# deepreinforce-ai/CUDA-L2

Measured on NVIDIA H100. Metric: HGEMM TFLOP/s, offline mode, per (M,N,K), higher is better.
Workload: dtype f16 x f16 -> f32 accumulate -> f16

## Files before the change

cuda_l2_b200/build.py:

```python
from __future__ import annotations

import os
import shutil
import subprocess
import sys
from pathlib import Path

PKG_DIR = Path(__file__).resolve().parent
REPO = PKG_DIR.parent
CSRC = PKG_DIR / "csrc"
LIB_DIR = PKG_DIR / "lib"

ARCH_FLAGS = ["-gencode", "arch=compute_90a,code=sm_90a"]
COMMON = ["-std=c++17", "-O3", "-lineinfo", "-Xcompiler", "-fPIC", "-Xcompiler", "-fno-gnu-unique"]


def nvcc_path() -> str:
    cand = os.environ.get("NVCC") or shutil.which("nvcc") or "/usr/local/cuda/bin/nvcc"
    if not Path(cand).exists():
        raise RuntimeError("nvcc not found: the HGEMM library cannot be built")
    return cand


def _stale(out: Path, inputs: list[Path]) -> bool:
    if not out.exists():
        return True
    t = out.stat().st_mtime
    return any(p.stat().st_mtime > t for p in inputs if p.exists())


def _run(cmd: list[str], verbose: bool) -> None:
    if verbose:
        print("+", " ".join(cmd), flush=True)
    r = subprocess.run(cmd, stdout=subprocess.PIPE, stderr=subprocess.STDOUT, text=True)
    if r.returncode != 0:
        sys.stderr.write(r.stdout)
        raise RuntimeError(f"build step failed ({r.returncode}): {' '.join(cmd)}")
    if verbose and r.stdout.strip():
        print(r.stdout)
    elif "warning" in r.stdout.lower():
        sys.stderr.write(r.stdout)
    if "C7510" in r.stdout:
        raise RuntimeError(f"ptxas serialised wgmma (warning C7510) in: {' '.join(cmd)}")


def _headers() -> list[Path]:
    return (sorted(CSRC.glob("*.cuh")) + sorted(CSRC.glob("*.inc")) + sorted(CSRC.glob("*.h")) +
            sorted((REPO / "include").glob("*.h")))


def _compile_and_link(out: Path, objects: list[tuple[Path, list[str]]], link_flags: list[str], verbose: bool,
                      force: bool) -> Path:
    LIB_DIR.mkdir(exist_ok=True)
    if force or _stale(out, [src for src, _ in objects] + _headers()):
        objs = [LIB_DIR / f"{out.stem}_{i}.o" for i in range(len(objects))]
        from concurrent.futures import ThreadPoolExecutor
        with ThreadPoolExecutor(len(objects)) as pool:
            for f in [pool.submit(_run, [nvcc_path(), *ARCH_FLAGS, *COMMON, *defines, "-c", "-o", str(obj), str(src)],
                                  verbose)
                      for (src, defines), obj in zip(objects, objs)]:
                f.result()
        _run([nvcc_path(), *ARCH_FLAGS, *COMMON, "--shared", "-o", str(out), *map(str, objs), *link_flags], verbose)
        for obj in objs:
            obj.unlink()
    return out


VARIANTS = (0, 1, 2)
BLOCK_VARIANTS = (5, 6)
BWD_VARIANTS = (0, 2)
EPILOGUE_VARIANTS = (0, 2, 3, 4)
BLOCK_1D1D_VARIANTS = (7, 8)
WGRAD_ACCUM_VARIANTS = (0, 2, 3, 7)
SWIGLU_VARIANTS = (0, 2)


def _per_variant(source: str, variants: tuple[int, ...]) -> list[tuple[Path, list[str]]]:
    return [(CSRC / source, [f"-DB200_VARIANT={v}"]) for v in variants]


LIBRARIES = {
    "capi": ("libb200_hgemm.so", [(CSRC / "b200_hgemm_capi.cu", []), (CSRC / "b200_fp8_capi.cu", [])], []),
    "fp8block": ("libb200_fp8block.so", [(CSRC / "b200_fp8_block_capi.cu", [])], []),
    "fp8block_1d1d": ("libb200_fp8block_1d1d.so", _per_variant("b200_fp8_block_1d1d.cu", BLOCK_1D1D_VARIANTS), []),
    "batched": ("libb200_batched.so", _per_variant("b200_batched_capi.cu", VARIANTS), []),
    "grouped": ("libb200_grouped.so", _per_variant("b200_grouped_capi.cu", VARIANTS), []),
    "grouped_fp8": ("libb200_grouped_fp8.so", _per_variant("b200_grouped_fp8_capi.cu", BLOCK_VARIANTS), []),
    "batched_fp8": ("libb200_batched_fp8.so", _per_variant("b200_batched_fp8_capi.cu", BLOCK_VARIANTS), []),
    "nn": ("libb200_nn.so", _per_variant("b200_nn.cu", VARIANTS), []),
    "grouped_bwd": ("libb200_grouped_bwd.so", _per_variant("b200_grouped_bwd.cu", BWD_VARIANTS), []),
    "epilogue": ("libb200_epilogue.so", _per_variant("b200_epilogue.cu", EPILOGUE_VARIANTS), []),
    "wgrad_accum": ("libb200_wgrad_accum.so", _per_variant("b200_wgrad_accum.cu", WGRAD_ACCUM_VARIANTS), []),
    "swiglu": ("libb200_swiglu.so", _per_variant("b200_swiglu.cu", SWIGLU_VARIANTS), []),
    "quant": ("libb200_quant.so", [(CSRC / "b200_quant.cu", [])], []),
    "quant_dual": ("libb200_quant_dual.so", [(CSRC / "b200_quant_dual.cu", [])], []),
    "quant_block_dual": ("libb200_quant_block_dual.so", [(CSRC / "b200_quant_block_dual.cu", [])], []),
    "baselines": ("libb200_baselines.so", [(CSRC / "b200_baselines_capi.cu", [])], ["-lcublas", "-lcublasLt"]),
}


def build_library(key: str, verbose: bool = False, force: bool = False) -> Path:
    name, objects, link_flags = LIBRARIES[key]
    return _compile_and_link(LIB_DIR / name, objects, link_flags, verbose, force)


def build_dev_check(verbose: bool = False, force: bool = False) -> Path:
    lib = build_library("capi", verbose, force)
    build_library("baselines", verbose, force)
    out = LIB_DIR / "dev_check"
    src = CSRC / "dev_check.cu"
    if force or _stale(out, [src, lib] + _headers()):
        _run([nvcc_path(), *ARCH_FLAGS, "-std=c++17", "-O3", "-lineinfo", "-o", str(out), str(src),
              f"-L{LIB_DIR}", "-lb200_hgemm", "-lb200_baselines", "-lcublas", "-Xlinker", "-rpath", "-Xlinker", "$ORIGIN"], verbose)
    return out


def build_all(verbose: bool = False, force: bool = False) -> dict[str, Path]:
    from concurrent.futures import ThreadPoolExecutor
    with ThreadPoolExecutor(len(LIBRARIES)) as pool:
        futures = {key: pool.submit(build_library, key, verbose, force) for key in LIBRARIES}
        out = {key: f.result() for key, f in futures.items()}
    out["dev_check"] = build_dev_check(verbose, force)
    return out


if __name__ == "__main__":
    for k, v in build_all(verbose=True, force="--force" in sys.argv).items():
        print(f"{k}: {v}")
```

cuda_l2_b200/capi.py:

```python
from __future__ import annotations

import ctypes
from pathlib import Path
from typing import NamedTuple

LIB_DIR = Path(__file__).resolve().parent / "lib"

ACC_BITS = {"fp32": 32, "fp16": 16, 32: 32, 16: 16}


class B200HgemmError(RuntimeError):
    pass


_vp, _i, _ip = ctypes.c_void_p, ctypes.c_int, ctypes.POINTER(ctypes.c_int)
_TILE_LIST_ABI = {
    "gemm": ([_i, _vp, _vp, _vp, _vp, _i, _i, _i, _i, _vp], _i),
    "gemm_run_config": ([_i, _i, _vp, _vp, _vp, _vp, _i, _i, _i, _i, _i, _i, _vp], _i),
    "select": ([_i, _i, _i, _i, _i, _ip, _ip], _i),
    "schedule_units": ([_i, _i, _i, _i, _i, _ip, _i, _i, _ip, _i, _ip], _i),
    "launch_count": ([], ctypes.c_ulonglong),
    "strerror": ([_i], ctypes.c_char_p),
}
_FP8_TILE_LIST_ABI = {
    "gemm": ([_vp, _vp, _vp, _vp, _i, _vp, _i, _vp, _i, _i, _i, _i, _vp], _i),
    "gemm_run_config": ([_i, _i, _vp, _vp, _vp, _vp, _i, _vp, _vp, _i, _i, _i, _i, _i, _i, _vp], _i),
    "select": ([_i, _i, _i, _i, _ip, _ip], _i),
    "launch_count": ([], ctypes.c_ulonglong),
    "strerror": ([_i], ctypes.c_char_p),
}


def _prefixed(prefix: str, abi: dict) -> dict:
    return {f"b200_{prefix}_{suffix}": sig for suffix, sig in abi.items()}


_GEMM = ([_vp, _vp, _vp, _vp, _i, _i, _i, _vp], _i)
_FP8GEMM = ([_vp, _vp, _vp, _vp, _vp, _i, _i, _i, _i, _vp], _i)
_FP8GEMM_RUN_CONFIG = ([_i, _i, _vp, _vp, _vp, _vp, _vp, _i, _i, _i, _i, _i, _i, _vp], _i)
_BASELINE = ([_i, _i, _vp, _vp, _vp, _i, _i, _i], _i)
ABI = {
    "libb200_hgemm.so": {
        "b200_hgemm_f32acc": _GEMM,
        "b200_hgemm_f16acc": _GEMM,
        "b200_bgemm_f32acc": _GEMM,
        "b200_bgemm_run_config": ([_i, _vp, _vp, _vp, _i, _i, _i, _i, _i, _i, _vp], _i),
        "b200_fp8gemm": _FP8GEMM,
        "b200_fp8gemm_run_config": _FP8GEMM_RUN_CONFIG,
        "b200_fp8gemm_rowwise": _FP8GEMM,
        "b200_fp8gemm_rowwise_run_config": _FP8GEMM_RUN_CONFIG,
        "b200_fp8gemm_select": ([_i, _i, _i, _ip, _ip, _ip], _i),
        "b200_hgemm_num_configs": ([], _i),
        "b200_hgemm_config_info": ([_i, _ip, _ip, _ip], _i),
        "b200_hgemm_config_cluster": ([_i, _ip, _ip], _i),
        "b200_hgemm_config_m_rep": ([_i], _i),
        "b200_hgemm_config_stages_requested": ([_i], _i),
        "b200_hgemm_select_config": ([_i, _i, _i, _i], _i),
        "b200_hgemm_select": ([_i, _i, _i, _i, _ip, _ip, _ip], _i),
        "b200_hgemm_run_config": ([_i, _i, _vp, _vp, _vp, _i, _i, _i, _i, _i, _i, _vp], _i),
        "b200_hgemm_host": ([_i, _vp, _vp, _vp, _i, _i, _i], _i),
        "b200_hgemm_schedule_units": ([_i, _i, _i, _i, _i, _i, _i, _ip, _i, _ip, _ip, _ip, _ip], _i),
        "b200_hgemm_prewarm": ([_vp], _i),
        "b200_hgemm_release": ([], _i),
        "b200_hgemm_launch_count": ([], ctypes.c_ulonglong),
        "b200_hgemm_strerror": ([_i], ctypes.c_char_p),
    },
    "libb200_fp8block.so": {
        "b200_fp8gemm_blockwise": ([_vp, _vp, _vp, _vp, _i, _vp, _i, _i, _i, _i, _vp], _i),
        "b200_fp8gemm_blockwise_run_config": ([_i, _i, _vp, _vp, _vp, _vp, _i, _vp, _i, _i, _i, _i, _i, _i, _vp], _i),
        "b200_fp8gemm_blockwise_select": ([_i, _i, _i, _ip, _ip, _ip], _i),
        "b200_fp8block_launch_count": ([], ctypes.c_ulonglong),
        "b200_fp8block_strerror": ([_i], ctypes.c_char_p),
    },
    "libb200_batched.so": _prefixed("batched", _TILE_LIST_ABI),
    "libb200_grouped.so": _prefixed("grouped", _TILE_LIST_ABI),
    "libb200_grouped_fp8.so": _prefixed("grouped_fp8", _FP8_TILE_LIST_ABI),
    "libb200_batched_fp8.so": _prefixed("batched_fp8", _FP8_TILE_LIST_ABI),
    "libb200_baselines.so": {
        "b200_bl_init": ([_i], _i),
        "b200_bl_destroy": ([_i], None),
        "b200_bl_cublas": _BASELINE,
        "b200_bl_lt_heuristic": _BASELINE,
        "b200_bl_lt_autotune_find": ([_i, _i, _i, _i, _i, _i, _i], _i),
        "b200_bl_lt_autotune": _BASELINE,
        "b200_bl_lt_autotune_info": ([_i, _i, _ip, ctypes.POINTER(ctypes.c_float)], _i),
    },
}
GROUPED_BWD_LIB = "libb200_grouped_bwd.so"
_BWD_RUN = ([_i, _i, _vp, _vp, _vp, _vp, _i, _i, _i, _i, _i, _i, _vp], _i)
_BWD_SELECT = ([_i, _i, _i, _i, _i, _ip, _ip], _i)
EPILOGUE_LIB = "libb200_epilogue.so"
QUANT_LIB = "libb200_quant.so"
QUANT_DUAL_LIB = "libb200_quant_dual.so"
FP8BLOCK_1D1D_LIB = "libb200_fp8block_1d1d.so"
QUANT_BLOCK_DUAL_LIB = "libb200_quant_block_dual.so"
WGRAD_ACCUM_LIB = "libb200_wgrad_accum.so"
SWIGLU_LIB = "libb200_swiglu.so"
_QUANT_BLOCK_DUAL = ([_i, _vp, _i, _i, _vp, _vp, _vp, _vp, _vp], _i)
_QUANT_BLOCKWISE = ([_i, _vp, _i, _i, _i, _vp, _vp, _i, _vp, _vp], _i)
INTERNAL_ABI = {
    GROUPED_BWD_LIB: {
        "cuda_l2_b200_grouped_bwd_nn": _BWD_RUN,
        "cuda_l2_b200_grouped_bwd_wgrad": _BWD_RUN,
        "cuda_l2_b200_grouped_bwd_nn_select": _BWD_SELECT,
        "cuda_l2_b200_grouped_bwd_wgrad_select": _BWD_SELECT,
        "cuda_l2_b200_grouped_bwd_wgrad_schedule": ([_i, _i, _i, _i, _i, _ip, _i, _i, _ip, _i, _ip], _i),
        "cuda_l2_b200_grouped_bwd_launch_count": ([], ctypes.c_ulonglong),
        "cuda_l2_b200_grouped_bwd_strerror": ([_i], ctypes.c_char_p),
    },
    EPILOGUE_LIB: {
        "cuda_l2_b200_epilogue_run": ([_i, _vp, _vp, _vp, _vp, _vp, _i, _vp, _i, _i, _i, _i, _vp], _i),
        "cuda_l2_b200_epilogue_run_config": ([_i, _i, _vp, _vp, _vp, _vp, _vp, _i, _vp, _i, _i, _i, _i, _i, _i, _i,
                                              _vp], _i),
        "cuda_l2_b200_epilogue_select": ([_i, _i, _i, _i, _ip, _ip, _ip], _i),
        "cuda_l2_b200_epilogue_prewarm": ([_vp], _i),
        "cuda_l2_b200_epilogue_release": ([], _i),
        "cuda_l2_b200_epilogue_launch_count": ([], ctypes.c_ulonglong),
        "cuda_l2_b200_epilogue_strerror": ([_i], ctypes.c_char_p),
    },
    QUANT_LIB: {
        "cuda_l2_b200_quant_e4m3_tensor": ([_i, _vp, ctypes.c_longlong, _vp, _vp, _vp, _vp], _i),
        "cuda_l2_b200_quant_e4m3_rowwise": ([_i, _vp, _i, _i, _vp, _vp, _vp], _i),
        "cuda_l2_b200_quant_e4m3_blockwise": _QUANT_BLOCKWISE,
        "cuda_l2_b200_quant_silu_mul_e4m3_blockwise": _QUANT_BLOCKWISE,
        "cuda_l2_b200_quant_launch_count": ([], ctypes.c_ulonglong),
        "cuda_l2_b200_quant_strerror": ([_i], ctypes.c_char_p),
    },
    QUANT_DUAL_LIB: {
        "cuda_l2_b200_quant_dual_e4m3_rowwise": ([_i, _vp, _i, _i, _vp, _vp, _vp, _vp, _vp, _vp], _i),
        "cuda_l2_b200_quant_dual_launch_count": ([], ctypes.c_ulonglong),
        "cuda_l2_b200_quant_dual_strerror": ([_i], ctypes.c_char_p),
    },
    FP8BLOCK_1D1D_LIB: {
        "cuda_l2_b200_fp8block_1d1d_run": ([_vp, _vp, _vp, _vp, _i, _vp, _i, _i, _i, _i, _i, _vp], _i),
        "cuda_l2_b200_fp8block_1d1d_run_config": ([_i, _i, _vp, _vp, _vp, _vp, _i, _vp, _i, _i, _i, _i, _i, _i, _i,
                                                   _vp], _i),
        "cuda_l2_b200_fp8block_1d1d_select": ([_i, _i, _i, _ip, _ip, _ip], _i),
        "cuda_l2_b200_fp8block_1d1d_launch_count": ([], ctypes.c_ulonglong),
        "cuda_l2_b200_fp8block_1d1d_strerror": ([_i], ctypes.c_char_p),
    },
    QUANT_BLOCK_DUAL_LIB: {
        "cuda_l2_b200_quant_block_dual_e4m3_1x128": _QUANT_BLOCK_DUAL,
        "cuda_l2_b200_quant_block_dual_e4m3_128x128": _QUANT_BLOCK_DUAL,
        "cuda_l2_b200_quant_block_dual_launch_count": ([], ctypes.c_ulonglong),
        "cuda_l2_b200_quant_block_dual_strerror": ([_i], ctypes.c_char_p),
    },
    WGRAD_ACCUM_LIB: {
        "cuda_l2_b200_wgrad_accum_grouped": _BWD_RUN,
        "cuda_l2_b200_wgrad_accum_fp8": ([_i, _i, _vp, _vp, _vp, _vp, _i, _vp, _i, _i, _i, _i, _i, _i, _i, _vp], _i),
        "cuda_l2_b200_wgrad_accum_grouped_select": _BWD_SELECT,
        "cuda_l2_b200_wgrad_accum_fp8_select": ([_i, _i, _i, _i, _ip, _ip, _ip], _i),
        "cuda_l2_b200_wgrad_accum_prewarm": ([_vp], _i),
        "cuda_l2_b200_wgrad_accum_release": ([], _i),
        "cuda_l2_b200_wgrad_accum_launch_count": ([], ctypes.c_ulonglong),
        "cuda_l2_b200_wgrad_accum_strerror": ([_i], ctypes.c_char_p),
    },
    SWIGLU_LIB: {
        "cuda_l2_b200_swiglu_run": ([_i, _vp, _vp, _vp, _vp, _i, _i, _i, _vp], _i),
        "cuda_l2_b200_swiglu_run_config": ([_i, _i, _vp, _vp, _vp, _vp, _i, _i, _i, _i, _i, _i, _vp], _i),
        "cuda_l2_b200_swiglu_select": ([_i, _i, _i, _i, _ip, _ip, _ip], _i),
        "cuda_l2_b200_swiglu_backward": ([_i, _vp, _vp, _vp, _i, _i, _vp], _i),
        "cuda_l2_b200_swiglu_launch_count": ([], ctypes.c_ulonglong),
        "cuda_l2_b200_swiglu_strerror": ([_i], ctypes.c_char_p),
    },
}
_TABLES = {**ABI, **INTERNAL_ABI}
_LIBRARY_OF = {symbol: name for name, table in _TABLES.items() for symbol in table}
_libs: dict = {}


def load(name: str) -> ctypes.CDLL:
    if name not in _libs:
        path = LIB_DIR / name
        if not path.exists():
            raise B200HgemmError(
                f"{path} is missing: build it with `python -c 'import __graft_entry__ as g; g.build()'` "
                "(or `python cuda_l2_b200/build.py`). There is no fallback path.")
        lib = ctypes.CDLL(str(path))
        for sym, (args, res) in _TABLES[name].items():
            fn = getattr(lib, sym)
            fn.argtypes, fn.restype = args, res
        _libs[name] = lib
    return _libs[name]


def hgemm_lib() -> ctypes.CDLL:
    return load("libb200_hgemm.so")


def fp8block_lib() -> ctypes.CDLL:
    return load("libb200_fp8block.so")


def batched_lib() -> ctypes.CDLL:
    return load("libb200_batched.so")


def grouped_lib() -> ctypes.CDLL:
    return load("libb200_grouped.so")


def grouped_fp8_lib() -> ctypes.CDLL:
    return load("libb200_grouped_fp8.so")


def batched_fp8_lib() -> ctypes.CDLL:
    return load("libb200_batched_fp8.so")


def baselines_lib() -> ctypes.CDLL:
    return load("libb200_baselines.so")


def exported_symbols() -> dict[str, list[str]]:
    return {name: list(symbols) for name, symbols in ABI.items()}


def strerror(status: int) -> str:
    return hgemm_lib().b200_hgemm_strerror(status).decode()


def _check(status: int, fn) -> None:
    if status != 0:
        symbol = fn if isinstance(fn, str) else fn.__name__
        name = _LIBRARY_OF[symbol]
        text = getattr(load(name), next(s for s in _TABLES[name] if s.endswith("_strerror")))(status).decode()
        raise B200HgemmError(f"{symbol} failed: status {status} ({text})")


def _shape_check(a, b_col_major, c):
    import torch

    for name, t in (("a", a), ("b_col_major", b_col_major), ("c", c)):
        if t.dtype != torch.half:
            raise B200HgemmError(f"{name} must be torch.half, got {t.dtype}")
        if not t.is_cuda:
            raise B200HgemmError(f"{name} must be a CUDA tensor")
        if not t.is_contiguous():
            raise B200HgemmError(f"{name} must be contiguous")
    m, k = a.shape
    kb, n = b_col_major.shape
    if kb != k or tuple(c.shape) != (m, n):
        raise B200HgemmError(f"shape mismatch: a {tuple(a.shape)}, b_col_major {tuple(b_col_major.shape)}, c {tuple(c.shape)}")
    return m, n, k


def hgemm(a, b_col_major, c, acc: str | int = "fp32", stream: int | None = None) -> None:
    m, n, k = _shape_check(a, b_col_major, c)
    bits = ACC_BITS[acc]
    fn = hgemm_lib().b200_hgemm_f32acc if bits == 32 else hgemm_lib().b200_hgemm_f16acc
    _check(fn(a.data_ptr(), None, b_col_major.data_ptr(), c.data_ptr(), m, n, k, stream), fn)


class GemmType(NamedTuple):
    k_align: int
    scale: object

    def fits(self, n: int, k: int) -> bool:
        return n % 8 == 0 and k % self.k_align == 0


_GEMM_TYPES: dict = {}


def gemm_type(operand, output, acc: str | int = "fp32") -> GemmType | None:
    if not _GEMM_TYPES:
        import torch
        h, b, e, f = torch.float16, torch.bfloat16, torch.float8_e4m3fn, torch.float32
        _GEMM_TYPES.update({(h, h, 32): GemmType(8, None), (h, h, 16): GemmType(8, None), (b, b, 32): GemmType(8, None),
                            (e, h, 32): GemmType(16, f), (e, b, 32): GemmType(16, f)})
    return _GEMM_TYPES.get((operand, output, ACC_BITS.get(acc)))


BLOCK = 128


def num_k_blocks(k: int) -> int:
    return -(-k // BLOCK)


def scale_granularity(m: int, n: int, scale_a, scale_b, k: int | None = None, groups: int | None = None,
                      batches: int | None = None) -> str:
    import torch

    sa, sb = tuple(scale_a.shape), tuple(scale_b.shape)
    lead_a = () if batches is None else (batches,)
    lead = lead_a if groups is None else (groups,)
    plain = groups is None and batches is None
    if scale_a.dtype == torch.float32 and scale_b.dtype == torch.float32:
        if plain and scale_a.numel() == 1 and scale_b.numel() == 1:
            return "tensor"
        if plain and sa == (m, 1) and sb == (1, n):
            return "rowwise"
        nkb = num_k_blocks(k) if k is not None else (sa[-1] if len(sa) == 2 + len(lead_a) else -1)
        if sa == (*lead_a, m, nkb) and sb == (*lead, -(-n // BLOCK), nkb):
            return "blockwise"
        if plain and sa == (m, nkb) and sb == (n, nkb) and n > -(-n // BLOCK):
            return "blockwise_1d1d"
    if groups is not None:
        raise B200HgemmError(f"grouped scales must be fp32 blockwise scales, scale_a [{m}, ceil(K/128)] with scale_b "
                             f"[{groups}, ceil({n}/128), ceil(K/128)], got {scale_a.dtype} {sa} and {scale_b.dtype} {sb}")
    if batches is not None:
        raise B200HgemmError(f"batched scales must be fp32 blockwise scales, scale_a [{batches}, {m}, ceil(K/128)] with "
                             f"scale_b [{batches}, ceil({n}/128), ceil(K/128)], got {scale_a.dtype} {sa} and "
                             f"{scale_b.dtype} {sb}")
    raise B200HgemmError(f"scales must be fp32 and either both one-element (per tensor), scale_a [{m}, 1] with "
                         f"scale_b [1, {n}] (rowwise), or scale_a [{m}, ceil(K/128)] with scale_b [ceil({n}/128), "
                         f"ceil(K/128)] (blockwise) or [{n}, ceil(K/128)] (blockwise_1d1d), got {scale_a.dtype} {sa} and "
                         f"{scale_b.dtype} {sb}")


def blockwise_ld_a(scale_a) -> int | None:
    *lead, m, nkb = scale_a.shape
    bsz, st = (lead[0] if lead else 1), scale_a.stride()
    ld = st[-1] if nkb > 1 else _m_major_ld(m)
    if nkb == 1 and bsz > 1:
        ld = st[0]
# ... 338 lines not shown
        raise B200HgemmError(f"the grouped backward takes fp16 or bf16 operands with fp32 accumulation, got {dtype} "
                             f"with acc={acc!r}")
    return v


def _bwd_operand_type(a, b, acc: str | int) -> GemmType:
    t = _operand_type(a, b, a.dtype, acc, (), scaled=False)
    _bwd_variant(a.dtype, acc)
    return t


def check_grouped_nn_operands(a, b, offs, acc: str | int = "fp32") -> tuple[int, int, int, int]:
    try:
        (t, k), (g, k2, n) = a.shape, b.shape
    except ValueError:
        raise B200HgemmError(f"a [T, K] and b [G, K, N] expected, got {tuple(a.shape)} and {tuple(b.shape)}") from None
    typ = _bwd_operand_type(a, b, acc)
    if k2 != k:
        raise B200HgemmError(f"inner dimensions differ: a {tuple(a.shape)}, b {tuple(b.shape)} (row-major: [G, K, N])")
    if not typ.fits(n, k):
        raise B200HgemmError(f"{a.dtype} operands need N % 8 == 0 and K % 8 == 0 (16-byte TMA strides), got N={n}, K={k}")
    _check_offs(offs, g)
    return g, t, n, k


def check_grouped_wgrad_operands(a, b, offs, acc: str | int = "fp32") -> tuple[int, int, int, int]:
    try:
        (t, m), (t2, n) = a.shape, b.shape
        (g,) = offs.shape
    except ValueError:
        raise B200HgemmError(f"a [T, M], b [T, N] and offs [G] expected, got {tuple(a.shape)}, {tuple(b.shape)} and "
                             f"{tuple(offs.shape)}") from None
    typ = _bwd_operand_type(a, b, acc)
    if t2 != t:
        raise B200HgemmError(f"row counts differ: a {tuple(a.shape)}, b {tuple(b.shape)}")
    if not typ.fits(n, m):
        raise B200HgemmError(f"{a.dtype} operands need M % 8 == 0 and N % 8 == 0 (16-byte TMA strides), got M={m}, N={n}")
    if g < 1:
        raise B200HgemmError("offs must hold at least one group")
    _check_offs(offs, g)
    return g, t, m, n


def _bwd_call(symbol: str, variant: int, ptrs: tuple, problem: tuple, config_id: int | None, group_m: int,
              max_ctas: int, stream: int | None) -> None:
    _check(getattr(grouped_bwd_lib(), symbol)(variant, -1 if config_id is None else config_id, *ptrs, *problem, group_m,
                                              max_ctas, stream), symbol)


def gemm_grouped_nn(a, b, c, offs, acc: str | int = "fp32", config_id: int | None = None, group_m: int = 0,
                    max_ctas: int = 0, stream: int | None = None) -> None:
    _contiguous_cuda(a=a, b=b, c=c, offs=offs)
    g, t, n, k = check_grouped_nn_operands(a, b, offs, acc)
    if c.dtype != a.dtype or tuple(c.shape) != (t, n):
        raise B200HgemmError(f"c must be {a.dtype} {[t, n]}, got {c.dtype} {tuple(c.shape)}")
    _bwd_call("cuda_l2_b200_grouped_bwd_nn", _bwd_variant(a.dtype, acc), (a.data_ptr(), b.data_ptr(), c.data_ptr(),
              offs.data_ptr()), (g, t, n, k), config_id, group_m, max_ctas, stream)


def gemm_grouped_wgrad(a, b, c, offs, acc: str | int = "fp32", config_id: int | None = None, group_m: int = 0,
                       max_ctas: int = 0, stream: int | None = None) -> None:
    _contiguous_cuda(a=a, b=b, c=c, offs=offs)
    g, t, m, n = check_grouped_wgrad_operands(a, b, offs, acc)
    if c.dtype != a.dtype or tuple(c.shape) != (g, m, n):
        raise B200HgemmError(f"c must be {a.dtype} {[g, m, n]}, got {c.dtype} {tuple(c.shape)}")
    _bwd_call("cuda_l2_b200_grouped_bwd_wgrad", _bwd_variant(a.dtype, acc), (a.data_ptr(), b.data_ptr(), c.data_ptr(),
              offs.data_ptr()), (g, t, m, n), config_id, group_m, max_ctas, stream)


def grouped_nn_select(variant: int, g: int, t: int, n: int, k: int) -> tuple[int, int]:
    return _select(grouped_bwd_lib().cuda_l2_b200_grouped_bwd_nn_select, variant, g, t, n, k)


def grouped_wgrad_select(variant: int, g: int, t: int, m: int, n: int) -> tuple[int, int]:
    return _select(grouped_bwd_lib().cuda_l2_b200_grouped_bwd_wgrad_select, variant, g, t, m, n)


def grouped_wgrad_schedule(config_id: int, t: int, m: int, n: int, offs, num_sms: int = 132) -> dict:
    ends = (ctypes.c_int * len(offs))(*offs)
    return _tile_list_schedule(grouped_bwd_lib().cuda_l2_b200_grouped_bwd_wgrad_schedule, 4, config_id, len(offs), t,
                               m, n, ends, num_sms)


def grouped_bwd_launch_count() -> int:
    return int(grouped_bwd_lib().cuda_l2_b200_grouped_bwd_launch_count())


def fp8_grouped_gemm(a, b_kmajor, c, scale_a, scale_b, offs, config_id: int | None = None, group_m: int = 0,
                     max_ctas: int = 0, stream: int | None = None) -> None:
    _tile_list_gemm("grouped", a, b_kmajor, c, offs, "fp32", (scale_a, scale_b), config_id, group_m, max_ctas, stream)


def fp8_grouped_select(g: int, t: int, n: int, k: int) -> tuple[int, int]:
    return _select(grouped_fp8_lib().b200_grouped_fp8_select, g, t, n, k)


def fp8_grouped_launch_count() -> int:
    return int(grouped_fp8_lib().b200_grouped_fp8_launch_count())


def fp8_batched_gemm(a, b_kmajor, c, scale_a, scale_b, masked_m=None, config_id: int | None = None, group_m: int = 0,
                     max_ctas: int = 0, stream: int | None = None) -> None:
    _tile_list_gemm("batched", a, b_kmajor, c, masked_m, "fp32", (scale_a, scale_b), config_id, group_m, max_ctas,
                    stream)


def fp8_batched_select(b: int, m: int, n: int, k: int) -> tuple[int, int]:
    return _select(batched_fp8_lib().b200_batched_fp8_select, b, m, n, k)


def fp8_batched_launch_count() -> int:
    return int(batched_fp8_lib().b200_batched_fp8_launch_count())


def hgemm_config(a, b_col_major, c, config_id: int, acc: str | int = "fp32", group_m: int = 0, max_ctas: int = 0,
                 splits: int = 1, stream: int | None = None) -> None:
    m, n, k = _shape_check(a, b_col_major, c)
    _check(hgemm_lib().b200_hgemm_run_config(ACC_BITS[acc], config_id, a.data_ptr(), b_col_major.data_ptr(),
                                            c.data_ptr(), m, n, k, group_m, max_ctas, splits, stream), "b200_hgemm_run_config")


def hgemm_host(a_host, b_col_major_host, c_host, acc: str | int = "fp32") -> None:
    m, k = a_host.shape
    kb, n = b_col_major_host.shape
    assert kb == k and tuple(c_host.shape) == (m, n)
    for t in (a_host, b_col_major_host, c_host):
        assert (not t.is_cuda) and t.is_contiguous()
    _check(hgemm_lib().b200_hgemm_host(ACC_BITS[acc], a_host.data_ptr(), b_col_major_host.data_ptr(),
                                       c_host.data_ptr(), m, n, k), "b200_hgemm_host")


def configs() -> list[dict]:
    lib = hgemm_lib()
    out = []
    for cid in range(lib.b200_hgemm_num_configs()):
        bn, st, cg = ctypes.c_int(), ctypes.c_int(), ctypes.c_int()
        lib.b200_hgemm_config_info(cid, ctypes.byref(bn), ctypes.byref(st), ctypes.byref(cg))
        cm, cn = ctypes.c_int(), ctypes.c_int()
        lib.b200_hgemm_config_cluster(cid, ctypes.byref(cm), ctypes.byref(cn))
        out.append({"id": cid, "bn": bn.value, "stages": st.value, "cta_group": cg.value,
                    "stages_requested": lib.b200_hgemm_config_stages_requested(cid),
                    "cluster_m": cm.value, "cluster_n": cn.value, "m_rep": lib.b200_hgemm_config_m_rep(cid)})
    return out


def select_config(acc: str | int, m: int, n: int, k: int) -> int:
    return hgemm_lib().b200_hgemm_select_config(ACC_BITS[acc], m, n, k)


def select(acc: str | int, m: int, n: int, k: int) -> tuple[int, int, int]:
    return _select(hgemm_lib().b200_hgemm_select, ACC_BITS[acc], m, n, k)


STREAMK_TAIL, STREAMK_TAIL_PLUS_WAVE = 100, 101
KMODES = ("plain", "split-k", "cluster-split-k", "stream-k")


def schedule(config_id: int, m: int, n: int, k: int, splits: int = 1, num_sms: int = 132) -> dict:
    lib = hgemm_lib()
    nw, sk, mode = ctypes.c_int(), ctypes.c_int(), ctypes.c_int()
    cap = 64
    buf, contrib = (ctypes.c_int * (3 * cap))(), (ctypes.c_int * cap)()
    st = lib.b200_hgemm_schedule_units(config_id, m, n, k, splits, num_sms, 0, buf, cap, ctypes.byref(nw),
                                       ctypes.byref(sk), ctypes.byref(mode), contrib)
    _check(min(st, 0), "b200_hgemm_schedule_units")
    units = []
    for w in range(nw.value):
        cnt = lib.b200_hgemm_schedule_units(config_id, m, n, k, splits, num_sms, w, buf, cap, None, None, None, contrib)
        _check(min(cnt, 0), "b200_hgemm_schedule_units")
        if cnt > cap:
            cap = cnt
            buf, contrib = (ctypes.c_int * (3 * cap))(), (ctypes.c_int * cap)()
            cnt = lib.b200_hgemm_schedule_units(config_id, m, n, k, splits, num_sms, w, buf, cap, None, None, None, contrib)
        units.append([(buf[3 * j], buf[3 * j + 1], buf[3 * j + 2], contrib[j]) for j in range(cnt)])
    return {"workers": nw.value, "sk_tiles": sk.value, "mode": KMODES[mode.value], "units": units}


def prewarm(stream: int | None = None) -> None:
    _check(hgemm_lib().b200_hgemm_prewarm(stream), "b200_hgemm_prewarm")


def release() -> None:
    _check(hgemm_lib().b200_hgemm_release(), "b200_hgemm_release")


def gpu_local_cpus(device_index: int = 0) -> set[int] | None:
    import os

    try:
        import pynvml as nv
        nv.nvmlInit()
        vis = os.environ.get("CUDA_VISIBLE_DEVICES")
        phys = device_index
        if vis:
            try:
                phys = int(vis.split(",")[device_index])
            except (ValueError, IndexError):
                pass
        h = nv.nvmlDeviceGetHandleByIndex(phys)
        words = nv.nvmlDeviceGetCpuAffinity(h, ((os.cpu_count() or 64) + 63) // 64)
        cpus = {64 * w + b for w, word in enumerate(words) for b in range(64) if (int(word) >> b) & 1}
        cpus &= os.sched_getaffinity(0)
        return cpus or None
    except Exception:
        return None


class host_near_gpu:

    def __init__(self, device_index: int = 0):
        self.device_index, self.saved, self.cpus = device_index, None, None

    def __enter__(self):
        import os
        self.cpus = gpu_local_cpus(self.device_index)
        if self.cpus:
            self.saved = os.sched_getaffinity(0)
            try:
                os.sched_setaffinity(0, self.cpus)
            except OSError:
                self.saved, self.cpus = None, None
        return self

    def __exit__(self, *exc):
        import os
        if self.saved is not None:
            os.sched_setaffinity(0, self.saved)
        return False


def launch_count() -> int:
    return int(hgemm_lib().b200_hgemm_launch_count())


class Baselines:

    NN, TN = 0, 1

    def __init__(self, acc: str | int = "fp32"):
        self.bits = ACC_BITS[acc]
        self.lib = baselines_lib()
        if self.lib.b200_bl_init(self.bits) != 0:
            raise B200HgemmError("cuBLAS/cuBLASLt handle creation failed")

    def close(self):
        self.lib.b200_bl_destroy(self.bits)

    def _call(self, fn, layout, a, b, c):
        m, k = a.shape
        n = c.shape[1]
        st = fn(self.bits, layout, a.data_ptr(), b.data_ptr(), c.data_ptr(), m, n, k)
        if st != 0:
            raise B200HgemmError(f"baseline call failed with status {st}")

    def cublas(self, layout, a, b, c):
        self._call(self.lib.b200_bl_cublas, layout, a, b, c)

    def lt_heuristic(self, layout, a, b, c):
        self._call(self.lib.b200_bl_lt_heuristic, layout, a, b, c)

    def lt_autotune_find(self, layout, m, n, k, warm_rounds=0, bench_rounds=0):
        st = self.lib.b200_bl_lt_autotune_find(self.bits, layout, m, n, k, warm_rounds, bench_rounds)
        if st != 0:
            raise B200HgemmError(f"cuBLASLt auto-tuning failed with status {st}")
        cand, ms = ctypes.c_int(), ctypes.c_float()
        self.lib.b200_bl_lt_autotune_info(self.bits, layout, ctypes.byref(cand), ctypes.byref(ms))
        return cand.value, ms.value

    def lt_autotune(self, layout, a, b, c):
        self._call(self.lib.b200_bl_lt_autotune, layout, a, b, c)


ACTIVATIONS = {"none": 0, "relu": 1, "gelu_tanh": 2}


def epilogue_lib() -> ctypes.CDLL:
    return load(EPILOGUE_LIB)


def epilogue_variant(operand, out_dtype) -> int:
    import torch

    variants = {(torch.float16, torch.float16): 0, (torch.bfloat16, torch.bfloat16): 2,
                (torch.float8_e4m3fn, torch.float16): 3, (torch.float8_e4m3fn, torch.bfloat16): 4}
    if (operand, out_dtype) not in variants:
        raise B200HgemmError(f"no bias + activation kernel for {operand} -> {out_dtype} (fp16, bf16 with fp32 accumulation; "
                             f"e4m3 -> fp16 / bf16 with per-tensor or rowwise scales)")
    return variants[(operand, out_dtype)]


def activation_code(activation: str) -> int:
    if activation not in ACTIVATIONS:
        raise B200HgemmError(f"unknown activation {activation!r}: one of {', '.join(ACTIVATIONS)}")
    return ACTIVATIONS[activation]


def check_bias(bias, n: int, out_dtype) -> None:
    if bias is not None and (bias.dim() != 1 or bias.shape[0] != n or bias.dtype != out_dtype):
        raise B200HgemmError(f"bias must be 1-D with N = {n} elements of {out_dtype}, got {bias.dtype} "
                             f"{tuple(bias.shape)}")


def _aligned(t):
    if t is None:
        return None
    t = t.contiguous()
# ... 352 lines not shown
```

cuda_l2_b200/csrc/b200_hgemm_capi.cu:

```cuda
#include "../../include/b200_hgemm.h"

#include <dlfcn.h>

#include <cstdlib>
#include <map>
#include <memory>
#include <mutex>
#include <string>

#include "b200_nn.h"
#include "hgemm_configs.cuh"
#include "hgemm_dispatch.cuh"

namespace {

using b200::host::GemmType;

template <class Cfg>
int schedule_units(int M, int N, int K, int splits, int num_sms, int worker, int* units, int max_units,
                   int* num_workers, int* sk_tiles, int* mode, int* contributors) {
  using namespace b200;
  const int max_workers = num_sms / Cfg::CLUSTER_CTAS;
  const host::Plan p = host::plan<Cfg>(M, N, K, splits, max_workers, [=] { return max_workers; });
  if (num_workers) *num_workers = p.workers;
  if (sk_tiles) *sk_tiles = p.sk_tiles;
  if (mode) *mode = p.mode;
  if (worker < 0 || worker >= p.workers) return host::kBadShape;
  WorkIter it(worker, p.workers, p.num_tiles, p.nkb, p.splits, p.sk_tiles);
  WorkUnit u;
  int n = 0;
  while (it.next(u)) {
    if (n < max_units && units) {
      units[3 * n] = u.tile; units[3 * n + 1] = u.kb0; units[3 * n + 2] = u.kb1;
      if (contributors)
        contributors[n] = (p.sk_tiles && u.kb0 == 0 && u.kb1 < p.nkb)
                              ? streamk_contributors(worker, p.workers, p.sk_tiles * p.nkb, u.tile, p.nkb) : 0;
    }
    ++n;
  }
  return n;
}

const b200::ConfigDesc* config_desc(int id) { return id >= 0 && id < b200::kNumConfigs ? &b200::kConfigs[id] : nullptr; }

GemmType fp16_type(int acc_bits) { return acc_bits == 32 ? GemmType::kF16Acc32 : GemmType::kF16Acc16; }

constexpr int kHostBlocks = 8;
struct HostCtx {
  std::mutex mu;
  void* dbuf = nullptr; size_t dcap = 0;
  cudaStream_t in = nullptr, run = nullptr, out = nullptr;
  cudaEvent_t b_in = nullptr, a_in[kHostBlocks] = {}, done[kHostBlocks] = {};
};
std::mutex g_host_mu;
std::map<int, std::unique_ptr<HostCtx>> g_host_ctx;
HostCtx& host_ctx(int dev) {
  std::lock_guard<std::mutex> lock(g_host_mu);
  auto& slot = g_host_ctx[dev];
  if (!slot) slot.reset(new HostCtx());
  return *slot;
}

b200::nn::RunConfigFn nn_run_config() {
  static const b200::nn::RunConfigFn fn = []() -> b200::nn::RunConfigFn {
    Dl_info self{};
    if (!dladdr(reinterpret_cast<const void*>(&nn_run_config), &self) || !self.dli_fname) return nullptr;
    const std::string here(self.dli_fname);
    const size_t slash = here.rfind('/');
    const std::string path = (slash == std::string::npos ? std::string() : here.substr(0, slash + 1)) + b200::nn::kLibrary;
    void* lib = dlopen(path.c_str(), RTLD_NOW | RTLD_LOCAL);
    return lib ? reinterpret_cast<b200::nn::RunConfigFn>(dlsym(lib, b200::nn::kRunConfigSymbol)) : nullptr;
  }();
  return fn;
}

template <GemmType T>
int gemm_rowmajor(const void* A, const void* B_rowmajor, void* C, int M, int N, int K, void* stream) {
  if (const int st = b200::host::validate(T, A, B_rowmajor, C, {}, M, N, K)) return st;
  const b200::nn::RunConfigFn run = nn_run_config();
  if (!run) return b200::host::kNoNNLibrary;
  const b200::dispatch::Choice ch = b200::dispatch::select_rowmajor(T, M, N, K);
  const int st = run(int(T), ch.config_id, A, B_rowmajor, C, M, N, K, ch.group_m, 0, ch.splits,
                     &b200::host::splitk_scratch, stream);
  if (st == b200::host::kOk) b200::g_launches.fetch_add(1, std::memory_order_relaxed);
  return st;
}

}

extern "C" {

int b200_hgemm_num_configs(void) { return b200::kNumConfigs; }

int b200_hgemm_config_info(int config_id, int* bn, int* stages, int* cta_group) {
  const b200::ConfigDesc* c = config_desc(config_id);
  if (!c) return b200::host::kBadConfig;
  if (bn) *bn = c->bn;
  if (stages) *stages = c->stages;
  if (cta_group) *cta_group = c->cta_group;
  return 0;
}

int b200_hgemm_config_cluster(int config_id, int* cluster_m, int* cluster_n) {
  const b200::ConfigDesc* c = config_desc(config_id);
  if (!c) return b200::host::kBadConfig;
  if (cluster_m) *cluster_m = c->cluster_m;
  if (cluster_n) *cluster_n = c->cluster_n;
  return 0;
}

int b200_hgemm_schedule_units(int config_id, int M, int N, int K, int splits, int num_sms, int worker, int* units,
                              int max_units, int* num_workers, int* sk_tiles, int* mode, int* contributors) {
  if (M <= 0 || N <= 0 || K <= 0 || num_sms <= 0) return b200::host::kBadShape;
  switch (config_id) {
#define B200_CASE(ID, BN, STAGES, CG, CM, CN, MR)                                                                   \
  case ID:                                                                                                          \
    return schedule_units<b200::Config<BN, STAGES, CG, true, CM, CN, MR>>(M, N, K, splits, num_sms, worker, units, \
                                                                          max_units, num_workers, sk_tiles, mode, contributors);
    B200_HGEMM_CONFIGS(B200_CASE)
#undef B200_CASE
    default:
      return b200::host::kBadConfig;
  }
}

int b200_hgemm_config_stages_requested(int config_id) {
  const b200::ConfigDesc* c = config_desc(config_id);
  return c ? c->stages_requested : b200::host::kBadConfig;
}

int b200_hgemm_config_m_rep(int config_id) {
  const b200::ConfigDesc* c = config_desc(config_id);
  return c ? c->m_rep : b200::host::kBadConfig;
}

int b200_hgemm_select_config(int acc_bits, int M, int N, int K) {
  if (acc_bits != 32 && acc_bits != 16) return b200::host::kBadConfig;
  if (M <= 0 || N <= 0 || K <= 0) return b200::host::kBadShape;
  return b200::dispatch::select(fp16_type(acc_bits), M, N, K).config_id;
}

int b200_hgemm_select(int acc_bits, int M, int N, int K, int* config_id, int* group_m, int* splits) {
  if (acc_bits != 32 && acc_bits != 16) return b200::host::kBadConfig;
  if (M <= 0 || N <= 0 || K <= 0) return b200::host::kBadShape;
  const b200::dispatch::Choice ch = b200::dispatch::select(fp16_type(acc_bits), M, N, K);
  if (config_id) *config_id = ch.config_id;
  if (group_m) *group_m = ch.group_m;
  if (splits) *splits = ch.splits;
  return 0;
}

int b200_hgemm_run_config(int acc_bits, int config_id, const void* A, const void* B_kmajor, void* C, int M,
                          int N, int K, int group_m, int max_ctas, int splits, void* stream) {
  if (acc_bits == 32)
    return b200::run_config<GemmType::kF16Acc32>(config_id, A, B_kmajor, C, {}, M, N, K, group_m, max_ctas, splits, stream);
  if (acc_bits == 16)
    return b200::run_config<GemmType::kF16Acc16>(config_id, A, B_kmajor, C, {}, M, N, K, group_m, max_ctas, splits, stream);
  return b200::host::kBadConfig;
}

int b200_hgemm_f32acc(const void* A, const void* B_rowmajor, const void* B_kmajor, void* C, int M, int N,
                      int K, void* stream) {
  if (!B_kmajor && B_rowmajor) return gemm_rowmajor<GemmType::kF16Acc32>(A, B_rowmajor, C, M, N, K, stream);
  return b200::dispatch::gemm<GemmType::kF16Acc32>(A, B_kmajor, C, {}, M, N, K, stream);
}

int b200_hgemm_f16acc(const void* A, const void* B_rowmajor, const void* B_kmajor, void* C, int M, int N,
                      int K, void* stream) {
  if (!B_kmajor && B_rowmajor) return gemm_rowmajor<GemmType::kF16Acc16>(A, B_rowmajor, C, M, N, K, stream);
  return b200::dispatch::gemm<GemmType::kF16Acc16>(A, B_kmajor, C, {}, M, N, K, stream);
}

int b200_bgemm_f32acc(const void* A, const void* B_rowmajor, const void* B_kmajor, void* C, int M, int N,
                      int K, void* stream) {
  if (!B_kmajor && B_rowmajor) return gemm_rowmajor<GemmType::kBF16>(A, B_rowmajor, C, M, N, K, stream);
  return b200::dispatch::gemm<GemmType::kBF16>(A, B_kmajor, C, {}, M, N, K, stream);
}

int b200_bgemm_run_config(int config_id, const void* A, const void* B_kmajor, void* C, int M, int N, int K,
                          int group_m, int max_ctas, int splits, void* stream) {
  return b200::run_config<GemmType::kBF16>(config_id, A, B_kmajor, C, {}, M, N, K, group_m, max_ctas, splits, stream);
}

int b200_hgemm_host(int acc_bits, const void* hA, const void* hB_kmajor, void* hC, int M, int N, int K) {
  if (!hA || !hB_kmajor || !hC) return b200::host::kNullPointer;
  if (M <= 0 || N <= 0 || K <= 0) return b200::host::kBadShape;
  if (acc_bits != 32 && acc_bits != 16) return b200::host::kBadConfig;
  int dev = 0;
  cudaError_t e = cudaGetDevice(&dev);
  if (e != cudaSuccess) return int(e);
  HostCtx& ctx = host_ctx(dev);
  std::lock_guard<std::mutex> turn(ctx.mu);
  const size_t a_bytes = size_t(M) * K * 2, b_bytes = size_t(N) * K * 2, c_bytes = size_t(M) * N * 2;
  auto up = [](size_t x) { return (x + 255) & ~size_t(255); };
  const size_t need = up(a_bytes) + up(b_bytes) + up(c_bytes);
  if (need > ctx.dcap) {
    if (ctx.dbuf) cudaFree(ctx.dbuf);
    ctx.dbuf = nullptr; ctx.dcap = 0;
    if ((e = cudaMalloc(&ctx.dbuf, need)) != cudaSuccess) return int(e);
    ctx.dcap = need;
  }
  char* dA = static_cast<char*>(ctx.dbuf);
  char* dB = dA + up(a_bytes);
  char* dC = dB + up(b_bytes);
  auto gemm = [&](const void* a, void* c, int m, cudaStream_t s) {
    return acc_bits == 32 ? b200_hgemm_f32acc(a, nullptr, dB, c, m, N, K, s) : b200_hgemm_f16acc(a, nullptr, dB, c, m, N, K, s);
  };

  const int blocks = std::min(kHostBlocks, M / 512);
  const bool pipelined = blocks >= 2 && (a_bytes + c_bytes) >= (size_t(8) << 20) &&
                         !(std::getenv("B200_HGEMM_HOST_UNPIPELINED"));
  if (!pipelined) {
    if ((e = cudaMemcpyAsync(dA, hA, a_bytes, cudaMemcpyHostToDevice, 0)) != cudaSuccess) return int(e);
    if ((e = cudaMemcpyAsync(dB, hB_kmajor, b_bytes, cudaMemcpyHostToDevice, 0)) != cudaSuccess) return int(e);
    int st = gemm(dA, dC, M, nullptr);
    if (st) return st;
    if ((e = cudaMemcpyAsync(hC, dC, c_bytes, cudaMemcpyDeviceToHost, 0)) != cudaSuccess) return int(e);
    e = cudaStreamSynchronize(0);
    return e == cudaSuccess ? 0 : int(e);
  }

  if (!ctx.in) {
    if ((e = cudaStreamCreateWithFlags(&ctx.in, cudaStreamNonBlocking)) != cudaSuccess) return int(e);
    if ((e = cudaStreamCreateWithFlags(&ctx.run, cudaStreamNonBlocking)) != cudaSuccess) return int(e);
    if ((e = cudaStreamCreateWithFlags(&ctx.out, cudaStreamNonBlocking)) != cudaSuccess) return int(e);
    if ((e = cudaEventCreateWithFlags(&ctx.b_in, cudaEventDisableTiming)) != cudaSuccess) return int(e);
    for (int i = 0; i < kHostBlocks; ++i) {
      if ((e = cudaEventCreateWithFlags(&ctx.a_in[i], cudaEventDisableTiming)) != cudaSuccess) return int(e);
      if ((e = cudaEventCreateWithFlags(&ctx.done[i], cudaEventDisableTiming)) != cudaSuccess) return int(e);
    }
  }
  if ((e = cudaStreamSynchronize(0)) != cudaSuccess) return int(e);
  const int rows_per = ((M + blocks - 1) / blocks + 127) / 128 * 128;
  if ((e = cudaMemcpyAsync(dB, hB_kmajor, b_bytes, cudaMemcpyHostToDevice, ctx.in)) != cudaSuccess) return int(e);
  if ((e = cudaEventRecord(ctx.b_in, ctx.in)) != cudaSuccess) return int(e);
  if ((e = cudaStreamWaitEvent(ctx.run, ctx.b_in, 0)) != cudaSuccess) return int(e);
  for (int i = 0; i < blocks; ++i) {
    const int r0 = i * rows_per, rows = std::min(rows_per, M - r0);
    if (rows <= 0) break;
    const size_t a_off = size_t(r0) * K * 2, c_off = size_t(r0) * N * 2;
    if ((e = cudaMemcpyAsync(dA + a_off, static_cast<const char*>(hA) + a_off, size_t(rows) * K * 2, cudaMemcpyHostToDevice, ctx.in)) != cudaSuccess) return int(e);
    if ((e = cudaEventRecord(ctx.a_in[i], ctx.in)) != cudaSuccess) return int(e);
    if ((e = cudaStreamWaitEvent(ctx.run, ctx.a_in[i], 0)) != cudaSuccess) return int(e);
    int st = gemm(dA + a_off, dC + c_off, rows, ctx.run);
    if (st) { cudaDeviceSynchronize(); return st; }
    if ((e = cudaEventRecord(ctx.done[i], ctx.run)) != cudaSuccess) return int(e);
    if ((e = cudaStreamWaitEvent(ctx.out, ctx.done[i], 0)) != cudaSuccess) return int(e);
    if ((e = cudaMemcpyAsync(static_cast<char*>(hC) + c_off, dC + c_off, size_t(rows) * N * 2, cudaMemcpyDeviceToHost, ctx.out)) != cudaSuccess) return int(e);
  }
  if ((e = cudaStreamSynchronize(ctx.out)) != cudaSuccess) return int(e);
  if ((e = cudaStreamSynchronize(ctx.run)) != cudaSuccess) return int(e);
  e = cudaStreamSynchronize(ctx.in);
  return e == cudaSuccess ? 0 : int(e);
}

int b200_hgemm_prewarm(void* stream) {
  int dev = 0;
  cudaError_t e = cudaGetDevice(&dev);
  if (e != cudaSuccess) return int(e);
  b200::host::SplitKScratch* sk = nullptr;
  return b200::host::splitk_scratch(dev, static_cast<cudaStream_t>(stream), &sk);
}

int b200_hgemm_release(void) {
  b200::host::release_scratch();
  int cur = 0;
  cudaGetDevice(&cur);
  std::lock_guard<std::mutex> lock(g_host_mu);
  for (auto& kv : g_host_ctx) {
    HostCtx& c = *kv.second;
    std::lock_guard<std::mutex> turn(c.mu);
    cudaSetDevice(kv.first);
    cudaDeviceSynchronize();
    if (c.dbuf) cudaFree(c.dbuf);
    c.dbuf = nullptr; c.dcap = 0;
    if (c.in) {
      cudaStreamDestroy(c.in); cudaStreamDestroy(c.run); cudaStreamDestroy(c.out);
      cudaEventDestroy(c.b_in);
      for (int i = 0; i < kHostBlocks; ++i) { cudaEventDestroy(c.a_in[i]); cudaEventDestroy(c.done[i]); }
      c.in = c.run = c.out = nullptr;
    }
  }
  cudaSetDevice(cur);
  cudaError_t e = cudaGetLastError();
  return e == cudaSuccess ? 0 : int(e);
}

unsigned long long b200_hgemm_launch_count(void) { return b200::g_launches.load(std::memory_order_relaxed); }

const char* b200_hgemm_strerror(int status) { return b200::host::status_string(status); }

}
```

cuda_l2_b200/csrc/hgemm_configs.cuh:

```cuda
#pragma once
#include <atomic>
#include <type_traits>

#include "hgemm_host.cuh"

#define B200_HGEMM_CONFIGS(X) \
  X(0, 256, 4, 1, 1, 1, 1)       \
  X(1, 128, 6, 1, 1, 1, 1)       \
  X(2, 64, 8, 1, 1, 1, 1)        \
  X(3, 256, 6, 2, 1, 1, 1)       \
  X(4, 128, 8, 2, 1, 1, 1)       \
  X(5, 192, 4, 1, 1, 1, 1)       \
  X(6, 192, 6, 2, 1, 1, 1)       \
  X(7, 64, 8, 1, 1, 2, 1)        \
  X(8, 64, 8, 1, 1, 4, 1)        \
  X(9, 64, 8, 1, 2, 2, 1)        \
  X(10, 128, 6, 1, 1, 2, 1)      \
  X(11, 128, 6, 1, 2, 2, 1)      \
  X(12, 32, 9, 1, 1, 1, 1)       \
  X(13, 32, 9, 1, 1, 4, 1)       \
  X(14, 32, 9, 1, 1, 8, 1)       \
  X(15, 64, 8, 1, 2, 1, 1)       \
  X(16, 64, 8, 1, 4, 1, 1)       \
  X(17, 128, 6, 1, 2, 1, 1)      \
  X(18, 256, 4, 1, 1, 2, 1)      \
  X(19, 256, 4, 1, 2, 1, 1)      \
  X(20, 256, 6, 2, 1, 2, 1)      \
  X(21, 256, 6, 2, 2, 1, 1)      \
  X(22, 128, 8, 2, 1, 2, 1)      \
  X(23, 128, 8, 2, 2, 1, 1)      \
  X(24, 192, 6, 2, 1, 2, 1)      \
  X(25, 192, 6, 2, 2, 1, 1)     \
  X(26, 128, 4, 2, 1, 1, 2)      \
  X(27, 128, 4, 2, 2, 1, 2)      \
  X(28, 128, 4, 2, 1, 2, 2)      \
  X(29, 256, 6, 2, 2, 2, 1)      \
  X(30, 128, 8, 2, 2, 2, 1)

namespace b200 {
constexpr int kNumConfigs = 31;

struct ConfigDesc {
  int bn, stages, stages_requested, cta_group, cluster_m, cluster_n, m_rep;
  bool split_k, stream_k;
};
template <class Cfg>
constexpr ConfigDesc describe(int stages_requested) {
  return ConfigDesc{Cfg::BN, Cfg::STAGES, stages_requested, Cfg::CTA_GROUP, Cfg::CLUSTER_M, Cfg::CLUSTER_N, Cfg::M_REP,
                    Cfg::SPLIT_K, Cfg::STREAM_K};
}
constexpr ConfigDesc kConfigs[kNumConfigs] = {
#define B200_DESC(ID, BN, STAGES, CG, CM, CN, MR) describe<Config<BN, STAGES, CG, true, CM, CN, MR>>(STAGES),
    B200_HGEMM_CONFIGS(B200_DESC)
#undef B200_DESC
};

namespace block {

constexpr bool eligible(int id) { return kConfigs[id].m_rep * kConfigs[id].bn <= 128; }

constexpr int sibling(int id) {
  const ConfigDesc& c = kConfigs[id];
  const int bn = c.bn < 128 ? c.bn : 128;
  for (int j = 0; j < kNumConfigs; ++j) {
    const ConfigDesc& d = kConfigs[j];
    if (d.cta_group == c.cta_group && d.cluster_m == c.cluster_m && d.cluster_n == c.cluster_n && d.m_rep == 1 &&
        d.bn == bn)
      return j;
  }
  return -1;
}
constexpr bool every_config_has_an_eligible_sibling() {
  for (int id = 0; id < kNumConfigs; ++id) {
    const int s = sibling(id);
    if (s < 0 || !eligible(s) || (eligible(id) && s != id)) return false;
  }
  return true;
}
static_assert(every_config_has_an_eligible_sibling(), "the configuration table lost a block-scaled sibling");

constexpr unsigned kModes = (1u << kPlain) | (1u << kClusterSplitK);

}

namespace nn {

constexpr bool has_kernel(int id) { return kConfigs[id].bn % 64 == 0; }

constexpr int sibling(int id) {
  const ConfigDesc& c = kConfigs[id];
  if (has_kernel(id)) return id;
  int best = -1;
  for (int j = 0; j < kNumConfigs; ++j) {
    const ConfigDesc& d = kConfigs[j];
    if (d.bn == 64 && d.cta_group == c.cta_group && d.cluster_m == c.cluster_m && d.m_rep == c.m_rep &&
        d.cluster_n <= c.cluster_n && (best < 0 || d.cluster_n > kConfigs[best].cluster_n))
      best = j;
  }
  return best;
}
constexpr bool every_config_has_a_sibling() {
  for (int id = 0; id < kNumConfigs; ++id) {
    const int s = sibling(id);
    if (s < 0 || !has_kernel(s) || (has_kernel(id) && s != id)) return false;
  }
  return true;
}
static_assert(every_config_has_a_sibling(), "the configuration table lost a row-major B sibling");

}

namespace gated {

constexpr bool has_kernel(int id) { return kConfigs[id].bn == 128 || kConfigs[id].bn == 256; }

constexpr int sibling(int id) {
  const ConfigDesc& c = kConfigs[id];
  if (has_kernel(id)) return id;
  int best = -1;
  for (int j = 0; j < kNumConfigs; ++j) {
    const ConfigDesc& d = kConfigs[j];
    if (d.bn == 128 && d.cta_group == c.cta_group && d.m_rep == c.m_rep && d.cluster_m <= c.cluster_m &&
        d.cluster_n <= c.cluster_n &&
        (best < 0 || d.cluster_m * d.cluster_n > kConfigs[best].cluster_m * kConfigs[best].cluster_n))
      best = j;
  }
  return best;
}
constexpr bool every_config_has_a_sibling() {
  for (int id = 0; id < kNumConfigs; ++id) {
    const int s = sibling(id);
    if (s < 0 || !has_kernel(s) || (has_kernel(id) && s != id)) return false;
  }
  return true;
}
static_assert(every_config_has_a_sibling(), "the configuration table lost a SwiGLU sibling");

constexpr unsigned kModes = 1u << kPlain;

}

template <class Probe>
constexpr bool has_kernel(int id) {
  return block_scaled<Probe>() ? block::eligible(id)
         : row_major_b<Probe>() ? nn::has_kernel(id)
         : is_gated<Probe>()    ? gated::has_kernel(id)
                                : true;
}
template <class Probe>
constexpr unsigned k_modes() { return block_scaled<Probe>() ? block::kModes : is_gated<Probe>() ? gated::kModes : 0xFu; }

template <class Cfg>
using Unwrapped = Cfg;

__attribute__((visibility("hidden"))) inline std::atomic<unsigned long long> g_launches{0};

template <host::GemmType T, template <class> class Wrapper = Unwrapped>
int run_config(int id, const void* A, const void* Bt, void* C, Scales scales, int M, int N, int K, int group_m,
               int max_ctas, int splits, void* stream, int ld_a = 0, host::ScratchFn scratch = host::splitk_scratch,
               const void* bias = nullptr, int act = kActNone, int ld_b = 0) {
  constexpr host::GemmTypeTraits t = host::traits(T);
  using Probe = Wrapper<Config<128, 6, 1, t.acc_f32, 1, 1, 1, t.bf16(), t.e4m3()>>;
  const cudaStream_t s = static_cast<cudaStream_t>(stream);
  int st = host::kBadConfig;
  switch (id) {
#define B200_CASE(ID, BN, STAGES, CG, CM, CN, MR)                                                                  \
  case ID:                                                                                                     \
    if constexpr (has_kernel<Probe>(ID))                                                                       \
      st = host::launch<Wrapper<Config<BN, STAGES, CG, t.acc_f32, CM, CN, MR, t.bf16(), t.e4m3()>>,            \
                        k_modes<Probe>()>(A, Bt, C, M, N, K, s, group_m, max_ctas, splits, scales, ld_a, scratch, \
                                          bias, act, ld_b);                                                    \
    break;
    B200_HGEMM_CONFIGS(B200_CASE)
#undef B200_CASE
    default:
      break;
  }
  if (st == host::kOk) g_launches.fetch_add(1, std::memory_order_relaxed);
  return st;
}

namespace tile_list {

inline bool known_out(int out_bf16) { return out_bf16 == 0 || out_bf16 == 1; }
inline host::GemmType block_type(int out_bf16) { return host::GemmType(int(host::GemmType::kE4M3F16Block) + out_bf16); }
inline Scales block_scales(const void* a, const void* b) {
  return Scales{static_cast<const float*>(a), static_cast<const float*>(b)};
}

__attribute__((visibility("hidden"))) inline std::atomic<unsigned long long> g_list_launches{0};

template <host::GemmType T, class Cfg>
using Variant = std::conditional_t<host::traits(T).block, BlockScaled<Cfg>, Cfg>;

template <template <class> class Wrapper, host::GemmType T>
int run_config(int id, const void* A, const void* Bt, void* C, const int* list, int count, int rows, int N, int K,
               int group_m, int max_ctas, cudaStream_t s, Scales scales, int ld_a) {
  constexpr host::GemmTypeTraits t = host::traits(T);
  static_assert(!t.scaled || t.block, "16-bit or block-scaled variants");
  using Probe = Wrapper<Variant<T, Config<128, 6, 1, t.acc_f32, 1, 1, 1, t.bf16(), t.e4m3()>>>;
  int st = host::kBadConfig;
  switch (id) {
#define B200_CASE(ID, BN, STAGES, CG, CM, CN, MR)                                                                  \
  case ID:                                                                                                     \
    if constexpr (has_kernel<Probe>(ID))                                                                       \
      st = host::launch_list<Wrapper<Variant<T, Config<BN, STAGES, CG, t.acc_f32, CM, CN, MR, t.bf16(), t.e4m3()>>>>( \
          A, Bt, C, list, count, rows, N, K, s, group_m, max_ctas, scales, ld_a);                               \
    break;
    B200_HGEMM_CONFIGS(B200_CASE)
#undef B200_CASE
    default:
      break;
  }
  if (st == host::kOk && rows > 0 && K > 0) g_list_launches.fetch_add(1, std::memory_order_relaxed);
  return st;
}

template <template <class> class Wrapper, host::GemmType... Types>
struct ListLibrary {};

template <template <class> class Wrapper, host::GemmType... Types>
constexpr bool holds(ListLibrary<Wrapper, Types...>, int variant) {
  return ((variant == int(Types)) || ...);
}

template <template <class> class Wrapper>
using ListProbe = Wrapper<Config<128, 6, 1, true>>;

#define B200_LIST_TYPES(X, W) X(W, host::GemmType::kF16Acc32) X(W, host::GemmType::kF16Acc16) X(W, host::GemmType::kBF16)
#define B200_BLOCK_LIST_TYPES(X, W) X(W, host::GemmType::kE4M3F16Block) X(W, host::GemmType::kE4M3BF16Block)

#define B200_LIST_RUN(W, T)                                                                                    \
  int run_config<W, T>(int, const void*, const void*, void*, const int*, int, int, int, int, int, int, cudaStream_t, \
                       Scales, int)
#define B200_LIST_EXTERN(W, T) extern template B200_LIST_RUN(W, T);
#define B200_LIST_ARG(W, T) , T
#define B200_LIST_OBJECT(NAME, W, TYPES)                                                                       \
  TYPES(B200_LIST_EXTERN, W)                                                                                   \
  template B200_LIST_RUN(W, host::GemmType(B200_VARIANT));                                                     \
  using NAME = ListLibrary<W TYPES(B200_LIST_ARG, W)>

template <template <class> class Wrapper, host::GemmType... Types>
int run(ListLibrary<Wrapper, Types...>, host::GemmType type, int config_id, const void* A, const void* Bt, void* C,
        Scales scales, int ld_a, const int* list, int count, int rows, int N, int K, int group_m, int max_ctas,
        void* stream) {
  const cudaStream_t s = static_cast<cudaStream_t>(stream);
  int st = host::kBadConfig;
  (void)((type == Types && (st = run_config<Wrapper, Types>(config_id, A, Bt, C, list, count, rows, N, K, group_m,
                                                            max_ctas, s, scales, ld_a), true)) || ...);
  return st;
}

template <class Cfg>
int schedule_units(int count, int rows, int N, int K, const int* list, int num_sms, int worker, int* units,
                   int max_units, int* num_workers) {
  const long long tiles = Cfg::Cursor::template max_tiles<Cfg>(count, rows, N);
  if (tiles > 0x7fffffffLL) return host::kBadShape;
  const int max_workers = num_sms / Cfg::CLUSTER_CTAS;
  const host::Plan p = host::list_plan<Cfg>(tiles, K, max_workers, [=] { return max_workers; });
  if (num_workers) *num_workers = p.workers;
  if (worker < 0 || worker >= p.workers) return host::kBadShape;
  const int n_blocks = (N + Cfg::BN * Cfg::CLUSTER_N - 1) / (Cfg::BN * Cfg::CLUSTER_N);
  typename Cfg::Cursor cursor = make_cursor<Cfg>(list, count, rows, K, Cfg::TILE_M * Cfg::CLUSTER_M, n_blocks,
                                                 host::default_group_m<Cfg>());
  constexpr int kInts = k_grouped<Cfg>() ? 4 : 3;
  WorkIter it(worker, p.workers, cursor.total(), p.nkb, 1, 0);
  WorkUnit u;
  int n = 0;
  while (it.next(u)) {
    BatchTile bt;
    if constexpr (k_grouped<Cfg>()) bt = cursor.unit(u);
    else bt = cursor.locate(u.tile);
    if (n < max_units && units) {
      int* v = units + kInts * n;
      v[0] = bt.batch; v[1] = bt.tc.m_blk; v[2] = bt.tc.n_blk;
      if constexpr (k_grouped<Cfg>()) v[3] = u.kb1 - u.kb0;
    }
    ++n;
  }
  return n;
}

template <template <class> class Wrapper>
long long fewest_tiles(int count, int rows, int N, bool block_only = false) {
  long long fewest = 0x7fffffffffffffffLL;
#define B200_TILES(ID, BN, STAGES, CG, CM, CN, MR)                                                               \
  if constexpr (has_kernel<ListProbe<Wrapper>>(ID)) {                                                           \
    using W = Wrapper<Config<BN, STAGES, CG, true, CM, CN, MR>>;                                                \
    if (!block_only || block::eligible(ID))                                                                     \
      fewest = std::min(fewest, W::Cursor::template max_tiles<W>(count, rows, N));                              \
  }
  B200_HGEMM_CONFIGS(B200_TILES)
#undef B200_TILES
  return fewest;
}

template <template <class> class Wrapper>
int schedule_config(int config_id, int count, int rows, int N, int K, const int* list, int num_sms, int worker,
                    int* units, int max_units, int* num_workers) {
  switch (config_id) {
#define B200_CASE(ID, BN, STAGES, CG, CM, CN, MR)                                                                 \
  case ID:                                                                                                      \
    if constexpr (has_kernel<ListProbe<Wrapper>>(ID))                                                           \
// ... 15 lines not shown
```

cuda_l2_b200/csrc/hgemm_host.cuh:

```cuda
#pragma once
#include <cuda.h>
#include <cuda_runtime.h>
#include <cstdint>
#include <cstdio>
#include <cstring>
#include <cstdlib>
#include <algorithm>
#include <deque>
#include <mutex>

#include "hgemm_sm90.cuh"

namespace b200 {
namespace host {

enum Status : int {
  kOk = 0,
  kBadShape = -1,
  kBadAlignment = -2,
  kNoDriver = -3,
  kEncodeFailed = -4,
  kNullPointer = -5,
  kBadConfig = -6,
  kNotHopper = -7,
  kNoScratch = -8,
  kBadFp8K = -9,
  kBadScaleLd = -10,
  kNoNNLibrary = -11,
  kBadActivation = -12,
  kBadScaleLdB = -13,
};

inline const char* status_string(int s) {
  switch (s) {
    case kOk: return "ok";
    case kBadShape: return "M, N and K must be positive";
    case kBadAlignment: return "operands must be 16-byte aligned with K % 8 == 0 and N % 8 == 0";
    case kNoDriver: return "cuTensorMapEncodeTiled unavailable (driver too old?)";
    case kEncodeFailed: return "cuTensorMapEncodeTiled failed";
    case kNullPointer: return "null operand pointer";
    case kBadConfig: return "unknown kernel configuration id";
    case kNotHopper: return "device is not compute capability 9.0 (sm_90a build)";
    case kNoScratch: return "split-K scratch unavailable (allocate it outside stream capture with b200_hgemm_prewarm)";
    case kBadFp8K: return "e4m3 operands need K % 16 == 0 (16-byte row strides at one byte per element)";
    case kBadScaleLd: return "block scales need ld_a >= M and ld_a % 4 == 0 (16-byte aligned k-block rows of A's scales)";
    case kNoNNLibrary: return "row-major B needs libb200_nn.so next to libb200_hgemm.so (missing, or it does not load)";
    case kBadActivation: return "unknown activation code (0 none, 1 relu, 2 gelu_tanh)";
    case kBadScaleLdB: return "1 x 128 scales of Bt need ld_b >= N and ld_b % 4 == 0 (16-byte aligned k-block rows)";
    default: return s > 0 ? cudaGetErrorString(static_cast<cudaError_t>(s)) : "unknown error";
  }
}

using EncodeTiledFn = CUresult (*)(CUtensorMap*, CUtensorMapDataType, cuuint32_t, void*, const cuuint64_t*,
                                   const cuuint64_t*, const cuuint32_t*, const cuuint32_t*,
                                   CUtensorMapInterleave, CUtensorMapSwizzle, CUtensorMapL2promotion,
                                   CUtensorMapFloatOOBfill);

inline EncodeTiledFn encode_fn() {
  static EncodeTiledFn fn = [] {
    void* p = nullptr;
    cudaDriverEntryPointQueryResult q;
    if (cudaGetDriverEntryPoint("cuTensorMapEncodeTiled", &p, cudaEnableDefault, &q) != cudaSuccess ||
        q != cudaDriverEntryPointSuccess)
      p = nullptr;
    return reinterpret_cast<EncodeTiledFn>(p);
  }();
  return fn;
}

enum class Elem : int { kF16 = 0, kBF16 = 1, kE4M3 = 2 };
constexpr int elem_bytes(Elem e) { return e == Elem::kE4M3 ? 1 : 2; }

enum class GemmType : int { kF16Acc32, kF16Acc16, kBF16, kE4M3F16, kE4M3BF16, kE4M3F16Block, kE4M3BF16Block,
                            kE4M3F16Block1D1D, kE4M3BF16Block1D1D };
struct GemmTypeTraits {
  Elem operand, output;
  bool acc_f32;
  int table_k_div;
  bool scaled;
  bool block = false;
  bool block_1d1d = false;
  constexpr bool bf16() const { return output == Elem::kBF16; }
  constexpr bool e4m3() const { return operand == Elem::kE4M3; }
};
constexpr GemmTypeTraits kGemmTypes[] = {
    {Elem::kF16, Elem::kF16, true, 1, false},
    {Elem::kF16, Elem::kF16, false, 1, false},
    {Elem::kBF16, Elem::kBF16, true, 1, false},
    {Elem::kE4M3, Elem::kF16, true, 2, true},
    {Elem::kE4M3, Elem::kBF16, true, 2, true},
    {Elem::kE4M3, Elem::kF16, true, 2, true, true},
    {Elem::kE4M3, Elem::kBF16, true, 2, true, true},
    {Elem::kE4M3, Elem::kF16, true, 2, true, true, true},
    {Elem::kE4M3, Elem::kBF16, true, 2, true, true, true},
};
constexpr const GemmTypeTraits& traits(GemmType t) { return kGemmTypes[int(t)]; }

template <class Cfg>
constexpr GemmType gemm_type(int t = 0) {
  const GemmTypeTraits& x = kGemmTypes[t];
  return x.acc_f32 == Cfg::ACC_F32 && x.bf16() == Cfg::BF16 && x.e4m3() == Cfg::E4M3 && x.block == block_scaled<Cfg>() &&
                 x.block_1d1d == block_1d1d<Cfg>()
             ? GemmType(t) : gemm_type<Cfg>(t + 1);
}

inline int encode_2d(CUtensorMap* map, const void* ptr, int rows, int cols, int box_rows, int box_cols = kBlockK,
                     Elem elem = Elem::kF16, int batches = 0) {
  EncodeTiledFn fn = encode_fn();
  if (!fn) return kNoDriver;
  const cuuint32_t rank = batches > 0 ? 3 : 2;
  cuuint64_t dims[3] = {cuuint64_t(cols), cuuint64_t(rows), cuuint64_t(batches)};
  cuuint64_t strides[2] = {cuuint64_t(cols) * elem_bytes(elem), cuuint64_t(rows) * cuuint64_t(cols) * elem_bytes(elem)};
  cuuint32_t box[3] = {cuuint32_t(box_cols), cuuint32_t(box_rows), 1};
  cuuint32_t estr[3] = {1, 1, 1};
  const CUtensorMapSwizzle swz = box_cols * elem_bytes(elem) == 128 ? CU_TENSOR_MAP_SWIZZLE_128B : CU_TENSOR_MAP_SWIZZLE_64B;
  static const CUtensorMapL2promotion promo = [] {
    const char* e = std::getenv("B200_HGEMM_L2_PROMOTION");
    const int v = (e && e[0] >= '0' && e[0] <= '3') ? e[0] - '0' : 3;
    return v == 0 ? CU_TENSOR_MAP_L2_PROMOTION_NONE : v == 1 ? CU_TENSOR_MAP_L2_PROMOTION_L2_64B
         : v == 2 ? CU_TENSOR_MAP_L2_PROMOTION_L2_128B : CU_TENSOR_MAP_L2_PROMOTION_L2_256B;
  }();
  const CUtensorMapDataType dt = elem == Elem::kE4M3 ? CU_TENSOR_MAP_DATA_TYPE_UINT8
                               : elem == Elem::kBF16 ? CU_TENSOR_MAP_DATA_TYPE_BFLOAT16 : CU_TENSOR_MAP_DATA_TYPE_FLOAT16;
  CUresult r = fn(map, dt, rank, const_cast<void*>(ptr), dims, strides, box, estr,
                  CU_TENSOR_MAP_INTERLEAVE_NONE, swz, promo, CU_TENSOR_MAP_FLOAT_OOB_FILL_NONE);
  return r == CUDA_SUCCESS ? kOk : kEncodeFailed;
}

struct MapKey {
  const void* ptr; int rows, cols, box_rows, box_cols; Elem elem; int batches;
  bool operator==(const MapKey& o) const {
    return ptr == o.ptr && rows == o.rows && cols == o.cols && box_rows == o.box_rows && box_cols == o.box_cols &&
           elem == o.elem && batches == o.batches;
  }
};
struct MapCache {
  static constexpr int kSlots = 64;
  MapKey keys[kSlots];
  CUtensorMap maps[kSlots];
  bool valid[kSlots];
  MapCache() { std::memset(valid, 0, sizeof(valid)); }
  int get(const void* ptr, int rows, int cols, int box_rows, CUtensorMap* out, int box_cols = kBlockK, Elem elem = Elem::kF16,
          int batches = 0) {
    MapKey k{ptr, rows, cols, box_rows, box_cols, elem, batches};
    uint64_t h = (reinterpret_cast<uint64_t>(ptr) >> 8) * 0x9E3779B97F4A7C15ull;
    h ^= uint64_t(uint32_t(rows)) * 0xC2B2AE3D27D4EB4Full + uint64_t(uint32_t(cols)) * 0x165667B19E3779F9ull +
         uint64_t(box_rows) * 131u + uint64_t(box_cols) + uint64_t(uint32_t(batches)) * 0x27D4EB2F165667C5ull;
    int slot = int((h >> 32) % kSlots);
    if (!(valid[slot] && keys[slot] == k)) {
      int st = encode_2d(&maps[slot], ptr, rows, cols, box_rows, box_cols, elem, batches);
      if (st != kOk) { valid[slot] = false; return st; }
      keys[slot] = k;
      valid[slot] = true;
    }
    std::memcpy(out, &maps[slot], sizeof(CUtensorMap));
    return kOk;
  }
};
inline MapCache& map_cache() {
  static thread_local MapCache c;
  return c;
}

struct DeviceInfo { int dev; int num_sms; int cc_major; };
inline const DeviceInfo& device_info() {
  static thread_local int cached_dev = -1;
  static thread_local DeviceInfo info{-1, 0, 0};
  int dev = 0;
  cudaGetDevice(&dev);
  if (dev != cached_dev) {
    cudaSetDevice(dev);
    cudaDeviceGetAttribute(&info.num_sms, cudaDevAttrMultiProcessorCount, dev);
    cudaDeviceGetAttribute(&info.cc_major, cudaDevAttrComputeCapabilityMajor, dev);
    info.dev = dev;
    cached_dev = dev;
  }
  return info;
}

inline int validate(GemmType type, const void* A, const void* Bt, const void* C, Scales scales, int M, int N, int K,
                    int ld_a = 0, int batches = 1, long long tiles = 1, const int* list = nullptr) {
  const GemmTypeTraits& t = traits(type);
  if (!A || !Bt || !C || (t.scaled && (!scales.a || !scales.b))) return kNullPointer;
  if (M <= 0 || N <= 0 || K <= 0 || batches < 1 || tiles > 0x7fffffffLL) return kBadShape;
  if (reinterpret_cast<uintptr_t>(list) & 3) return kBadAlignment;
  if (K % (16 / elem_bytes(t.operand))) return t.e4m3() ? kBadFp8K : kBadAlignment;
  if (N % 8) return kBadAlignment;
  if ((reinterpret_cast<uintptr_t>(A) | reinterpret_cast<uintptr_t>(Bt) | reinterpret_cast<uintptr_t>(C)) & 15)
    return kBadAlignment;
  if (t.block) {
    if ((reinterpret_cast<uintptr_t>(scales.a) & 15) || (reinterpret_cast<uintptr_t>(scales.b) & (t.block_1d1d ? 15 : 3)))
      return kBadAlignment;
    if (ld_a < M || ld_a % 4) return kBadScaleLd;
    return kOk;
  }
  if (t.scaled && ((reinterpret_cast<uintptr_t>(scales.a) | reinterpret_cast<uintptr_t>(scales.b)) & (scales.rowwise ? 15 : 3)))
    return kBadAlignment;
  return kOk;
}

inline int validate_bias_act(const void* bias, int act) {
// ... 167 lines not shown
inline bool cooperative_enabled() {
  static const bool on = [] { const char* e = std::getenv("B200_HGEMM_NO_COOPERATIVE"); return !(e && e[0] == '1'); }();
  return on;
}

inline bool pdl_enabled() {
  static const bool on = [] { const char* e = std::getenv("B200_HGEMM_NO_PDL"); return !(e && e[0] == '1'); }();
  return on;
}

struct LaunchArgs {
  CUtensorMap ma, mb, mc;
  int M, N, K, group_m;
  Plan plan;
  float* ws; unsigned* ctr; __half* c;
  uint64_t hint_a, hint_b;
  Scales scales;
  int ld_a;
  int ld_b;
  int batches;
  const int* masked_m;
  cudaStream_t stream;
  const void* bias;
  int act;
  GatedArgs gated;
};

template <class Cfg>
typename Cfg::EpiArgs epi_args(const LaunchArgs& a) {
  if constexpr (is_gated<Cfg>()) return a.gated;
  else if constexpr (accum_f32<Cfg>())
    return typename Cfg::EpiArgs{epi_args<typename Cfg::AccumBase>(a), reinterpret_cast<float*>(a.c)};
  else if constexpr (bias_act<Cfg>()) return BiasActArgs{a.scales, a.bias, a.act};
  else if constexpr (block_1d1d<Cfg>()) return Block1D1DArgs{a.scales, a.ld_b};
  else return a.scales;
}

template <class Cfg, int KMODE>
int launch_mode(const DeviceInfo& di, const LaunchArgs& a) {
  static thread_local int attr_dev = -1;
  static thread_local const void* attr_fn = nullptr;
  constexpr auto kernel = kernel_of<Cfg, KMODE>();
  const void* this_fn = reinterpret_cast<const void*>(kernel);
  if (attr_dev != di.dev || attr_fn != this_fn) {
    cudaError_t e = cudaFuncSetAttribute(kernel, cudaFuncAttributeMaxDynamicSharedMemorySize, Cfg::SMEM_BYTES);
    if (e != cudaSuccess) return int(e);
    attr_dev = di.dev;
    attr_fn = this_fn;
  }
  constexpr bool kSplit = (KMODE == kWorkspaceSplitK || KMODE == kClusterSplitK);
  const int cluster = (KMODE == kClusterSplitK) ? a.plan.cluster_reduce : Cfg::CLUSTER_CTAS;
  cudaLaunchConfig_t cfg{};
  cfg.gridDim = dim3(unsigned(a.plan.workers * (kSplit ? 1 : Cfg::CLUSTER_CTAS)), 1, 1);
  cfg.blockDim = dim3(Cfg::NUM_THREADS, 1, 1);
  cfg.dynamicSmemBytes = Cfg::SMEM_BYTES;
  cfg.stream = a.stream;
  cudaLaunchAttribute attr[3];
  unsigned na = 0;
  if (cluster > 1) {
    attr[na].id = cudaLaunchAttributeClusterDimension;
    attr[na].val.clusterDim.x = unsigned(cluster);
    attr[na].val.clusterDim.y = 1;
    attr[na].val.clusterDim.z = 1;
    ++na;
  }
  const bool coop = (KMODE == kWorkspaceSplitK || KMODE == kStreamK) && cooperative_enabled();
  if (coop) {
    attr[na].id = cudaLaunchAttributeCooperative;
    attr[na].val.cooperative = 1;
    ++na;
  }
  static bool coop_pdl_ok = [] { const char* e = std::getenv("B200_HGEMM_COOP_PDL"); return e && e[0] == '1'; }();
  const bool pdl = pdl_enabled() && (!coop || coop_pdl_ok);
  if (pdl) {
    attr[na].id = cudaLaunchAttributeProgrammaticStreamSerialization;
    attr[na].val.programmaticStreamSerializationAllowed = 1;
    ++na;
  }
  cfg.attrs = attr;
  cfg.numAttrs = na;
  const int aux = block_scaled<Cfg>() ? a.ld_a : a.plan.sk_tiles;
  constexpr bool kTileList = batched<Cfg>() || grouped<Cfg>() || k_grouped<Cfg>();
  const int splits_arg = kTileList ? a.batches : a.plan.splits;
  unsigned* ctr = kTileList ? reinterpret_cast<unsigned*>(const_cast<int*>(a.masked_m)) : a.ctr;
  cudaError_t e = cudaLaunchKernelEx(&cfg, kernel, a.ma, a.mb, a.mc, a.M, a.N, a.K, a.group_m, splits_arg, aux, a.ws,
                                     ctr, a.c, a.hint_a, a.hint_b, epi_args<Cfg>(a));
  if (e != cudaSuccess && coop && pdl && e != cudaErrorCooperativeLaunchTooLarge) {
    cudaGetLastError();
    coop_pdl_ok = false;
    cfg.numAttrs = na - 1;
    e = cudaLaunchKernelEx(&cfg, kernel, a.ma, a.mb, a.mc, a.M, a.N, a.K, a.group_m, splits_arg, aux, a.ws, ctr, a.c,
                           a.hint_a, a.hint_b, epi_args<Cfg>(a));
  }
  return e == cudaSuccess ? kOk : int(e);
}

template <class Cfg>
constexpr int default_group_m() { return Cfg::CTA_GROUP == 2 ? 8 : 16; }

template <class Cfg, unsigned MODES = 0xFu>
int launch(const void* A, const void* Bt, void* C, int M, int N, int K, cudaStream_t stream,
           int group_m = 0, int max_ctas = 0, int splits = 1, Scales scales = Scales{nullptr, nullptr}, int ld_a = 0,
           ScratchFn scratch = splitk_scratch, const void* bias = nullptr, int act = kActNone, int ld_b = 0,
           void* y = nullptr) {
  constexpr GemmType kType = gemm_type<Cfg>();
  [[maybe_unused]] const bool store_h = C != nullptr;
  if constexpr (is_gated<Cfg>()) {
    if (!y) return kNullPointer;
    if (!C) C = y;
    if ((reinterpret_cast<uintptr_t>(y) & 15) || N % 128) return kBadAlignment;
  }
  int st = validate(kType, A, Bt, C, scales, M, N, K, ld_a);
  if (st != kOk) return st;
  if constexpr (bias_act<Cfg>()) {
    if ((st = validate_bias_act(bias, act)) != kOk) return st;
  }
  if constexpr (block_1d1d<Cfg>()) {
    if (ld_b < N || ld_b % 4) return kBadScaleLdB;
  }
  const DeviceInfo& di = device_info();
  if (di.cc_major != 9) return kNotHopper;

  LaunchArgs a{};
  MapCache& cache = map_cache();
  const Elem operand = traits(kType).operand, output = traits(kType).output;
  if ((st = cache.get(A, M, K, Cfg::A_BOX_ROWS, &a.ma, Cfg::BLOCK_K, operand)) != kOk) return st;
  if constexpr (row_major_b<Cfg>()) {
    if ((st = cache.get(Bt, K, N, Cfg::B_K_ROWS, &a.mb, 64, operand)) != kOk) return st;
  } else {
    if ((st = cache.get(Bt, N, K, Cfg::B_BOX_ROWS, &a.mb, Cfg::BLOCK_K, operand)) != kOk) return st;
  }
  if constexpr (is_gated<Cfg>()) {
    if ((st = cache.get(store_h ? C : y, M, store_h ? N : N / 2, Cfg::EPI_ROWS, &a.mc, Cfg::EPI_N, output)) != kOk)
      return st;
    if ((st = cache.get(y, M, N / 2, Cfg::EPI_ROWS, &a.gated.y_map, Cfg::EPI_N, output)) != kOk) return st;
    a.gated.store_h = store_h ? 1 : 0;
  } else {
    if ((st = cache.get(C, M, N, Cfg::EPI_ROWS, &a.mc, Cfg::EPI_N, output)) != kOk) return st;
  }

  const int max_workers = (max_ctas > 0 ? max_ctas : di.num_sms) / Cfg::CLUSTER_CTAS;
  a.plan = plan<Cfg, MODES>(M, N, K, splits, max_workers, [&] { return max_resident_clusters<Cfg>(di); });
  if (a.plan.mode == kWorkspaceSplitK || a.plan.mode == kStreamK) {
    SplitKScratch* sk = nullptr;
    if (scratch(di.dev, stream, &sk) == kOk) {
      a.ws = sk->ws; a.ctr = sk->ctr;
    } else {
      cudaGetLastError();
      a.plan = undivided(a.plan);
    }
  }
  a.M = M; a.N = N; a.K = K;
  a.group_m = group_m > 0 ? group_m : default_group_m<Cfg>();
  a.c = static_cast<__half*>(C);
  a.scales = scales;
  a.ld_a = ld_a;
  a.ld_b = ld_b;
  a.stream = stream;
  a.bias = bias;
  a.act = act;
  a.hint_a = ptx::kL2EvictNormal; a.hint_b = ptx::kL2EvictNormal;
  if (cache_hints_enabled()) {
    const size_t a_bytes = size_t(M) * K * Cfg::OP_BYTES, b_bytes = size_t(N) * K * Cfg::OP_BYTES;
    const int n_tiles = (N + Cfg::BN - 1) / Cfg::BN, m_tiles = (M + Cfg::TILE_M - 1) / Cfg::TILE_M;
    constexpr size_t kL2Keep = size_t(20) << 20, kStream = size_t(40) << 20;
    if (a_bytes >= kStream && b_bytes <= kL2Keep && n_tiles <= 4) { a.hint_a = ptx::kL2EvictFirst; a.hint_b = ptx::kL2EvictLast; }
    else if (b_bytes >= kStream && a_bytes <= kL2Keep && m_tiles <= 4) { a.hint_b = ptx::kL2EvictFirst; a.hint_a = ptx::kL2EvictLast; }
  }
  auto or_undivided = [&](int err) {
    if (err != int(cudaErrorCooperativeLaunchTooLarge) && err != int(cudaErrorLaunchOutOfResources)) return err;
    cudaGetLastError();
    a.plan = undivided(a.plan);
    return launch_mode<Cfg, kPlain>(di, a);
  };
  switch (a.plan.mode) {
    case kStreamK:
      if constexpr (has_mode<Cfg, MODES>(kStreamK)) return or_undivided(launch_mode<Cfg, kStreamK>(di, a));
      break;
    case kClusterSplitK:
      if constexpr (has_mode<Cfg, MODES>(kClusterSplitK)) return launch_mode<Cfg, kClusterSplitK>(di, a);
      break;
    case kWorkspaceSplitK:
      if constexpr (has_mode<Cfg, MODES>(kWorkspaceSplitK)) return or_undivided(launch_mode<Cfg, kWorkspaceSplitK>(di, a));
      break;
    case kPlain:
      break;
  }
  return launch_mode<Cfg, kPlain>(di, a);
}

template <class Cfg, class ResidentClusters>
Plan list_plan(long long max_tiles, int K, int max_workers, ResidentClusters&& resident_clusters) {
  Plan p{};
  p.mode = kPlain;
  p.splits = 1;
  p.num_tiles = int(max_tiles);
  p.nkb = (K + Cfg::BLOCK_K - 1) / Cfg::BLOCK_K;
  if (Cfg::CLUSTER_CTAS > 2) max_workers = std::min(max_workers, resident_clusters());
  p.workers = std::min(std::max(max_workers, 1), p.num_tiles);
  return p;
}

inline int validate_grouped(GemmType type, const void* A, const void* Bt, const void* C, const int* offs, int groups,
                            int T, int N, int K, long long worst_tiles, Scales scales = Scales{nullptr, nullptr},
                            int ld_a = 0) {
  if (!A || !Bt || !C || !offs) return kNullPointer;
  if (T < 0 || groups < 1) return kBadShape;
  return validate(type, A, Bt, C, scales, T > 0 ? T : 1, N, K, ld_a, 1, worst_tiles, offs);
}

inline int validate_k_grouped(GemmType type, const void* A, const void* B, const void* C, const int* offs, int groups,
                              int T, int M, int N, long long tiles) {
  if (!C || !offs || (T != 0 && (!A || !B))) return kNullPointer;
  if (T < 0 || groups < 1) return kBadShape;
  if (T == 0) A = B = C;
  return validate(type, A, B, C, Scales{nullptr, nullptr}, M, N, M, 0, 1, tiles, offs);
}

template <class Cfg>
int validate_list(GemmType type, const void* A, const void* Bt, const void* C, const int* list, int count, int rows,
                  int N, int K, long long tiles, Scales scales, int ld_a) {
  return k_grouped<Cfg>() ? validate_k_grouped(type, A, Bt, C, list, count, K, rows, N, tiles)
         : grouped<Cfg>() ? validate_grouped(type, A, Bt, C, list, count, rows, N, K, tiles, scales, ld_a)
                          : validate(type, A, Bt, C, scales, rows, N, K, ld_a, count, tiles, list);
}

template <class Cfg>
int launch_list(const void* A, const void* Bt, void* C, const int* list, int count, int rows, int N, int K,
                cudaStream_t stream, int group_m = 0, int max_ctas = 0, Scales scales = Scales{nullptr, nullptr},
                int ld_a = 0) {
  static_assert(batched<Cfg>() || grouped<Cfg>() || k_grouped<Cfg>(), "a Batched<>, Grouped<> or GroupedK<> configuration");
  constexpr GemmType kType = gemm_type<Cfg>();
  const long long tiles = Cfg::Cursor::template max_tiles<Cfg>(count, rows, N);
  int st = validate_list<Cfg>(kType, A, Bt, C, list, count, rows, N, K, tiles, scales, ld_a);
  if (st != kOk || rows == 0) return st;
  const Elem elem = traits(kType).operand, output = traits(kType).output;
  if constexpr (k_grouped<Cfg>()) {
    if (K == 0) {
      if constexpr (accum_f32<Cfg>()) return kOk;
      const cudaError_t e = cudaMemsetAsync(C, 0, size_t(count) * size_t(rows) * size_t(N) * elem_bytes(output),
                                            stream);
      return e == cudaSuccess ? kOk : int(e);
    }
  }
  const DeviceInfo& di = device_info();
  if (di.cc_major != 9) return kNotHopper;

  LaunchArgs a{};
  MapCache& cache = map_cache();
  if constexpr (k_grouped<Cfg>()) {
    if ((st = cache.get(A, K, rows, Cfg::A_K_ROWS, &a.ma, 64, elem)) != kOk) return st;
    if ((st = cache.get(Bt, K, N, Cfg::B_K_ROWS, &a.mb, 64, elem)) != kOk) return st;
    if ((st = cache.get(C, rows, N, Cfg::EPI_ROWS, &a.mc, Cfg::EPI_N, output, count)) != kOk) return st;
  } else {
  const int depth = batched<Cfg>() ? count : 0;
  if ((st = cache.get(A, rows, K, Cfg::A_BOX_ROWS, &a.ma, Cfg::BLOCK_K, elem, depth)) != kOk) return st;
  if constexpr (row_major_b<Cfg>()) {
    if ((st = cache.get(Bt, K, N, Cfg::B_K_ROWS, &a.mb, 64, elem, count)) != kOk) return st;
  } else {
    if ((st = cache.get(Bt, N, K, Cfg::B_BOX_ROWS, &a.mb, Cfg::BLOCK_K, elem, count)) != kOk) return st;
  }
  if ((st = cache.get(C, rows, N, Cfg::EPI_ROWS, &a.mc, Cfg::EPI_N, output, depth)) != kOk) return st;
  }
  const int max_workers = (max_ctas > 0 ? max_ctas : di.num_sms) / Cfg::CLUSTER_CTAS;
  a.plan = list_plan<Cfg>(tiles, K, max_workers, [&] { return max_resident_clusters<Cfg>(di); });
  a.M = rows; a.N = N; a.K = K;
  a.group_m = group_m > 0 ? group_m : default_group_m<Cfg>();
  a.c = static_cast<__half*>(C);
  a.hint_a = ptx::kL2EvictNormal; a.hint_b = ptx::kL2EvictNormal;
  a.scales = scales;
  a.ld_a = ld_a;
  a.batches = count;
  a.masked_m = list;
  a.stream = stream;
  return launch_mode<Cfg, kPlain>(di, a);
}

}
}
```

cuda_l2_b200/csrc/hgemm_schedule.cuh:

```cuda
#pragma once
#include <cuda_runtime.h>

namespace b200 {

struct TileCoord { int m_blk, n_blk; };

__host__ __device__ __forceinline__ TileCoord tile_coord(int t, int num_m_blocks, int num_n_blocks, int group_m) {
  const int tiles_per_group = group_m * num_n_blocks;
  const int group = t / tiles_per_group;
  const int first_m = group * group_m;
  const int rest = num_m_blocks - first_m;
  const int gsz = group_m < rest ? group_m : rest;
  const int in_group = t - group * tiles_per_group;
  TileCoord c;
  c.m_blk = first_m + in_group % gsz;
  c.n_blk = in_group / gsz;
  if (group & 1) c.n_blk = num_n_blocks - 1 - c.n_blk;
  return c;
}

struct WorkUnit {
  int tile;
  int kb0, kb1;
};

__host__ __device__ __forceinline__ int streamk_slice_begin(int w, int num_workers, int sk_iters) {
  const int base = sk_iters / num_workers, rem = sk_iters - base * num_workers;
  return w * base + (w < rem ? w : rem);
}

struct WorkIter {
  int it, end;
  int dp_tile;
  int nkb, num_tiles, num_workers;

  __host__ __device__ WorkIter(int worker, int num_workers_, int num_tiles_, int nkb_, int splits, int sk_tiles)
      : nkb(nkb_), num_tiles(num_tiles_), num_workers(num_workers_) {
    if (splits > 1) {
      const int t = worker / splits, s = worker - t * splits;
      const int per = (nkb + splits - 1) / splits;
      const int k0 = s * per, k1 = (k0 + per < nkb) ? k0 + per : nkb;
      it = t * nkb + k0;
      end = (t < num_tiles && k0 < k1) ? t * nkb + k1 : it;
      dp_tile = num_tiles;
    } else {
      const int sk_iters = sk_tiles * nkb;
      it = streamk_slice_begin(worker, num_workers, sk_iters);
      end = streamk_slice_begin(worker + 1, num_workers, sk_iters);
      dp_tile = sk_tiles + worker;
    }
  }

  __host__ __device__ __forceinline__ bool has_more() const { return it < end || dp_tile < num_tiles; }

  __host__ __device__ __forceinline__ bool next(WorkUnit& u) {
    if (it < end) {
      u.tile = it / nkb;
      u.kb0 = it - u.tile * nkb;
      const int left = end - it, room = nkb - u.kb0;
      u.kb1 = u.kb0 + (left < room ? left : room);
      it += u.kb1 - u.kb0;
      return true;
    }
    if (dp_tile < num_tiles) {
      u.tile = dp_tile;
      u.kb0 = 0;
      u.kb1 = nkb;
      dp_tile += num_workers;
      return true;
    }
    return false;
  }
};

struct BatchTile {
  int batch;
  int rows;
  TileCoord tc;
};

struct BatchCursor {
  const int* counts;
  int num_batches, M, block_rows, n_blocks, group_m;
  int batch, first, m_blocks;

  __host__ __device__ BatchCursor(const int* counts_, int num_batches_, int M_, int block_rows_, int n_blocks_,
                                  int group_m_)
      : counts(counts_), num_batches(num_batches_), M(M_), block_rows(block_rows_), n_blocks(n_blocks_),
        group_m(group_m_), batch(0), first(0), m_blocks(blocks_of(0)) {}

  template <class Cfg>
  static constexpr long long max_tiles(int num_batches, int M, int N) {
    const long long per_matrix = ((M - 1LL + Cfg::TILE_M * Cfg::CLUSTER_M) / (Cfg::TILE_M * Cfg::CLUSTER_M)) *
                                 ((N - 1LL + Cfg::BN * Cfg::CLUSTER_N) / (Cfg::BN * Cfg::CLUSTER_N));
    return num_batches * (per_matrix < 0x80000000LL ? per_matrix : 0x80000000LL);
  }

  __host__ __device__ __forceinline__ int rows_of(int b) const {
    if (!counts) return M;
    const int r = counts[b];
    return r < 0 ? 0 : r < M ? r : M;
  }
  __host__ __device__ __forceinline__ int blocks_of(int b) const {
    return b < num_batches ? (rows_of(b) + block_rows - 1) / block_rows : 0;
  }
  __host__ __device__ __forceinline__ int total() const {
    if (!counts) return num_batches * m_blocks * n_blocks;
    int blocks = 0;
    for (int b = 0; b < num_batches; ++b) blocks += blocks_of(b);
    return blocks * n_blocks;
  }
  __host__ __device__ __forceinline__ BatchTile locate(int t) {
    if (!counts) {
      const int per = m_blocks * n_blocks;
      batch = t / per;
      first = batch * per;
    } else {
      while (t >= first + m_blocks * n_blocks) {
        first += m_blocks * n_blocks;
        m_blocks = blocks_of(++batch);
      }
    }
    BatchTile r;
    r.batch = batch;
    r.rows = rows_of(batch);
    r.tc = tile_coord(t - first, m_blocks, n_blocks, group_m);
    return r;
  }
};

struct GroupCursor {
  const int* offs;
  int num_groups, T, block_rows, n_blocks, group_m;
  int group, first, m_blocks, start, end;

  __host__ __device__ GroupCursor(const int* offs_, int num_groups_, int T_, int block_rows_, int n_blocks_,
                                  int group_m_)
      : offs(offs_), num_groups(num_groups_), T(T_), block_rows(block_rows_), n_blocks(n_blocks_), group_m(group_m_),
        group(0), first(0), start(0) {
    end = end_of(0, 0);
    m_blocks = (end - start + block_rows - 1) / block_rows;
  }

  template <class Cfg>
  static constexpr long long max_tiles(int num_groups, int T, int N) {
    return (((long long)T + Cfg::TILE_M * Cfg::CLUSTER_M - 1) / (Cfg::TILE_M * Cfg::CLUSTER_M) + num_groups) *
           (((long long)N + Cfg::BN * Cfg::CLUSTER_N - 1) / (Cfg::BN * Cfg::CLUSTER_N));
  }

  __host__ __device__ __forceinline__ int end_of(int g, int s) const {
    if (g >= num_groups) return s;
    const int e = offs[g];
    return e < s ? s : e < T ? e : T;
  }
  __host__ __device__ __forceinline__ int total() const {
    int blocks = 0, s = 0;
    for (int g = 0; g < num_groups; ++g) {
      const int e = end_of(g, s);
      blocks += (e - s + block_rows - 1) / block_rows;
      s = e;
    }
    return blocks * n_blocks;
  }
  __host__ __device__ __forceinline__ BatchTile locate(int t) {
    while (t >= first + m_blocks * n_blocks) {
      first += m_blocks * n_blocks;
      start = end;
      end = end_of(++group, start);
      m_blocks = (end - start + block_rows - 1) / block_rows;
    }
    BatchTile r;
// ... 68 lines not shown
```

cuda_l2_b200/csrc/hgemm_sm90.cuh:

```cuda
#pragma once
#include <cuda.h>
#include <cuda_runtime.h>
#include <cstdint>
#include <type_traits>

#include "hgemm_schedule.cuh"
#include "ptx_sm90.cuh"
#include "swiglu_arith.cuh"
#include "wgmma_sm90.cuh"


namespace b200 {

constexpr int kBlockKBytes = 128;
constexpr int kBlockK = 64;
constexpr int kWgmmaK = 16;
constexpr int kBlockM = 128;
constexpr int kNumThreads = 384;
constexpr int kEpiWarp0 = 4;
constexpr int kConsumerThreads = 256;
constexpr int kProducerRegs = 40;
constexpr int kConsumerRegs = 232;
constexpr int kSmemLimit = 232448;
enum KMode : int { kPlain = 0, kWorkspaceSplitK = 1, kClusterSplitK = 2, kStreamK = 3 };
struct Scales;
struct Block1D1DArgs;

template <int BN_, int STAGES_, int CTA_GROUP_, bool ACC_F32_, int CLUSTER_M_ = 1, int CLUSTER_N_ = 1, int M_REP_ = 1, bool BF16_ = false,
          bool E4M3_ = false>
struct Config {
  static constexpr int BN = BN_;
  static constexpr int CTA_GROUP = CTA_GROUP_;
  static constexpr bool ACC_F32 = ACC_F32_;
  static constexpr bool BF16 = BF16_;
  static_assert(!BF16_ || ACC_F32_, "bf16 operands accumulate in fp32");
  static constexpr bool E4M3 = E4M3_;
  static_assert(!E4M3_ || ACC_F32_, "e4m3 operands accumulate in fp32");
  static constexpr int OP_BYTES = E4M3_ ? 1 : 2;
  static constexpr int BLOCK_K = kBlockKBytes / OP_BYTES;
  static constexpr int CLUSTER_M = CLUSTER_M_;
  static constexpr int CLUSTER_N = CLUSTER_N_;
  static constexpr int MCAST_CTAS = CLUSTER_M * CLUSTER_N;
  static constexpr int MCAST_M = CTA_GROUP * CLUSTER_M;
  static constexpr int CLUSTER_CTAS = MCAST_M * CLUSTER_N;
  static constexpr int M_REP = M_REP_;
  static constexpr int CTA_M = kBlockM * M_REP;
  static constexpr int TILE_M = CTA_M * CTA_GROUP;
  static constexpr int A_BOX_ROWS = CTA_M / CLUSTER_N;
  static constexpr int B_BOX_ROWS = BN / MCAST_M;
  static constexpr int A_STAGE_BYTES = CTA_M * kBlockK * 2;
  static constexpr int B_STAGE_BYTES = BN * kBlockK * 2;
  static constexpr int STAGE_BYTES = A_STAGE_BYTES + B_STAGE_BYTES;
  static constexpr int EPI_N = BN < 64 ? BN : 64;
  static constexpr int EPI_CHUNKS = BN / EPI_N;
  static constexpr int EPI_ROWS = 16;
  static constexpr int NUM_THREADS = kNumThreads;
  static constexpr bool STREAM_K = CLUSTER_M_ * CLUSTER_N_ == 1 && BN_ >= 64 && M_REP_ == 1;
  static constexpr bool SPLIT_K = STREAM_K && CTA_GROUP_ == 1;
  static constexpr bool BLOCK_SCALED = false, BATCHED = false, GROUPED = false, ROW_MAJOR_B = false, K_GROUPED = false,
                        BIAS_ACT = false, BLOCK_1D1D = false, ACCUM_F32 = false;
  using Cursor = NoBatches;
  using EpiArgs = Scales;
  static constexpr int EPI_BYTES = 8 * EPI_ROWS * 64 * 2;
  static constexpr int BAR_BYTES = 256;
  static constexpr int MAX_STAGES = (kSmemLimit - 1024 - EPI_BYTES - BAR_BYTES) / STAGE_BYTES;
  static constexpr int STAGES = STAGES_ < MAX_STAGES ? STAGES_ : MAX_STAGES;
  static constexpr int SMEM_BYTES = 1024  + STAGES * STAGE_BYTES + EPI_BYTES + BAR_BYTES;
  static_assert(BN == 32 || BN % 64 == 0, "tile N is 32 or a multiple of 64");
  static_assert(BN >= 32 && BN <= 256, "wgmma N constraints");
  static_assert(M_REP * BN <= 256, "register accumulators: at most 256 columns x 128 rows per consumer warpgroup");
  static_assert(CLUSTER_CTAS <= 8, "portable cluster size");
  static_assert(A_BOX_ROWS % 8 == 0 && B_BOX_ROWS % 8 == 0, "slices must cover whole 8-row swizzle atoms");
  static_assert(M_REP == 1 || M_REP == 2, "one or two 128-row blocks per CTA");
  static_assert(A_BOX_ROWS <= 256 && B_BOX_ROWS <= 256, "TMA box dimension limit");
  static_assert(STAGES >= 2, "the ring needs two stages");
  static_assert(SMEM_BYTES <= kSmemLimit, "exceeds 227 KB of shared memory");
  static_assert(A_STAGE_BYTES % 1024 == 0 && B_STAGE_BYTES % 1024 == 0, "swizzle-128B tiles need 1 KB alignment");
  static_assert(8 * (2 * STAGES + 1) <= BAR_BYTES, "barrier block too small");
};

constexpr int kMaxSplitTiles = 256;

template <class Base>
struct BlockScaled : Base {
  static constexpr bool BLOCK_SCALED = true;
  static_assert(Base::E4M3 && Base::M_REP * Base::BN <= 128, "block scales: e4m3, and room for two accumulator sets");
  static constexpr int SA_WINDOW_BYTES = Base::CTA_M * 4;
  static constexpr int SCALE_STAGE_BYTES = SA_WINDOW_BYTES + 16;
  static constexpr int MAX_STAGES =
      (kSmemLimit - 1024 - Base::EPI_BYTES - Base::BAR_BYTES) / (Base::STAGE_BYTES + SCALE_STAGE_BYTES);
  static constexpr int STAGES = Base::STAGES < MAX_STAGES ? Base::STAGES : MAX_STAGES;
  static constexpr int SMEM_BYTES = Base::SMEM_BYTES + STAGES * SCALE_STAGE_BYTES - (Base::STAGES - STAGES) * Base::STAGE_BYTES;
  static_assert(STAGES >= 2 && SMEM_BYTES <= kSmemLimit, "block-scaled ring does not fit");
};
template <class Cfg>
__host__ __device__ constexpr bool block_scaled() { return Cfg::BLOCK_SCALED; }

template <class Base>
struct BlockScaled1D1D : BlockScaled<Base> {
  static constexpr bool BLOCK_1D1D = true;
  using EpiArgs = Block1D1DArgs;
  static constexpr int SA_WINDOW_BYTES = Base::CTA_M * 4;
  static constexpr int SCALE_STAGE_BYTES = SA_WINDOW_BYTES + Base::BN * 4;
  static constexpr int MAX_STAGES =
      (kSmemLimit - 1024 - Base::EPI_BYTES - Base::BAR_BYTES) / (Base::STAGE_BYTES + SCALE_STAGE_BYTES);
  static constexpr int STAGES = Base::STAGES < MAX_STAGES ? Base::STAGES : MAX_STAGES;
  static constexpr int SMEM_BYTES = Base::SMEM_BYTES + STAGES * SCALE_STAGE_BYTES - (Base::STAGES - STAGES) * Base::STAGE_BYTES;
  static_assert(STAGES >= 2 && SMEM_BYTES <= kSmemLimit, "1D1D block-scaled ring does not fit");
  static_assert(SA_WINDOW_BYTES % 16 == 0 && SCALE_STAGE_BYTES % 16 == 0, "bulk copies need 16-byte aligned slices");
};
template <class Cfg>
__host__ __device__ constexpr bool block_1d1d() { return Cfg::BLOCK_1D1D; }

template <class Base>
struct Batched : Base {
  static constexpr bool BATCHED = true;
  using Cursor = BatchCursor;
  static_assert(!Base::E4M3, "batched: 16-bit operands, or block-scaled e4m3 (Batched<BlockScaled<...>>)");
};
template <class Base>
struct Batched<BlockScaled<Base>> : BlockScaled<Base> {
  static constexpr bool BATCHED = true;
  using Cursor = BatchCursor;
};
template <class Cfg>
__host__ __device__ constexpr bool batched() { return Cfg::BATCHED; }

template <class Base>
struct Grouped : Base {
  static constexpr bool GROUPED = true;
  using Cursor = GroupCursor;
  static_assert(!Base::E4M3, "grouped: 16-bit operands, or block-scaled e4m3 (Grouped<BlockScaled<...>>)");
};
template <class Base>
struct Grouped<BlockScaled<Base>> : BlockScaled<Base> {
  static constexpr bool GROUPED = true;
  using Cursor = GroupCursor;
  static constexpr int SA_WINDOW_BYTES = Base::CTA_M * 4 + 16;
  static constexpr int SCALE_STAGE_BYTES = SA_WINDOW_BYTES + 16;
  static constexpr int MAX_STAGES =
      (kSmemLimit - 1024 - Base::EPI_BYTES - Base::BAR_BYTES) / (Base::STAGE_BYTES + SCALE_STAGE_BYTES);
  static constexpr int STAGES = Base::STAGES < MAX_STAGES ? Base::STAGES : MAX_STAGES;
  static constexpr int SMEM_BYTES = Base::SMEM_BYTES + STAGES * SCALE_STAGE_BYTES - (Base::STAGES - STAGES) * Base::STAGE_BYTES;
  static_assert(STAGES >= 2 && SMEM_BYTES <= kSmemLimit, "grouped block-scaled ring does not fit");
  static_assert(Base::CTA_M % 4 == 0, "the scale window's shift is the group's");
};
template <class Cfg>
__host__ __device__ constexpr bool grouped() { return Cfg::GROUPED; }

template <class Base>
struct RowMajorB : Base {
  static constexpr bool ROW_MAJOR_B = true;
  static_assert(!Base::E4M3 && !Base::BLOCK_SCALED && !Base::BATCHED && !Base::GROUPED,
                "row-major B: the 2-D 16-bit kernels only");
  static_assert(Base::BN % 64 == 0, "row-major B: whole 64-column atom columns");
  static constexpr int B_ATOMS = Base::BN / 64;
  static constexpr int B_ATOM_BYTES = 64 * kBlockK * 2;
  static constexpr int B_K_ROWS = kBlockK / Base::MCAST_M;
  static_assert(B_K_ROWS % 8 == 0, "K slices of whole 8-row swizzle groups");
  static_assert(B_ATOMS * B_ATOM_BYTES == Base::B_STAGE_BYTES, "the stage holds the same bytes as the K-major one");
};
template <class Cfg>
__host__ __device__ constexpr bool row_major_b() { return Cfg::ROW_MAJOR_B; }

template <class Base>
struct Grouped<RowMajorB<Base>> : RowMajorB<Base> {
  static constexpr bool GROUPED = true;
  using Cursor = GroupCursor;
};

template <class Base>
struct GroupedK : Base {
  static constexpr bool K_GROUPED = true;
  using Cursor = GroupKCursor;
  static_assert(Base::ROW_MAJOR_B && !Base::GROUPED && Base::ACC_F32, "K-grouped: RowMajorB<> 16-bit configurations, fp32 accumulation");
  static constexpr int A_ATOMS = Base::CTA_M / 64;
  static constexpr int A_K_ROWS = kBlockK / Base::CLUSTER_N;
  static_assert(A_K_ROWS % 8 == 0, "K slices of whole 8-row swizzle groups");
  static_assert(A_ATOMS * Base::B_ATOM_BYTES == Base::A_STAGE_BYTES, "the stage holds the same bytes as the K-major one");
};
template <class Cfg>
__host__ __device__ constexpr bool k_grouped() { return Cfg::K_GROUPED; }

template <class Cfg>
__host__ __device__ __forceinline__ typename Cfg::Cursor make_cursor(const int* list, int count, int M, int K,
                                                                     int block_rows, int n_blocks, int group_m) {
  if constexpr (k_grouped<Cfg>()) return typename Cfg::Cursor(list, count, M, K, block_rows, n_blocks, group_m);
  else return typename Cfg::Cursor(list, count, M, block_rows, n_blocks, group_m);
}

struct Scales { const float* a; const float* b; bool rowwise = false; };

enum Activation : int { kActNone = 0, kActRelu = 1, kActGeluTanh = 2 };
constexpr int kNumActivations = 3;
struct BiasActArgs { Scales scales; const void* bias; int act; };
template <class Base>
struct BiasAct : Base {
  static constexpr bool BIAS_ACT = true;
  using EpiArgs = BiasActArgs;
  static_assert(Base::ACC_F32 && !Base::BLOCK_SCALED && !Base::BATCHED && !Base::GROUPED && !Base::ROW_MAJOR_B &&
                    !Base::K_GROUPED,
                "bias + activation: the 2-D TN kernels with fp32 accumulation only");
};
template <class Cfg>
__host__ __device__ constexpr bool bias_act() { return Cfg::BIAS_ACT; }
__host__ __device__ __forceinline__ const Scales& scales_of(const Scales& s) { return s; }
__host__ __device__ __forceinline__ const Scales& scales_of(const BiasActArgs& e) { return e.scales; }

struct Block1D1DArgs { Scales scales; int ld_b; };
__host__ __device__ __forceinline__ const Scales& scales_of(const Block1D1DArgs& e) { return e.scales; }
template <class E>
__host__ __device__ __forceinline__ int ld_b_of(const E& e) {
  if constexpr (std::is_same_v<E, Block1D1DArgs>) return e.ld_b;
  else return 0;
}

template <class E>
struct AccumArgs { E base; float* c32; };
template <class Base>
struct AccumF32 : Base {
  static constexpr bool ACCUM_F32 = true;
  using AccumBase = Base;
  using EpiArgs = AccumArgs<typename Base::EpiArgs>;
  static_assert(Base::ACC_F32 && !Base::BIAS_ACT && !Base::BATCHED && !Base::GROUPED &&
                    (Base::K_GROUPED || (Base::E4M3 && !Base::ROW_MAJOR_B)) && (!Base::BLOCK_SCALED || Base::BLOCK_1D1D),
                "fp32 accumulation: the K-grouped 16-bit kernels, the 2-D e4m3 ones and the 1 x 128 block-scaled ones");
};
template <class Cfg>
__host__ __device__ constexpr bool accum_f32() { return Cfg::ACCUM_F32; }
template <class E>
__host__ __device__ __forceinline__ const Scales& scales_of(const AccumArgs<E>& e) { return scales_of(e.base); }
template <class E>
__host__ __device__ __forceinline__ int ld_b_of(const AccumArgs<E>& e) { return ld_b_of(e.base); }
template <class E>
__host__ __device__ __forceinline__ float* c32_of(const E&) { return nullptr; }
template <class E>
__host__ __device__ __forceinline__ float* c32_of(const AccumArgs<E>& e) { return e.c32; }

struct GatedArgs { CUtensorMap y_map; int store_h; };
template <class Base>
struct Gated : Base {
  using EpiArgs = GatedArgs;
  static_assert(Base::ACC_F32 && !Base::E4M3 && !Base::BLOCK_SCALED && !Base::BATCHED && !Base::GROUPED &&
                    !Base::ROW_MAJOR_B && !Base::K_GROUPED && !Base::BIAS_ACT && !Base::ACCUM_F32,
                "SwiGLU: the 2-D 16-bit TN kernels with fp32 accumulation only");
  static_assert(Base::BN == 128 || Base::BN == 256, "SwiGLU: whole gate / up pairs of 64-column chunks per tile");
};
template <class Cfg>
__host__ __device__ constexpr bool is_gated() { return std::is_same_v<typename Cfg::EpiArgs, GatedArgs>; }

__device__ __forceinline__ float activate(float z, int act) {
  if (act == kActRelu) return z > 0.f ? z : 0.f;
  if (act == kActGeluTanh) {
    const float inner = __fadd_rn(z, __fmul_rn(0.044715f, __fmul_rn(__fmul_rn(z, z), z)));
    const float u = __fmul_rn(0.7978845608028654f, inner);
    return __fmul_rn(__fmul_rn(0.5f, z), __fadd_rn(1.f, tanhf(u)));
  }
  return z;
}
template <class Cfg>
__device__ __forceinline__ float2 unpack_out_x2(uint32_t v) {
  if constexpr (Cfg::BF16) return make_float2(__uint_as_float(v << 16), __uint_as_float(v & 0xffff0000u));
  else {
    const __half2 h = *reinterpret_cast<const __half2*>(&v);
    return make_float2(__low2float(h), __high2float(h));
  }
}
constexpr uint32_t kNegZeroPair = 0x80008000u;

template <class Cfg>
__device__ __forceinline__ float output_scale(const Scales& s) {
  if constexpr (Cfg::E4M3 && !block_scaled<Cfg>()) return s.rowwise ? 1.f : __fmul_rn(*s.a, *s.b);
  else return 1.f;
}

template <class Cfg>
__device__ __forceinline__ void scale_quad(float4& acc, float scale, const Scales& s, int gm, int gn) {
  if constexpr (Cfg::E4M3 && !block_scaled<Cfg>()) {
    if (s.rowwise) {
      const float sa = s.a[gm];
      const float4 sb = *reinterpret_cast<const float4*>(s.b + gn);
      acc.x = __fmul_rn(__fmul_rn(acc.x, sb.x), sa); acc.y = __fmul_rn(__fmul_rn(acc.y, sb.y), sa);
      acc.z = __fmul_rn(__fmul_rn(acc.z, sb.z), sa); acc.w = __fmul_rn(__fmul_rn(acc.w, sb.w), sa);
    } else {
      acc.x = __fmul_rn(acc.x, scale); acc.y = __fmul_rn(acc.y, scale);
      acc.z = __fmul_rn(acc.z, scale); acc.w = __fmul_rn(acc.w, scale);
    }
  }
}

template <class Cfg>
__device__ __forceinline__ void bias_act_quad(float4& acc, const typename Cfg::EpiArgs& epi, int gn) {
  if constexpr (bias_act<Cfg>()) {
    uint2 bv = make_uint2(kNegZeroPair, kNegZeroPair);
    if (epi.bias) bv = *reinterpret_cast<const uint2*>(static_cast<const uint16_t*>(epi.bias) + gn);
    const float2 lo = unpack_out_x2<Cfg>(bv.x), hi = unpack_out_x2<Cfg>(bv.y);
    acc.x = activate(__fadd_rn(acc.x, lo.x), epi.act); acc.y = activate(__fadd_rn(acc.y, lo.y), epi.act);
    acc.z = activate(__fadd_rn(acc.z, hi.x), epi.act); acc.w = activate(__fadd_rn(acc.w, hi.y), epi.act);
  }
}

struct RowwiseEpi { float sa_lo, sa_hi; const float* sb; };

__device__ __forceinline__ int frag_row(int lane, int p) { return (lane >> 2) + 8 * (p & 1); }
__device__ __forceinline__ int frag_col(int lane, int p) { return (p >> 1) * 8 + (lane & 3) * 2; }

template <class Cfg, class Reg, int NR>
__device__ __forceinline__ float2 acc_pair(const Reg (&d)[NR], int p) {
  if constexpr (Cfg::ACC_F32) {
    return make_float2(d[2 * p], d[2 * p + 1]);
  } else {
    const uint32_t v = d[p];
    const __half2 h = *reinterpret_cast<const __half2*>(&v);
    return make_float2(__low2float(h), __high2float(h));
  }
}
template <class Cfg, class Reg, int NR>
__device__ __forceinline__ uint32_t acc_packed(const Reg (&d)[NR], int p) {
  if constexpr (Cfg::ACC_F32) return ptx::pack_out_x2_rn<Cfg::BF16>(d[2 * p], d[2 * p + 1]);
  else return d[p];
}

template <class Cfg>
__device__ __forceinline__ void bias_act_prefetch(const BiasActArgs& epi, int m0, int n0, int M, int N, int lane) {
  constexpr int kLine = 128;
  const int cols = min(Cfg::BN, N - n0), rows = min(64 * Cfg::M_REP, M - m0);
  if (cols <= 0) return;
  auto fetch = [&](const void* base, int bytes, int first_line) {
    const int i = lane - first_line;
    if (i >= 0 && i * kLine < bytes) asm volatile("prefetch.global.L1 [%0];" ::"l"(static_cast<const char*>(base) + i * kLine));
  };
  if (epi.bias) fetch(static_cast<const uint16_t*>(epi.bias) + n0, cols * 2, 0);
  if constexpr (Cfg::E4M3) {
    if (epi.scales.rowwise) {
      fetch(epi.scales.b + n0, cols * 4, 4);
      if (rows > 0) fetch(epi.scales.a + m0, rows * 4, 12);
    }
  }
}

template <class Cfg, class Reg, int MR, int NR>
__device__ __forceinline__ void bias_in_place(Reg (&d)[MR][NR], int lane, int m_row0, int n0, int M, int N,
                                              const BiasActArgs& epi) {
  const uint32_t* bias = static_cast<const uint32_t*>(epi.bias);
  [[maybe_unused]] const float scale = output_scale<Cfg>(epi.scales);
  [[maybe_unused]] float sa_held[2] = {0.f, 0.f};
  if constexpr (Cfg::E4M3 && MR == 1) {
    if (epi.scales.rowwise) {
#pragma unroll
      for (int h = 0; h < 2; ++h) {
        const int m = m_row0 + frag_row(lane, h);
        sa_held[h] = m < M ? epi.scales.a[m] : 0.f;
      }
    }
  }
#pragma unroll
  for (int c = 0; c < NR / 4; ++c) {
    const int n = n0 + frag_col(lane, 2 * c);
    const float2 b = unpack_out_x2<Cfg>(bias && n < N ? __ldg(bias + n / 2) : kNegZeroPair);
    [[maybe_unused]] float2 sb = make_float2(0.f, 0.f);
    if constexpr (Cfg::E4M3) {
      if (epi.scales.rowwise && n < N) sb = __ldg(reinterpret_cast<const float2*>(epi.scales.b + n));
    }
#pragma unroll
    for (int r = 0; r < MR; ++r) {
#pragma unroll
      for (int h = 0; h < 2; ++h) {
        const int p = 2 * c + h;
        float x = d[r][2 * p], y = d[r][2 * p + 1];
        if constexpr (Cfg::E4M3) {
          if (epi.scales.rowwise) {
            float sa = sa_held[h];
            if constexpr (MR > 1) {
              const int m = m_row0 + 64 * r + frag_row(lane, p);
              sa = m < M ? __ldg(epi.scales.a + m) : 0.f;
            }
            x = __fmul_rn(__fmul_rn(x, sb.x), sa);
            y = __fmul_rn(__fmul_rn(y, sb.y), sa);
          } else {
            x = __fmul_rn(x, scale);
            y = __fmul_rn(y, scale);
          }
        }
        d[r][2 * p] = __fadd_rn(x, b.x);
        d[r][2 * p + 1] = __fadd_rn(y, b.y);
      }
    }
  }
}

template <class Cfg, int ACT, class Reg, int NR>
__device__ __forceinline__ void store_activated(const Reg (&d)[NR], int chunk, uint32_t epi_buf, int lane) {
  constexpr int EN = Cfg::EPI_N;
  constexpr int PER_CHUNK = EN / 4;
#pragma unroll
  for (int q = 0; q < PER_CHUNK; ++q) {
    uint32_t off = uint32_t(frag_row(lane, q) * (EN * 2) + frag_col(lane, q) * 2);
    off ^= (EN == 64 ? ((off >> 7) & 7u) : ((off >> 7) & 3u)) << 4;
    const float2 v = acc_pair<Cfg>(d, chunk * PER_CHUNK + q);
    ptx::st_shared_b32(epi_buf + off, ptx::pack_out_x2_rn<Cfg::BF16>(activate(v.x, ACT), activate(v.y, ACT)));
  }
}

template <class Cfg, class Reg, int NR>
__device__ __forceinline__ void epilogue_store_chunk(const Reg (&d)[NR], int chunk, uint32_t epi_buf, int lane,
                                                     const CUtensorMap* tmap_c, int col0, int row0, int M, int N,
                                                     const RowwiseEpi* rw = nullptr, int batch = 0,
                                                     __half* __restrict__ c_raw = nullptr,
                                                     const typename Cfg::EpiArgs* epi = nullptr) {
  using namespace ptx;
  constexpr int EN = Cfg::EPI_N;
  constexpr int PER_CHUNK = EN / 4;
  if (lane == 0) tma_store_wait_read<0>();
  __syncwarp();
  [[maybe_unused]] float2 sb_lane = make_float2(0.f, 0.f);
  [[maybe_unused]] float sbx = 0.f, sby = 0.f;
  if constexpr (Cfg::E4M3) {
    const int n = col0 + 2 * lane;
    if (rw && 2 * lane < EN && n < N) sb_lane = *reinterpret_cast<const float2*>(rw->sb + n);
  }
  if constexpr (bias_act<Cfg>()) {
    if (epi->act == kActGeluTanh) store_activated<Cfg, kActGeluTanh>(d, chunk, epi_buf, lane);
    else if (epi->act == kActRelu) store_activated<Cfg, kActRelu>(d, chunk, epi_buf, lane);
    else store_activated<Cfg, kActNone>(d, chunk, epi_buf, lane);
  } else {
#pragma unroll
  for (int q = 0; q < PER_CHUNK; ++q) {
    uint32_t off = uint32_t(frag_row(lane, q) * (EN * 2) + frag_col(lane, q) * 2);
    off ^= (EN == 64 ? ((off >> 7) & 7u) : ((off >> 7) & 3u)) << 4;
    if constexpr (Cfg::E4M3) {
      if (rw) {
        if ((q & 1) == 0) {
          const int src = frag_col(lane, q) / 2;
          sbx = __shfl_sync(0xffffffffu, sb_lane.x, src);
          sby = __shfl_sync(0xffffffffu, sb_lane.y, src);
        }
        const float sa = (q & 1) ? rw->sa_hi : rw->sa_lo;
        const float2 v = acc_pair<Cfg>(d, chunk * PER_CHUNK + q);
        st_shared_b32(epi_buf + off, pack_out_x2_rn<Cfg::BF16>(__fmul_rn(__fmul_rn(v.x, sbx), sa),
                                                               __fmul_rn(__fmul_rn(v.y, sby), sa)));
        continue;
      }
    }
    st_shared_b32(epi_buf + off, acc_packed<Cfg>(d, chunk * PER_CHUNK + q));
  }
  }
  fence_proxy_async_smem();
  __syncwarp();
  if constexpr (grouped<Cfg>()) {
    if (row0 + Cfg::EPI_ROWS > M) {
      constexpr int CPR = EN * 2 / 16;
#pragma unroll 1
      for (int i = lane; i < Cfg::EPI_ROWS * CPR; i += 32) {
        const int r = i / CPR, c = i % CPR;
        if (row0 + r < M && col0 + 8 * c < N) {
          uint32_t off = uint32_t(r * (EN * 2) + c * 16);
          off ^= (EN == 64 ? ((off >> 7) & 7u) : ((off >> 7) & 3u)) << 4;
          *reinterpret_cast<uint4*>(c_raw + size_t(row0 + r) * N + col0 + 8 * c) = ld_shared_v4_b32(epi_buf + off);
        }
      }
      return;
    }
  }
  if (lane == 0) {
    if (row0 < M && col0 < N) {
      if constexpr (batched<Cfg>() || k_grouped<Cfg>()) tma_store_3d(tmap_c, epi_buf, col0, row0, batch);
      else tma_store_2d(tmap_c, epi_buf, col0, row0);
    }
    tma_store_commit();
  }
}

template <class Cfg, int R = 0, int J = 0, class Reg, int MR, int NR>
__device__ __forceinline__ void bias_act_epilogue(Reg (&acc)[MR][NR], uint32_t epi_buf, int lane, const CUtensorMap* tmap_c,
                                                  int m_row0, int n0, int M, int N, const BiasActArgs& epi) {
  if constexpr (R < MR) {
    const int row0 = m_row0 + R * 64;
    if constexpr (R == 0 && J == 0) {
      bias_in_place<Cfg>(acc, lane, m_row0, n0, M, N, epi);
#pragma unroll
      for (int r = 0; r < MR; ++r) ptx::reg_fence(acc[r]);
    }
    if constexpr (J < Cfg::EPI_CHUNKS) {
      epilogue_store_chunk<Cfg>(acc[R], J, epi_buf, lane, tmap_c, n0 + J * Cfg::EPI_N, row0, M, N, nullptr, 0, nullptr,
                                &epi);
      bias_act_epilogue<Cfg, R, J + 1>(acc, epi_buf, lane, tmap_c, m_row0, n0, M, N, epi);
    } else {
      bias_act_epilogue<Cfg, R + 1, 0>(acc, epi_buf, lane, tmap_c, m_row0, n0, M, N, epi);
    }
  }
}

template <class Cfg, class Reg, int NR>
__device__ __forceinline__ void gated_store_chunk(const Reg (&d)[NR], int chunk, uint32_t epi_buf, int lane,
                                                  const CUtensorMap* tmap_y, int col0, int row0, int M, int I) {
  using namespace ptx;
  using T = std::conditional_t<Cfg::BF16, __nv_bfloat16, __half>;
  constexpr int EN = Cfg::EPI_N;
  constexpr int PER_CHUNK = EN / 4;
  static_assert(EN == 64, "64-column chunks");
  if (lane == 0) tma_store_wait_read<0>();
  __syncwarp();
#pragma unroll
  for (int q = 0; q < PER_CHUNK; ++q) {
    uint32_t off = uint32_t(frag_row(lane, q) * (EN * 2) + frag_col(lane, q) * 2);
    off ^= ((off >> 7) & 7u) << 4;
    const float2 g = acc_pair<Cfg>(d, chunk * PER_CHUNK + q), u = acc_pair<Cfg>(d, (chunk + 1) * PER_CHUNK + q);
    const float y0 = silu_mul<T>(round_to(g.x, T()), round_to(u.x, T()));
    const float y1 = silu_mul<T>(round_to(g.y, T()), round_to(u.y, T()));
    st_shared_b32(epi_buf + off, pack_out_x2_rn<Cfg::BF16>(y0, y1));
  }
  fence_proxy_async_smem();
  __syncwarp();
  if (lane == 0) {
    if (row0 < M && col0 < I) tma_store_2d(tmap_y, epi_buf, col0, row0);
    tma_store_commit();
  }
}

template <class Cfg, int R = 0, int J = 0, class Reg, int MR, int NR>
__device__ __forceinline__ void gated_epilogue(const Reg (&acc)[MR][NR], uint32_t epi_buf, int lane,
                                               const CUtensorMap* tmap_h, const GatedArgs& epi, int m_row0, int n0,
                                               int M, int N) {
  if constexpr (R < MR) {
    const int row0 = m_row0 + R * 64;
    if constexpr (J < Cfg::EPI_CHUNKS) {
      if (epi.store_h) {
        epilogue_store_chunk<Cfg>(acc[R], J, epi_buf, lane, tmap_h, n0 + J * Cfg::EPI_N, row0, M, N);
        epilogue_store_chunk<Cfg>(acc[R], J + 1, epi_buf, lane, tmap_h, n0 + (J + 1) * Cfg::EPI_N, row0, M, N);
      }
      gated_store_chunk<Cfg>(acc[R], J, epi_buf, lane, &epi.y_map, (n0 + J * Cfg::EPI_N) / 2, row0, M, N / 2);
      gated_epilogue<Cfg, R, J + 2>(acc, epi_buf, lane, tmap_h, epi, m_row0, n0, M, N);
    } else {
      gated_epilogue<Cfg, R + 1, 0>(acc, epi_buf, lane, tmap_h, epi, m_row0, n0, M, N);
    }
  }
}

template <class Cfg>
__device__ __forceinline__ void zero_tile_store(__half* __restrict__ c, int batch, int row0, int col0, int M, int N,
                                                int lane) {
  constexpr int CPR = Cfg::BN / 8;
#pragma unroll 1
  for (int r = 0; r < Cfg::M_REP; ++r) {
#pragma unroll 1
    for (int i = lane; i < Cfg::EPI_ROWS * CPR; i += 32) {
      const int gm = row0 + r * 64 + i / CPR, gn = col0 + 8 * (i % CPR);
      if (gm < M && gn < N) *reinterpret_cast<uint4*>(c + (size_t(batch) * M + gm) * N + gn) = make_uint4(0u, 0u, 0u, 0u);
    }
  }
}

__device__ __forceinline__ void accum_quad(float* __restrict__ dst, const float4& v) {
  float4* p = reinterpret_cast<float4*>(dst);
  float4 o = *p;
  o.x = __fadd_rn(o.x, v.x); o.y = __fadd_rn(o.y, v.y);
  o.z = __fadd_rn(o.z, v.z); o.w = __fadd_rn(o.w, v.w);
  *p = o;
}

template <class Cfg, class Reg, int NR>
__device__ __forceinline__ void accum_block(const Reg (&d)[NR], int lane, int row0, int n0, int M, int N,
                                           float* __restrict__ c32, const Scales& s, float scale) {
  constexpr int PAIRS = NR / 4;
  constexpr int G_MAX = (Cfg::E4M3 && !block_scaled<Cfg>()) ? 2 : 8;
  constexpr int G = PAIRS < G_MAX ? PAIRS : G_MAX;
  static_assert(PAIRS % G == 0, "whole groups");
#pragma unroll
  for (int h = 0; h < 2; ++h) {
    const int m = row0 + frag_row(lane, h);
    if (m >= M) continue;
    [[maybe_unused]] float sa = 0.f;
    if constexpr (Cfg::E4M3 && !block_scaled<Cfg>()) {
      if (s.rowwise) sa = __ldg(s.a + m);
    }
    float* row = c32 + size_t(m) * N;
#pragma unroll
    for (int c0 = 0; c0 < PAIRS; c0 += G) {
      float2 old[G];
#pragma unroll
      for (int j = 0; j < G; ++j) {
        const int n = n0 + frag_col(lane, 2 * (c0 + j) + h);
        old[j] = n < N ? *reinterpret_cast<const float2*>(row + n) : make_float2(0.f, 0.f);
      }
#pragma unroll
      for (int j = 0; j < G; ++j) {
        const int p = 2 * (c0 + j) + h;
        const int n = n0 + frag_col(lane, p);
        if (n >= N) continue;
        float x = d[2 * p], y = d[2 * p + 1];
        if constexpr (Cfg::E4M3 && !block_scaled<Cfg>()) {
          if (s.rowwise) {
            const float2 sb = __ldg(reinterpret_cast<const float2*>(s.b + n));
            x = __fmul_rn(__fmul_rn(x, sb.x), sa);
            y = __fmul_rn(__fmul_rn(y, sb.y), sa);
          } else {
            x = __fmul_rn(x, scale);
            y = __fmul_rn(y, scale);
          }
        }
        *reinterpret_cast<float2*>(row + n) = make_float2(__fadd_rn(old[j].x, x), __fadd_rn(old[j].y, y));
      }
    }
  }
}

template <class Cfg, class Reg, int MR, int NR>
__device__ __forceinline__ void accum_epilogue(const Reg (&d)[MR][NR], int lane, int m_row0, int n0, int M, int N,
                                               float* __restrict__ c32, const Scales& s) {
  static_assert(MR == 1 || MR == 2, "one or two 64-row blocks per warpgroup");
  const float scale = output_scale<Cfg>(s);
  accum_block<Cfg>(d[0], lane, m_row0, n0, M, N, c32, s, scale);
  if constexpr (MR == 2) accum_block<Cfg>(d[1], lane, m_row0 + 64, n0, M, N, c32, s, scale);
}

template <class Cfg, class Reg, int NR>
__device__ __forceinline__ void splitk_epilogue(const Reg (&d)[NR], int e, int row_base, int lane, int tile, int split,
                                                int splits, int m_base, int n0, int M, int N, float* __restrict__ ws,
                                                unsigned* __restrict__ ctr, __half* __restrict__ C,
// ... 284 lines not shown
```

cuda_l2_b200/csrc/hgemm_tn_kernel_body.inc:

```
  constexpr bool kBiasAct = bias_act<Cfg>();
  constexpr bool kAccum = accum_f32<Cfg>();
  constexpr bool kGated = is_gated<Cfg>();
  constexpr int BN = Cfg::BN;
  constexpr int STAGES = Cfg::STAGES;
  constexpr int EM = Cfg::MCAST_M;
  constexpr int CN = Cfg::CLUSTER_N;
  constexpr int MR = Cfg::M_REP;
  constexpr bool kSplit = (KMODE == kWorkspaceSplitK || KMODE == kClusterSplitK);
  static_assert(!kSplit || Cfg::SPLIT_K, "this configuration has no split-K epilogues");
  static_assert(KMODE != kStreamK || Cfg::STREAM_K, "this configuration has no stream-K epilogues");
  static_assert(!kSplit || (kBlockM + 32) * BN * 4 <= STAGES * Cfg::STAGE_BYTES, "split-K partials must fit the pipeline smem");
  const int splits = kSplit ? splits_arg : 1;
  const int sk_tiles = (KMODE == kStreamK) ? aux_arg : 0;
  using namespace ptx;

  extern __shared__ uint8_t smem_raw[];
  const uint32_t smem_base = (smem_u32(smem_raw) + 1023u) & ~1023u;
  const uint32_t smem_a = smem_base;
  const uint32_t smem_b = smem_a + STAGES * Cfg::A_STAGE_BYTES;
  const uint32_t smem_epi = smem_b + STAGES * Cfg::B_STAGE_BYTES;
  const uint32_t smem_bar = smem_epi + Cfg::EPI_BYTES;
  const uint32_t bar_full = smem_bar;
  const uint32_t bar_empty = bar_full + 8 * STAGES;
  const uint32_t bar_splitk = bar_empty + 8 * STAGES;
  constexpr bool kBlock = block_scaled<Cfg>();
  static_assert(!kBlock || KMODE == kPlain || KMODE == kClusterSplitK, "block scales: plain and cluster split-K only");
  [[maybe_unused]] const int ld_a = kBlock ? aux_arg : 0;
  constexpr bool k1D1D = block_1d1d<Cfg>();
  [[maybe_unused]] const int ld_b = ld_b_of(epi);
  [[maybe_unused]] const uint32_t smem_scales = smem_bar + Cfg::BAR_BYTES;
  constexpr bool kBatched = batched<Cfg>();
  constexpr bool kGrouped = grouped<Cfg>();
  constexpr bool kKGrouped = k_grouped<Cfg>();
  constexpr bool kTileList = kBatched || kGrouped || kKGrouped;
  constexpr bool kRowMajorB = row_major_b<Cfg>();
  static_assert(!kTileList || KMODE == kPlain, "batched / grouped: plain schedule only");
  [[maybe_unused]] const int num_batches = kTileList ? splits_arg : 1;
  [[maybe_unused]] const int* masked_m = kTileList ? reinterpret_cast<const int*>(splitk_ctr) : nullptr;
  using Cursor = typename Cfg::Cursor;

  const int warp = __shfl_sync(0xffffffffu, int(threadIdx.x) >> 5, 0);
  const int lane = threadIdx.x & 31;
  const uint32_t cluster_rank = (Cfg::CLUSTER_CTAS > 1) ? cluster_ctarank() : 0u;
  const int mi = int(cluster_rank) % EM;
  const int cn = int(cluster_rank) / EM;

  const int num_m_blocks = (M + Cfg::CTA_M * EM - 1) / (Cfg::CTA_M * EM);
  const int num_n_blocks = (N + BN * CN - 1) / (BN * CN);
  const int num_tiles = num_m_blocks * num_n_blocks;
  [[maybe_unused]] auto gated_m_blocks = [&]() {
    int m = M;
    asm volatile("" : "+r"(m));
    return (m + Cfg::CTA_M * EM - 1) / (Cfg::CTA_M * EM);
  };
  const int num_k_blocks = (K + Cfg::BLOCK_K - 1) / Cfg::BLOCK_K;
  const int num_workers = gridDim.x / Cfg::CLUSTER_CTAS;
  const int worker = blockIdx.x / Cfg::CLUSTER_CTAS;

  constexpr int kReleaseTargets = EM + CN - 1;
  if (threadIdx.x == 0) {
    for (int s = 0; s < STAGES; ++s) {
      mbar_init(bar_full + 8 * s, 1);
      mbar_init(bar_empty + 8 * s, 8 * kReleaseTargets);
    }
    mbar_init(bar_splitk, 1);
    fence_mbar_init();
    tma_prefetch_desc(&tmap_a);
    tma_prefetch_desc(&tmap_b);
    tma_prefetch_desc(&tmap_c);
  }
  if constexpr (Cfg::CLUSTER_CTAS > 1) cluster_sync_all(); else __syncthreads();

  grid_dependency_launch_dependents();
  grid_dependency_wait();

  if (warp < kEpiWarp0) {
    setmaxnreg_dec<kProducerRegs>();
    if (warp == 0) {
      uint16_t mask_a = 0, mask_b = 0;
#pragma unroll
      for (int j = 0; j < CN; ++j) mask_a |= uint16_t(1u << (mi + EM * j));
#pragma unroll
      for (int i = 0; i < EM; ++i) mask_b |= uint16_t(1u << (i + EM * cn));
      const uint32_t a_slice = uint32_t(cn) * (Cfg::A_BOX_ROWS * kBlockK * 2);
      const uint32_t b_slice = uint32_t(mi) * (Cfg::B_BOX_ROWS * kBlockK * 2);
      int stage = 0; uint32_t phase = 0;
      [[maybe_unused]] Cursor batches = make_cursor<Cfg>(masked_m, num_batches, M, K, Cfg::CTA_M * EM, num_n_blocks, group_m);
      WorkIter work(worker, num_workers,
                    kTileList ? batches.total() : kGated ? gated_m_blocks() * num_n_blocks : num_tiles, num_k_blocks,
                    splits, sk_tiles);
      WorkUnit u;
      while (work.next(u)) {
        [[maybe_unused]] BatchTile bt{0, M, TileCoord{0, 0}};
        if constexpr (kKGrouped) bt = batches.unit(u);
        else if constexpr (kTileList) bt = batches.locate(u.tile);
        const TileCoord tc =
            kTileList ? bt.tc : tile_coord(u.tile, kGated ? gated_m_blocks() : num_m_blocks, num_n_blocks, group_m);
        const int m0 = (tc.m_blk * EM + mi) * Cfg::CTA_M + cn * Cfg::A_BOX_ROWS;
        const int n0 = (tc.n_blk * CN + cn) * BN + mi * Cfg::B_BOX_ROWS;
        [[maybe_unused]] int sa_m0 = (tc.m_blk * EM + mi) * Cfg::CTA_M;
        [[maybe_unused]] int sa_rows = kBlock ? max(0, min(Cfg::CTA_M, ld_a - sa_m0)) : 0;
        [[maybe_unused]] const int sb_n0 = (tc.n_blk * CN + cn) * BN;
        [[maybe_unused]] const float* sb_row = (kBlock && !k1D1D && sb_n0 < N) ? scales.b + size_t(sb_n0 / 128) * num_k_blocks : nullptr;
        [[maybe_unused]] const int sb_rows = k1D1D ? max(0, min(BN, ld_b - sb_n0)) : 0;
        if constexpr (kBlock && kGrouped) {
          const int r0 = batches.start + sa_m0;
          sa_m0 = r0 & ~3;
          sa_rows = max(0, min(ld_a - sa_m0, ((r0 & 3) + Cfg::CTA_M + 3) & ~3));
        }
        if constexpr (kBlock && kTileList) {
          if (sb_row) sb_row += size_t(bt.batch) * ((N + 127) / 128) * num_k_blocks;
        }
        [[maybe_unused]] float sb_chunk = 0.f;
        for (int kb = u.kb0; kb < u.kb1; ++kb) {
          mbar_wait(bar_empty + 8 * stage, phase ^ 1);
          [[maybe_unused]] float sb_kb = 0.f;
          if constexpr (kBlock && !k1D1D) {
            if (((kb - u.kb0) & 31) == 0) sb_chunk = (sb_row && kb + lane < u.kb1) ? sb_row[kb + lane] : 0.f;
            sb_kb = __shfl_sync(0xffffffffu, sb_chunk, (kb - u.kb0) & 31);
          }
          if (elect_one()) {
            const uint32_t full = bar_full + 8 * stage;
            if constexpr (k1D1D) {
              const uint32_t sc = smem_scales + stage * Cfg::SCALE_STAGE_BYTES;
              mbar_arrive_expect_tx(full, Cfg::STAGE_BYTES + uint32_t(sa_rows + sb_rows) * 4u);
              if (sa_rows > 0) bulk_load_1d(sc, scales.a + size_t(kb) * ld_a + sa_m0, uint32_t(sa_rows) * 4u, full);
              if (sb_rows > 0)
                bulk_load_1d(sc + Cfg::SA_WINDOW_BYTES, scales.b + size_t(kb) * ld_b + sb_n0, uint32_t(sb_rows) * 4u, full);
            } else if constexpr (kBlock) {
              const uint32_t sc = smem_scales + stage * Cfg::SCALE_STAGE_BYTES;
              st_shared_f32(sc + Cfg::SA_WINDOW_BYTES, sb_kb);
              mbar_arrive_expect_tx(full, Cfg::STAGE_BYTES + uint32_t(sa_rows) * 4u);
              if (sa_rows > 0) {
                if constexpr (kBatched)
                  bulk_load_1d(sc, scales.a + (size_t(bt.batch) * num_k_blocks + kb) * ld_a + sa_m0,
                               uint32_t(sa_rows) * 4u, full);
                else
                  bulk_load_1d(sc, scales.a + size_t(kb) * ld_a + sa_m0, uint32_t(sa_rows) * 4u, full);
              }
            } else {
              mbar_arrive_expect_tx(full, Cfg::STAGE_BYTES);
            }
            const uint32_t dst_a = smem_a + stage * Cfg::A_STAGE_BYTES + a_slice;
            const uint32_t dst_b = smem_b + stage * Cfg::B_STAGE_BYTES + b_slice;
            if constexpr (kBatched) {
              const int b = bt.batch;
              if constexpr (CN > 1) tma_load_3d_mcast_hint(dst_a, &tmap_a, full, kb * Cfg::BLOCK_K, m0, b, mask_a, hint_a);
              else tma_load_3d_hint(dst_a, &tmap_a, full, kb * Cfg::BLOCK_K, m0, b, hint_a);
              if constexpr (EM > 1) tma_load_3d_mcast_hint(dst_b, &tmap_b, full, kb * Cfg::BLOCK_K, n0, b, mask_b, hint_b);
              else tma_load_3d_hint(dst_b, &tmap_b, full, kb * Cfg::BLOCK_K, n0, b, hint_b);
            } else if constexpr (kGrouped) {
              const int ma = batches.start + m0, g = bt.batch;
              if constexpr (CN > 1) tma_load_2d_mcast_hint(dst_a, &tmap_a, full, kb * Cfg::BLOCK_K, ma, mask_a, hint_a);
              else tma_load_2d_hint(dst_a, &tmap_a, full, kb * Cfg::BLOCK_K, ma, hint_a);
              if constexpr (kRowMajorB) {
                const uint32_t dst = smem_b + stage * Cfg::B_STAGE_BYTES + uint32_t(mi) * (Cfg::B_K_ROWS * kBlockKBytes);
                const int nb = (tc.n_blk * CN + cn) * BN, kr = kb * Cfg::BLOCK_K + mi * Cfg::B_K_ROWS;
#pragma unroll
                for (int j = 0; j < Cfg::B_ATOMS; ++j) {
                  if constexpr (EM > 1)
                    tma_load_3d_mcast_hint(dst + j * Cfg::B_ATOM_BYTES, &tmap_b, full, nb + 64 * j, kr, g, mask_b, hint_b);
                  else
                    tma_load_3d_hint(dst + j * Cfg::B_ATOM_BYTES, &tmap_b, full, nb + 64 * j, kr, g, hint_b);
                }
              } else {
              if constexpr (EM > 1) tma_load_3d_mcast_hint(dst_b, &tmap_b, full, kb * Cfg::BLOCK_K, n0, g, mask_b, hint_b);
              else tma_load_3d_hint(dst_b, &tmap_b, full, kb * Cfg::BLOCK_K, n0, g, hint_b);
              }
            } else if constexpr (kKGrouped) {
              const int t0 = batches.start + kb * Cfg::BLOCK_K;
              const uint32_t da = smem_a + stage * Cfg::A_STAGE_BYTES + uint32_t(cn) * (Cfg::A_K_ROWS * kBlockKBytes);
              const int ma = (tc.m_blk * EM + mi) * Cfg::CTA_M, ka = t0 + cn * Cfg::A_K_ROWS;
#pragma unroll
              for (int j = 0; j < Cfg::A_ATOMS; ++j) {
                if constexpr (CN > 1)
                  tma_load_2d_mcast_hint(da + j * Cfg::B_ATOM_BYTES, &tmap_a, full, ma + 64 * j, ka, mask_a, hint_a);
                else
                  tma_load_2d_hint(da + j * Cfg::B_ATOM_BYTES, &tmap_a, full, ma + 64 * j, ka, hint_a);
              }
              const uint32_t db = smem_b + stage * Cfg::B_STAGE_BYTES + uint32_t(mi) * (Cfg::B_K_ROWS * kBlockKBytes);
              const int nb = (tc.n_blk * CN + cn) * BN, kr = t0 + mi * Cfg::B_K_ROWS;
#pragma unroll
              for (int j = 0; j < Cfg::B_ATOMS; ++j) {
                if constexpr (EM > 1)
                  tma_load_2d_mcast_hint(db + j * Cfg::B_ATOM_BYTES, &tmap_b, full, nb + 64 * j, kr, mask_b, hint_b);
                else
                  tma_load_2d_hint(db + j * Cfg::B_ATOM_BYTES, &tmap_b, full, nb + 64 * j, kr, hint_b);
              }
            } else {
            if constexpr (CN > 1) tma_load_2d_mcast_hint(dst_a, &tmap_a, full, kb * Cfg::BLOCK_K, m0, mask_a, hint_a);
            else tma_load_2d_hint(dst_a, &tmap_a, full, kb * Cfg::BLOCK_K, m0, hint_a);
            if constexpr (kRowMajorB) {
              const uint32_t dst = smem_b + stage * Cfg::B_STAGE_BYTES + uint32_t(mi) * (Cfg::B_K_ROWS * kBlockKBytes);
              const int nb = (tc.n_blk * CN + cn) * BN, kr = kb * Cfg::BLOCK_K + mi * Cfg::B_K_ROWS;
#pragma unroll
              for (int j = 0; j < Cfg::B_ATOMS; ++j) {
                if constexpr (EM > 1)
                  tma_load_2d_mcast_hint(dst + j * Cfg::B_ATOM_BYTES, &tmap_b, full, nb + 64 * j, kr, mask_b, hint_b);
                else
                  tma_load_2d_hint(dst + j * Cfg::B_ATOM_BYTES, &tmap_b, full, nb + 64 * j, kr, hint_b);
              }
            } else {
            if constexpr (EM > 1) tma_load_2d_mcast_hint(dst_b, &tmap_b, full, kb * Cfg::BLOCK_K, n0, mask_b, hint_b);
            else tma_load_2d_hint(dst_b, &tmap_b, full, kb * Cfg::BLOCK_K, n0, hint_b);
            }
            }
          }
          __syncwarp();
          if (++stage == STAGES) { stage = 0; phase ^= 1; }
        }
      }
    }
    __syncwarp();
    if constexpr (KMODE == kClusterSplitK) {
      cluster_sync_all();
      cluster_sync_all();
    } else if constexpr (Cfg::CLUSTER_CTAS > 1) {
      cluster_sync_all();
    }
  } else {
    setmaxnreg_inc<kConsumerRegs>();
    using W = typename std::conditional<kKGrouped, Wgmma<BN, true, Cfg::BF16, false, true, true>,
                                        Wgmma<BN, Cfg::ACC_F32, Cfg::BF16 && !Cfg::E4M3, Cfg::E4M3, kRowMajorB>>::type;
    constexpr int kDescBStep = kRowMajorB ? 16 * kBlockKBytes / 16 : 2;
    constexpr int kDescAStep = kKGrouped ? 16 * kBlockKBytes / 16 : 2;
    using Reg = typename W::Reg;
    constexpr int NR = W::kRegs;
    const int wg = warp / 4 - 1;
    const int wq = warp % 4;
    const int ew = warp - kEpiWarp0;
    const int t = int(threadIdx.x) - 128;
    const uint32_t epi_buf = smem_epi + uint32_t(ew) * (Cfg::EPI_ROWS * 64 * 2);
    [[maybe_unused]] int ck_m_base = 0, ck_n0 = 0, ck_split = 0;
    Reg acc[MR][NR];
#pragma unroll
    for (int r = 0; r < MR; ++r)
#pragma unroll
      for (int i = 0; i < NR; ++i) acc[r][i] = Reg(0);
    uint32_t empty_target = bar_empty;
    if constexpr (kReleaseTargets > 1) {
      uint32_t rank = cluster_rank;
      if (lane < EM) rank = uint32_t(lane + EM * cn);
      else if (lane < kReleaseTargets) { const int j = lane - EM; rank = uint32_t(mi + EM * (j < cn ? j : j + 1)); }
      empty_target = mapa(bar_empty, rank);
    }
    auto release = [&](int s) {
      __syncwarp();
      if constexpr (kReleaseTargets > 1) {
        if (lane < kReleaseTargets) mbar_arrive_cluster(empty_target + 8 * s);
      } else {
        if (lane == 0) mbar_arrive(bar_empty + 8 * s);
      }
    };
    int stage = 0; uint32_t phase = 0;
    [[maybe_unused]] Cursor batches = make_cursor<Cfg>(masked_m, num_batches, M, K, Cfg::CTA_M * EM, num_n_blocks, group_m);
    WorkIter work(worker, num_workers,
                  kTileList ? batches.total() : kGated ? gated_m_blocks() * num_n_blocks : num_tiles, num_k_blocks,
                  splits, sk_tiles);
    WorkUnit u;
    while (work.next(u)) {
      if constexpr (kKGrouped) {
        const BatchTile zt = batches.unit(u);
        if (u.kb1 == 0) {
          if constexpr (!kAccum)
            zero_tile_store<Cfg>(c_raw, zt.batch, (zt.tc.m_blk * EM + mi) * Cfg::CTA_M + wg * MR * 64 + wq * 16,
                                 (zt.tc.n_blk * CN + cn) * BN, M, N, lane);
          continue;
        }
      }
      if constexpr (kBiasAct && !kSplit) {
        const TileCoord ptc = tile_coord(u.tile, num_m_blocks, num_n_blocks, group_m);
        if (wq == 0 && (KMODE != kStreamK || u.kb0 == 0))
          bias_act_prefetch<Cfg>(epi, (ptc.m_blk * EM + mi) * Cfg::CTA_M + wg * MR * 64, (ptc.n_blk * CN + cn) * BN, M,
                                 N, lane);
      }
      if constexpr (kBlock) {
        static_assert(MR == 1 && Cfg::ACC_F32, "one 64-row block of fp32 accumulators per warpgroup");
        Reg part[NR];
        [[maybe_unused]] uint32_t sa_shift = 0;
        if constexpr (kGrouped) {
          batches.locate(u.tile);
          sa_shift = uint32_t(batches.start & 3) * 4u;
        }
        const uint32_t sa_off = uint32_t(wg * 64 + wq * 16 + (lane >> 2)) * 4u + sa_shift;
        for (int kb = u.kb0; kb < u.kb1; ++kb) {
          mbar_wait(bar_full + 8 * stage, phase);
          const uint64_t da = make_smem_desc(smem_a + stage * Cfg::A_STAGE_BYTES + uint32_t(wg) * (64 * kBlockK * 2));
          const uint64_t db = make_smem_desc(smem_b + stage * Cfg::B_STAGE_BYTES);
          reg_fence(part);
          wgmma_fence();
#pragma unroll
          for (int k = 0; k < kBlockK / kWgmmaK; ++k) W::mma(da + uint64_t(2 * k), db + uint64_t(2 * k), part, k > 0 ? 1u : 0u);
          wgmma_commit();
          wgmma_wait<0>();
          reg_fence(part);
          const uint32_t sc = smem_scales + stage * Cfg::SCALE_STAGE_BYTES;
          if constexpr (k1D1D) {
            const float sa_lo = ld_shared_f32(sc + sa_off), sa_hi = ld_shared_f32(sc + sa_off + 32u);
            const uint32_t sb_addr = sc + Cfg::SA_WINDOW_BYTES + uint32_t(2 * (lane & 3)) * 4u;
            if (kb == u.kb0) {
#pragma unroll
              for (int j = 0; j < BN / 8; ++j) {
                const float2 sb = ld_shared_v2f(sb_addr + uint32_t(32 * j));
#pragma unroll
                for (int e = 0; e < 4; ++e)
                  acc[0][4 * j + e] = __fmul_rn(part[4 * j + e], __fmul_rn((e & 2) ? sa_hi : sa_lo, (e & 1) ? sb.y : sb.x));
              }
            } else {
#pragma unroll
              for (int j = 0; j < BN / 8; ++j) {
                const float2 sb = ld_shared_v2f(sb_addr + uint32_t(32 * j));
#pragma unroll
                for (int e = 0; e < 4; ++e)
                  acc[0][4 * j + e] = __fmaf_rn(part[4 * j + e], __fmul_rn((e & 2) ? sa_hi : sa_lo, (e & 1) ? sb.y : sb.x),
                                                acc[0][4 * j + e]);
              }
            }
            release(stage);
            if (++stage == STAGES) { stage = 0; phase ^= 1; }
            continue;
          }
          const float sb = ld_shared_f32(sc + Cfg::SA_WINDOW_BYTES);
          const float s_lo = __fmul_rn(ld_shared_f32(sc + sa_off), sb);
          const float s_hi = __fmul_rn(ld_shared_f32(sc + sa_off + 32u), sb);
          release(stage);
          if (kb == u.kb0) {
#pragma unroll
            for (int i = 0; i < NR; ++i) acc[0][i] = __fmul_rn(part[i], (i & 2) ? s_hi : s_lo);
          } else {
#pragma unroll
            for (int i = 0; i < NR; ++i) acc[0][i] = __fmaf_rn(part[i], (i & 2) ? s_hi : s_lo, acc[0][i]);
          }
          if (++stage == STAGES) { stage = 0; phase ^= 1; }
        }
        reg_fence(acc[0]);
      } else {
      int prev = -1;
      for (int kb = u.kb0; kb < u.kb1; ++kb) {
        mbar_wait(bar_full + 8 * stage, phase);
        if constexpr (kKGrouped) {
          const int r = (batches.end - batches.start) - kb * Cfg::BLOCK_K;
          if (r < Cfg::BLOCK_K) {
            const uint32_t a0 = smem_a + stage * Cfg::A_STAGE_BYTES, b0 = smem_b + stage * Cfg::B_STAGE_BYTES;
#pragma unroll 1
            for (uint32_t o = uint32_t(r * kBlockKBytes + 16 * t); o < uint32_t(Cfg::B_ATOM_BYTES); o += 16u * kConsumerThreads) {
#pragma unroll
              for (int j = 0; j < Cfg::A_ATOMS; ++j) st_shared_zero_v4(a0 + uint32_t(j * Cfg::B_ATOM_BYTES) + o);
#pragma unroll
              for (int j = 0; j < Cfg::B_ATOMS; ++j) st_shared_zero_v4(b0 + uint32_t(j * Cfg::B_ATOM_BYTES) + o);
            }
            fence_proxy_async_smem();
            asm volatile("bar.sync 2, %0;" ::"n"(kConsumerThreads) : "memory");
          }
        }
        uint64_t da;
        if constexpr (kKGrouped)
          da = make_smem_desc_mn(smem_a + stage * Cfg::A_STAGE_BYTES + uint32_t(wg * MR) * (64 * kBlockK * 2), 64 * kBlockKBytes);
        else
          da = make_smem_desc(smem_a + stage * Cfg::A_STAGE_BYTES + uint32_t(wg * MR) * (64 * kBlockK * 2));
        uint64_t db;
        if constexpr (kRowMajorB) db = make_smem_desc_mn(smem_b + stage * Cfg::B_STAGE_BYTES, 64 * kBlockKBytes);
        else db = make_smem_desc(smem_b + stage * Cfg::B_STAGE_BYTES);
#pragma unroll
        for (int r = 0; r < MR; ++r) reg_fence(acc[r]);
        wgmma_fence();
#pragma unroll
        for (int k = 0; k < kBlockK / kWgmmaK; ++k) {
#pragma unroll
          for (int r = 0; r < MR; ++r)
            W::mma(da + uint64_t(r * ((64 * kBlockK * 2) >> 4) + kDescAStep * k), db + uint64_t(kDescBStep * k), acc[r],
                   (kb > u.kb0 || k > 0) ? 1u : 0u);
        }
        wgmma_commit();
        if constexpr (KMODE == kStreamK) wgmma_wait<0>();
        else wgmma_wait<1>();
#pragma unroll
        for (int r = 0; r < MR; ++r) reg_fence(acc[r]);
        if (prev >= 0) release(prev);
        prev = stage;
        if (++stage == STAGES) { stage = 0; phase ^= 1; }
      }
      wgmma_wait<0>();
#pragma unroll
      for (int r = 0; r < MR; ++r) reg_fence(acc[r]);
      release(prev);
      }

      const int tile = u.tile;
      [[maybe_unused]] BatchTile bt{0, M, TileCoord{0, 0}};
      if constexpr (kTileList) bt = batches.locate(tile);
      const TileCoord tc =
          kTileList ? bt.tc : tile_coord(tile, kGated ? gated_m_blocks() : num_m_blocks, num_n_blocks, group_m);
      const int m_cta = (tc.m_blk * EM + mi) * Cfg::CTA_M;
      const int n0 = (tc.n_blk * CN + cn) * BN;
      [[maybe_unused]] uint4* ws4 = reinterpret_cast<uint4*>(splitk_ws);
      [[maybe_unused]] unsigned* sk_flags = splitk_ctr + 2 * kMaxSplitTiles;
      if constexpr (KMODE == kStreamK) {
        const int slot = worker * Cfg::CLUSTER_CTAS + int(cluster_rank);
        if (u.kb0 > 0) {
          streamk_contribute<Cfg>(acc[0], t, ew, lane, ws4, sk_flags, slot);
          continue;
        }
        if (u.kb1 < num_k_blocks) {
          const int n = streamk_contributors(worker, num_workers, sk_tiles * num_k_blocks, tile, num_k_blocks);
          streamk_own<Cfg>(acc[0], t, ew, lane, ws4, sk_flags, slot + Cfg::CLUSTER_CTAS, Cfg::CLUSTER_CTAS, n);
        }
      }
      if constexpr (KMODE == kClusterSplitK) {
        asm volatile("bar.sync 1, %0;" ::"n"(kConsumerThreads) : "memory");
        cluster_splitk_park<Cfg>(acc[0], wg * 64 + wq * 16, lane, smem_a);
        ck_m_base = m_cta; ck_n0 = n0; ck_split = worker - tile * splits;
      } else if constexpr (KMODE == kWorkspaceSplitK) {
        splitk_epilogue<Cfg>(acc[0], t, wg * 64 + wq * 16, lane, tile, worker - tile * splits, splits, m_cta, n0, M, N,
                             splitk_ws, splitk_ctr, c_raw, smem_a, bar_splitk, epi);
      } else if constexpr (kAccum) {
        float* c32 = c32_of(epi);
        if constexpr (kKGrouped) c32 += size_t(bt.batch) * M * N;
        accum_epilogue<Cfg>(acc, lane, m_cta + wg * MR * 64 + wq * 16, n0, M, N, c32, scales);
      } else if constexpr (kGated) {
        gated_epilogue<Cfg>(acc, epi_buf, lane, &tmap_c, epi, m_cta + wg * MR * 64 + wq * 16, n0, M, N);
      } else if constexpr (kBiasAct) {
        bias_act_epilogue<Cfg>(acc, epi_buf, lane, &tmap_c, m_cta + wg * MR * 64 + wq * 16, n0, M, N, epi);
      } else {
        if constexpr (Cfg::E4M3 && !kBlock) {
          if (scales.rowwise) {
#pragma unroll
            for (int r = 0; r < MR; ++r) {
              const int row0 = m_cta + (wg * MR + r) * 64 + wq * 16;
              const int ra = row0 + (lane >> 2), rb = ra + 8;
              const RowwiseEpi rw{ra < M ? scales.a[ra] : 0.f, rb < M ? scales.a[rb] : 0.f, scales.b};
#pragma unroll
              for (int j = 0; j < Cfg::EPI_CHUNKS; ++j)
                epilogue_store_chunk<Cfg>(acc[r], j, epi_buf, lane, &tmap_c, n0 + j * Cfg::EPI_N, row0, M, N, &rw);
            }
            continue;
          }
          const float scale = output_scale<Cfg>(scales);
#pragma unroll
          for (int r = 0; r < MR; ++r)
#pragma unroll
            for (int i = 0; i < NR; ++i) acc[r][i] = __fmul_rn(acc[r][i], scale);
#pragma unroll
          for (int r = 0; r < MR; ++r) reg_fence(acc[r]);
        }
#pragma unroll
        for (int r = 0; r < MR; ++r) {
          const int row0 = m_cta + (wg * MR + r) * 64 + wq * 16;
#pragma unroll
          for (int j = 0; j < Cfg::EPI_CHUNKS; ++j) {
            if constexpr (kGrouped)
              epilogue_store_chunk<Cfg>(acc[r], j, epi_buf, lane, &tmap_c, n0 + j * Cfg::EPI_N, batches.start + row0,
                                        batches.end, N, nullptr, 0, c_raw);
            else
              epilogue_store_chunk<Cfg>(acc[r], j, epi_buf, lane, &tmap_c, n0 + j * Cfg::EPI_N, row0,
                                        kBatched ? bt.rows : M, N, nullptr, bt.batch);
          }
        }
      }
    }
    if (lane == 0) tma_store_wait_read<0>();
    __syncwarp();
    if constexpr (KMODE == kClusterSplitK) {
      cluster_sync_all();
      cluster_splitk_reduce<Cfg>(t, ck_split, splits, ck_m_base, ck_n0, M, N, smem_a, c_raw, epi);
      __syncwarp();
      cluster_sync_all();
    } else if constexpr (Cfg::CLUSTER_CTAS > 1) {
      cluster_sync_all();
    }
  }
```

cuda_l2_b200/csrc/ptx_sm90.cuh:

```cuda
#pragma once
#include <cstdint>
#include <cuda_bf16.h>
#include <cuda_fp16.h>

#ifndef B200_HGEMM_WATCHDOG
#define B200_HGEMM_WATCHDOG 1
#endif

namespace b200 {
namespace ptx {

__device__ __forceinline__ uint32_t smem_u32(const void* p) {
  return static_cast<uint32_t>(__cvta_generic_to_shared(p));
}

__device__ __forceinline__ bool elect_one() {
  uint32_t pred = 0;
  asm volatile(
      "{\n\t.reg .pred P;\n\t"
      "elect.sync _|P, 0xffffffff;\n\t"
      "selp.u32 %0, 1, 0, P;\n\t}\n"
      : "=r"(pred));
  return pred != 0;
}

__device__ __forceinline__ uint32_t cluster_ctarank() {
  uint32_t r;
  asm volatile("mov.u32 %0, %%cluster_ctarank;" : "=r"(r));
  return r;
}
__device__ __forceinline__ void cluster_sync_all() {
  asm volatile("barrier.cluster.arrive.release.aligned;\n\t"
               "barrier.cluster.wait.acquire.aligned;" ::: "memory");
}
__device__ __forceinline__ uint32_t mapa(uint32_t local_addr, uint32_t rank) {
  uint32_t r;
  asm volatile("mapa.shared::cluster.u32 %0, %1, %2;" : "=r"(r) : "r"(local_addr), "r"(rank));
  return r;
}

__device__ __forceinline__ void mbar_init(uint32_t bar, uint32_t count) {
  asm volatile("mbarrier.init.shared::cta.b64 [%0], %1;" ::"r"(bar), "r"(count) : "memory");
}
__device__ __forceinline__ void fence_mbar_init() {
  asm volatile("fence.mbarrier_init.release.cluster;" ::: "memory");
}
__device__ __forceinline__ void mbar_arrive(uint32_t bar) {
  asm volatile("mbarrier.arrive.shared::cta.b64 _, [%0];" ::"r"(bar) : "memory");
}
__device__ __forceinline__ void mbar_arrive_cluster(uint32_t cluster_bar) {
  asm volatile("mbarrier.arrive.shared::cluster.b64 _, [%0];" ::"r"(cluster_bar)
               : "memory");
}
__device__ __forceinline__ void mbar_arrive_expect_tx(uint32_t bar, uint32_t bytes) {
  asm volatile("mbarrier.arrive.expect_tx.shared::cta.b64 _, [%0], %1;" ::"r"(bar), "r"(bytes)
               : "memory");
}
__device__ __forceinline__ bool mbar_try_wait(uint32_t bar, uint32_t parity) {
  uint32_t ok;
  asm volatile(
      "{\n\t.reg .pred P;\n\t"
      "mbarrier.try_wait.parity.shared::cta.b64 P, [%1], %2;\n\t"
      "selp.u32 %0, 1, 0, P;\n\t}\n"
      : "=r"(ok)
      : "r"(bar), "r"(parity)
      : "memory");
  return ok != 0;
}
__device__ __forceinline__ void mbar_wait(uint32_t bar, uint32_t parity) {
#if B200_HGEMM_WATCHDOG
  uint32_t spins = 0;
  while (!mbar_try_wait(bar, parity)) {
    if (++spins > (1u << 26)) __trap();
  }
#else
  while (!mbar_try_wait(bar, parity)) {}
#endif
}

__device__ __forceinline__ void fence_proxy_async_smem() {
  asm volatile("fence.proxy.async.shared::cta;" ::: "memory");
}
__device__ __forceinline__ void fence_proxy_async_all() {
  asm volatile("fence.proxy.async;" ::: "memory");
}

__device__ __forceinline__ void tma_prefetch_desc(const void* tmap) {
  asm volatile("prefetch.tensormap [%0];" ::"l"(reinterpret_cast<uint64_t>(tmap)) : "memory");
}
constexpr uint64_t kL2EvictNormal = 0x1000000000000000ull;
constexpr uint64_t kL2EvictFirst = 0x12F0000000000000ull;
constexpr uint64_t kL2EvictLast = 0x14F0000000000000ull;

__device__ __forceinline__ void tma_load_2d_hint(uint32_t smem_dst, const void* tmap, uint32_t bar,
                                                 int32_t c0, int32_t c1, uint64_t hint) {
  asm volatile(
      "cp.async.bulk.tensor.2d.shared::cluster.global.mbarrier::complete_tx::bytes.L2::cache_hint"
      " [%0], [%1, {%3, %4}], [%2], %5;"
      ::"r"(smem_dst), "l"(reinterpret_cast<uint64_t>(tmap)), "r"(bar), "r"(c0), "r"(c1), "l"(hint)
      : "memory");
}
__device__ __forceinline__ void tma_load_2d_mcast_hint(uint32_t smem_dst, const void* tmap, uint32_t bar,
                                                       int32_t c0, int32_t c1, uint16_t mask, uint64_t hint) {
  asm volatile(
      "cp.async.bulk.tensor.2d.shared::cluster.global.mbarrier::complete_tx::bytes.multicast::cluster.L2::cache_hint"
      " [%0], [%1, {%3, %4}], [%2], %5, %6;"
      ::"r"(smem_dst), "l"(reinterpret_cast<uint64_t>(tmap)), "r"(bar), "r"(c0), "r"(c1), "h"(mask), "l"(hint)
      : "memory");
}

__device__ __forceinline__ void tma_load_3d_hint(uint32_t smem_dst, const void* tmap, uint32_t bar,
                                                 int32_t c0, int32_t c1, int32_t c2, uint64_t hint) {
  asm volatile(
      "cp.async.bulk.tensor.3d.shared::cluster.global.mbarrier::complete_tx::bytes.L2::cache_hint"
      " [%0], [%1, {%3, %4, %5}], [%2], %6;"
      ::"r"(smem_dst), "l"(reinterpret_cast<uint64_t>(tmap)), "r"(bar), "r"(c0), "r"(c1), "r"(c2), "l"(hint)
      : "memory");
}
__device__ __forceinline__ void tma_load_3d_mcast_hint(uint32_t smem_dst, const void* tmap, uint32_t bar,
                                                       int32_t c0, int32_t c1, int32_t c2, uint16_t mask, uint64_t hint) {
  asm volatile(
      "cp.async.bulk.tensor.3d.shared::cluster.global.mbarrier::complete_tx::bytes.multicast::cluster.L2::cache_hint"
      " [%0], [%1, {%3, %4, %5}], [%2], %6, %7;"
      ::"r"(smem_dst), "l"(reinterpret_cast<uint64_t>(tmap)), "r"(bar), "r"(c0), "r"(c1), "r"(c2), "h"(mask), "l"(hint)
      : "memory");
}

__device__ __forceinline__ void bulk_load_1d(uint32_t smem_dst, const void* gsrc, uint32_t bytes, uint32_t bar) {
  asm volatile("cp.async.bulk.shared::cluster.global.mbarrier::complete_tx::bytes [%0], [%1], %2, [%3];"
               ::"r"(smem_dst), "l"(reinterpret_cast<uint64_t>(gsrc)), "r"(bytes), "r"(bar)
               : "memory");
}
__device__ __forceinline__ void tma_store_2d(const void* tmap, uint32_t smem_src, int32_t c0, int32_t c1) {
  asm volatile("cp.async.bulk.tensor.2d.global.shared::cta.bulk_group [%0, {%2, %3}], [%1];"
               ::"l"(reinterpret_cast<uint64_t>(tmap)), "r"(smem_src), "r"(c0), "r"(c1)
               : "memory");
}
__device__ __forceinline__ void tma_store_3d(const void* tmap, uint32_t smem_src, int32_t c0, int32_t c1, int32_t c2) {
  asm volatile("cp.async.bulk.tensor.3d.global.shared::cta.bulk_group [%0, {%2, %3, %4}], [%1];"
               ::"l"(reinterpret_cast<uint64_t>(tmap)), "r"(smem_src), "r"(c0), "r"(c1), "r"(c2)
               : "memory");
}
__device__ __forceinline__ void tma_store_commit() {
  asm volatile("cp.async.bulk.commit_group;" ::: "memory");
}
template <int kPending>
__device__ __forceinline__ void tma_store_wait_read() {
  asm volatile("cp.async.bulk.wait_group.read %0;" ::"n"(kPending) : "memory");
}

__device__ __forceinline__ uint64_t make_smem_desc(uint32_t smem_addr) {
  uint64_t d = 0;
  d |= uint64_t((smem_addr & 0x3FFFF) >> 4);
  d |= uint64_t(1) << 16;
  d |= uint64_t(1024 >> 4) << 32;
  d |= uint64_t(1) << 62;
  return d;
}
__device__ __forceinline__ uint64_t make_smem_desc_mn(uint32_t smem_addr, uint32_t lbo) {
  uint64_t d = 0;
  d |= uint64_t((smem_addr & 0x3FFFF) >> 4);
  d |= uint64_t((lbo & 0x3FFFF) >> 4) << 16;
  d |= uint64_t(1024 >> 4) << 32;
  d |= uint64_t(1) << 62;
  return d;
}
__device__ __forceinline__ void wgmma_fence() {
  asm volatile("wgmma.fence.sync.aligned;" ::: "memory");
}
__device__ __forceinline__ void wgmma_commit() {
  asm volatile("wgmma.commit_group.sync.aligned;" ::: "memory");
}
template <int kPending>
__device__ __forceinline__ void wgmma_wait() {
  asm volatile("wgmma.wait_group.sync.aligned %0;" ::"n"(kPending) : "memory");
}
template <int N>
__device__ __forceinline__ void reg_fence(float (&r)[N]) {
#pragma unroll
  for (int i = 0; i < N; ++i) asm volatile("" : "+f"(r[i])::"memory");
}
template <int N>
__device__ __forceinline__ void reg_fence(uint32_t (&r)[N]) {
#pragma unroll
  for (int i = 0; i < N; ++i) asm volatile("" : "+r"(r[i])::"memory");
}

template <int kRegs>
__device__ __forceinline__ void setmaxnreg_dec() {
  asm volatile("setmaxnreg.dec.sync.aligned.u32 %0;" ::"n"(kRegs));
}
template <int kRegs>
__device__ __forceinline__ void setmaxnreg_inc() {
  asm volatile("setmaxnreg.inc.sync.aligned.u32 %0;" ::"n"(kRegs));
}

__device__ __forceinline__ void grid_dependency_wait() {
  asm volatile("griddepcontrol.wait;" ::: "memory");
}
__device__ __forceinline__ void grid_dependency_launch_dependents() {
  asm volatile("griddepcontrol.launch_dependents;" ::: "memory");
}

__device__ __forceinline__ void st_shared_b32(uint32_t addr, uint32_t v) {
  asm volatile("st.shared.b32 [%0], %1;" ::"r"(addr), "r"(v) : "memory");
}
__device__ __forceinline__ void st_shared_f32(uint32_t addr, float v) {
  asm volatile("st.shared.f32 [%0], %1;" ::"r"(addr), "f"(v) : "memory");
}
__device__ __forceinline__ float ld_shared_f32(uint32_t addr) {
  float v;
  asm volatile("ld.shared.f32 %0, [%1];" : "=f"(v) : "r"(addr) : "memory");
  return v;
}
__device__ __forceinline__ float2 ld_shared_v2f(uint32_t addr) {
  float2 v;
  asm volatile("ld.shared.v2.f32 {%0, %1}, [%2];" : "=f"(v.x), "=f"(v.y) : "r"(addr) : "memory");
  return v;
}
__device__ __forceinline__ void st_shared_v2f(uint32_t addr, float a, float b) {
  asm volatile("st.shared.v2.f32 [%0], {%1, %2};" ::"r"(addr), "f"(a), "f"(b) : "memory");
}
__device__ __forceinline__ void st_shared_zero_v4(uint32_t addr) {
  asm volatile("st.shared.v4.b32 [%0], {%1, %1, %1, %1};" ::"r"(addr), "r"(0u) : "memory");
}
__device__ __forceinline__ float4 ld_dsmem_v4f(uint32_t cluster_addr) {
  float4 v;
  asm volatile("ld.shared::cluster.v4.f32 {%0, %1, %2, %3}, [%4];"
               : "=f"(v.x), "=f"(v.y), "=f"(v.z), "=f"(v.w) : "r"(cluster_addr) : "memory");
  return v;
}
__device__ __forceinline__ float4 ld_shared_v4f(uint32_t addr) {
  float4 v;
  asm volatile("ld.shared.v4.f32 {%0, %1, %2, %3}, [%4];" : "=f"(v.x), "=f"(v.y), "=f"(v.z), "=f"(v.w) : "r"(addr) : "memory");
  return v;
}
__device__ __forceinline__ uint4 ld_shared_v4_b32(uint32_t addr) {
  uint4 v;
  asm volatile("ld.shared.v4.b32 {%0, %1, %2, %3}, [%4];" : "=r"(v.x), "=r"(v.y), "=r"(v.z), "=r"(v.w) : "r"(addr) : "memory");
  return v;
}
__device__ __forceinline__ uint32_t pack_f16x2_rn(float lo, float hi) {
  __half2 h = __floats2half2_rn(lo, hi);
  return *reinterpret_cast<uint32_t*>(&h);
}
__device__ __forceinline__ uint32_t pack_bf16x2_rn(float lo, float hi) {
  __nv_bfloat162 h = __floats2bfloat162_rn(lo, hi);
  return *reinterpret_cast<uint32_t*>(&h);
}
template <bool kBf16>
__device__ __forceinline__ uint32_t pack_out_x2_rn(float lo, float hi) {
  if constexpr (kBf16) return pack_bf16x2_rn(lo, hi);
  else return pack_f16x2_rn(lo, hi);
}

__device__ __forceinline__ void st_global_cg_v4(uint4* p, uint32_t a, uint32_t b, uint32_t c, uint32_t d) {
  asm volatile("st.global.cg.v4.b32 [%0], {%1, %2, %3, %4};" ::"l"(p), "r"(a), "r"(b), "r"(c), "r"(d) : "memory");
}
__device__ __forceinline__ uint4 ld_global_cg_v4(const uint4* p) {
  uint4 v;
  asm volatile("ld.global.cg.v4.b32 {%0, %1, %2, %3}, [%4];" : "=r"(v.x), "=r"(v.y), "=r"(v.z), "=r"(v.w) : "l"(p) : "memory");
  return v;
}
__device__ __forceinline__ void st_release_gpu(unsigned* p, unsigned v) {
  asm volatile("st.release.gpu.global.u32 [%0], %1;" ::"l"(p), "r"(v) : "memory");
}
__device__ __forceinline__ unsigned ld_acquire_gpu(const unsigned* p) {
  unsigned v;
  asm volatile("ld.acquire.gpu.global.u32 %0, [%1];" : "=r"(v) : "l"(p) : "memory");
  return v;
}

}
}
```

Before: 741.2.

## Add super-tile raster with per-panel L2 eviction hints for 4096 cube

```diff
diff --git a/cuda_l2_b200/build.py b/cuda_l2_b200/build.py
--- a/cuda_l2_b200/build.py
+++ b/cuda_l2_b200/build.py
@@ -92,6 +92,7 @@
     "epilogue": ("libb200_epilogue.so", _per_variant("b200_epilogue.cu", EPILOGUE_VARIANTS), []),
     "wgrad_accum": ("libb200_wgrad_accum.so", _per_variant("b200_wgrad_accum.cu", WGRAD_ACCUM_VARIANTS), []),
     "swiglu": ("libb200_swiglu.so", _per_variant("b200_swiglu.cu", SWIGLU_VARIANTS), []),
+    "supertile": ("libb200_supertile.so", [(CSRC / "b200_supertile.cu", [])], []),
     "quant": ("libb200_quant.so", [(CSRC / "b200_quant.cu", [])], []),
     "quant_dual": ("libb200_quant_dual.so", [(CSRC / "b200_quant_dual.cu", [])], []),
     "quant_block_dual": ("libb200_quant_block_dual.so", [(CSRC / "b200_quant_block_dual.cu", [])], []),
diff --git a/cuda_l2_b200/capi.py b/cuda_l2_b200/capi.py
--- a/cuda_l2_b200/capi.py
+++ b/cuda_l2_b200/capi.py
@@ -96,6 +96,7 @@
 QUANT_BLOCK_DUAL_LIB = "libb200_quant_block_dual.so"
 WGRAD_ACCUM_LIB = "libb200_wgrad_accum.so"
 SWIGLU_LIB = "libb200_swiglu.so"
+SUPERTILE_LIB = "libb200_supertile.so"
 _QUANT_BLOCK_DUAL = ([_i, _vp, _i, _i, _vp, _vp, _vp, _vp, _vp], _i)
 _QUANT_BLOCKWISE = ([_i, _vp, _i, _i, _i, _vp, _vp, _i, _vp, _vp], _i)
 INTERNAL_ABI = {
@@ -163,6 +164,10 @@
         "cuda_l2_b200_swiglu_launch_count": ([], ctypes.c_ulonglong),
         "cuda_l2_b200_swiglu_strerror": ([_i], ctypes.c_char_p),
     },
+    SUPERTILE_LIB: {
+        "cuda_l2_b200_supertile_run": ([_i, _vp, _vp, _vp, _i, _i, _i, _i, _i, _vp], _i),
+        "cuda_l2_b200_supertile_strerror": ([_i], ctypes.c_char_p),
+    },
 }
 _TABLES = {**ABI, **INTERNAL_ABI}
 _LIBRARY_OF = {symbol: name for name, table in _TABLES.items() for symbol in table}
@@ -807,6 +812,13 @@
     return _select(hgemm_lib().b200_hgemm_select, ACC_BITS[acc], m, n, k)
 
 
+def hgemm_super_tile(a, b_col_major, c, sm: int, sn: int, acc: str | int = "fp32", stream: int | None = None) -> None:
+    m, n, k = _shape_check(a, b_col_major, c)
+    _check(load(SUPERTILE_LIB).cuda_l2_b200_supertile_run(ACC_BITS[acc], a.data_ptr(), b_col_major.data_ptr(),
+                                                          c.data_ptr(), m, n, k, sm, sn, stream),
+           "cuda_l2_b200_supertile_run")
+
+
 STREAMK_TAIL, STREAMK_TAIL_PLUS_WAVE = 100, 101
 KMODES = ("plain", "split-k", "cluster-split-k", "stream-k")
 
diff --git a/cuda_l2_b200/csrc/b200_hgemm_capi.cu b/cuda_l2_b200/csrc/b200_hgemm_capi.cu
--- a/cuda_l2_b200/csrc/b200_hgemm_capi.cu
+++ b/cuda_l2_b200/csrc/b200_hgemm_capi.cu
@@ -9,6 +9,7 @@
 #include <string>
 
 #include "b200_nn.h"
+#include "b200_supertile.h"
 #include "hgemm_configs.cuh"
 #include "hgemm_dispatch.cuh"
 
@@ -61,17 +62,40 @@
   return *slot;
 }
 
+void* sibling_symbol(const char* name, const char* symbol) {
+  Dl_info self{};
+  if (!dladdr(reinterpret_cast<const void*>(&sibling_symbol), &self) || !self.dli_fname) return nullptr;
+  const std::string here(self.dli_fname);
+  const size_t slash = here.rfind('/');
+  const std::string path = (slash == std::string::npos ? std::string() : here.substr(0, slash + 1)) + name;
+  void* lib = dlopen(path.c_str(), RTLD_NOW | RTLD_LOCAL);
+  return lib ? dlsym(lib, symbol) : nullptr;
+}
+
 b200::nn::RunConfigFn nn_run_config() {
-  static const b200::nn::RunConfigFn fn = []() -> b200::nn::RunConfigFn {
-    Dl_info self{};
-    if (!dladdr(reinterpret_cast<const void*>(&nn_run_config), &self) || !self.dli_fname) return nullptr;
-    const std::string here(self.dli_fname);
-    const size_t slash = here.rfind('/');
-    const std::string path = (slash == std::string::npos ? std::string() : here.substr(0, slash + 1)) + b200::nn::kLibrary;
-    void* lib = dlopen(path.c_str(), RTLD_NOW | RTLD_LOCAL);
-    return lib ? reinterpret_cast<b200::nn::RunConfigFn>(dlsym(lib, b200::nn::kRunConfigSymbol)) : nullptr;
-  }();
+  static const auto fn = reinterpret_cast<b200::nn::RunConfigFn>(sibling_symbol(b200::nn::kLibrary,
+                                                                                b200::nn::kRunConfigSymbol));
   return fn;
+}
+
+b200::supertile::RunFn supertile_run() {
+  static const auto fn = reinterpret_cast<b200::supertile::RunFn>(sibling_symbol(b200::supertile::kLibrary,
+                                                                                 b200::supertile::kRunSymbol));
+  return fn;
+}
+
+template <GemmType T>
+int gemm_kmajor(const void* A, const void* B_kmajor, void* C, int M, int N, int K, void* stream) {
+  if (const int st = b200::host::validate(T, A, B_kmajor, C, {}, M, N, K)) return st;
+  const b200::dispatch::Choice ch = b200::dispatch::select(T, M, N, K);
+  if (const b200::supertile::Shape* s = b200::supertile::find(T, ch.config_id, ch.splits, M, N, K)) {
+    const b200::supertile::RunFn run = supertile_run();
+    if (!run) return b200::host::kNoSuperTileLibrary;
+    const int st = run(b200::host::traits(T).acc_f32 ? 32 : 16, A, B_kmajor, C, M, N, K, s->sm, s->sn, stream);
+    if (st == b200::host::kOk) b200::g_launches.fetch_add(1, std::memory_order_relaxed);
+    return st;
+  }
+  return b200::run_config<T>(ch.config_id, A, B_kmajor, C, {}, M, N, K, ch.group_m, 0, ch.splits, stream);
 }
 
 template <GemmType T>
@@ -162,13 +186,13 @@
 int b200_hgemm_f32acc(const void* A, const void* B_rowmajor, const void* B_kmajor, void* C, int M, int N,
                       int K, void* stream) {
   if (!B_kmajor && B_rowmajor) return gemm_rowmajor<GemmType::kF16Acc32>(A, B_rowmajor, C, M, N, K, stream);
-  return b200::dispatch::gemm<GemmType::kF16Acc32>(A, B_kmajor, C, {}, M, N, K, stream);
+  return gemm_kmajor<GemmType::kF16Acc32>(A, B_kmajor, C, M, N, K, stream);
 }
 
 int b200_hgemm_f16acc(const void* A, const void* B_rowmajor, const void* B_kmajor, void* C, int M, int N,
                       int K, void* stream) {
   if (!B_kmajor && B_rowmajor) return gemm_rowmajor<GemmType::kF16Acc16>(A, B_rowmajor, C, M, N, K, stream);
-  return b200::dispatch::gemm<GemmType::kF16Acc16>(A, B_kmajor, C, {}, M, N, K, stream);
+  return gemm_kmajor<GemmType::kF16Acc16>(A, B_kmajor, C, M, N, K, stream);
 }
 
 int b200_bgemm_f32acc(const void* A, const void* B_rowmajor, const void* B_kmajor, void* C, int M, int N,
diff --git a/cuda_l2_b200/csrc/b200_supertile.cu b/cuda_l2_b200/csrc/b200_supertile.cu
--- /dev/null
+++ b/cuda_l2_b200/csrc/b200_supertile.cu
@@ -0,0 +1,18 @@
+#include "b200_supertile.h"
+#include "hgemm_configs.cuh"
+
+extern "C" int cuda_l2_b200_supertile_run(int acc_bits, const void* A, const void* B_kmajor, void* C, int M, int N,
+                                          int K, int sm, int sn, void* stream) {
+  using b200::host::GemmType;
+  if (sm < 1 || sm > 255 || sn < 1 || sn > 255) return b200::host::kBadShape;
+  const int word = b200::super_tile(sm, sn);
+  if (acc_bits == 32)
+    return b200::run_config<GemmType::kF16Acc32, b200::SuperTile>(b200::supertile::kConfig, A, B_kmajor, C, {}, M, N, K,
+                                                                  word, 0, 1, stream);
+  if (acc_bits == 16)
+    return b200::run_config<GemmType::kF16Acc16, b200::SuperTile>(b200::supertile::kConfig, A, B_kmajor, C, {}, M, N, K,
+                                                                  word, 0, 1, stream);
+  return b200::host::kBadConfig;
+}
+
+extern "C" const char* cuda_l2_b200_supertile_strerror(int status) { return b200::host::status_string(status); }
diff --git a/cuda_l2_b200/csrc/b200_supertile.h b/cuda_l2_b200/csrc/b200_supertile.h
--- /dev/null
+++ b/cuda_l2_b200/csrc/b200_supertile.h
@@ -0,0 +1,33 @@
+#pragma once
+#include "hgemm_configs.cuh"
+
+extern "C" {
+
+int cuda_l2_b200_supertile_run(int acc_bits, const void* A, const void* B_kmajor, void* C, int M, int N, int K, int sm,
+                               int sn, void* stream);
+const char* cuda_l2_b200_supertile_strerror(int status);
+
+}
+
+namespace b200 {
+namespace supertile {
+
+using RunFn = decltype(&cuda_l2_b200_supertile_run);
+constexpr const char* kLibrary = "libb200_supertile.so";
+constexpr const char* kRunSymbol = "cuda_l2_b200_supertile_run";
+
+struct Shape { int m, n, k, sm, sn; };
+constexpr Shape kShapes[] = {
+    {4096, 4096, 4096, 8, 8},
+};
+
+inline const Shape* find(host::GemmType type, int config_id, int splits, int M, int N, int K) {
+  if ((type != host::GemmType::kF16Acc32 && type != host::GemmType::kF16Acc16) || config_id != kConfig || splits != 1)
+    return nullptr;
+  for (const Shape& s : kShapes)
+    if (s.m == M && s.n == N && s.k == K) return &s;
+  return nullptr;
+}
+
+}
+}
diff --git a/cuda_l2_b200/csrc/hgemm_configs.cuh b/cuda_l2_b200/csrc/hgemm_configs.cuh
--- a/cuda_l2_b200/csrc/hgemm_configs.cuh
+++ b/cuda_l2_b200/csrc/hgemm_configs.cuh
@@ -140,15 +140,25 @@
 
 }
 
+namespace supertile {
+constexpr int kConfig = 3;
+constexpr bool has_kernel(int id) { return id == kConfig; }
+constexpr unsigned kModes = 1u << kPlain;
+}
+
 template <class Probe>
 constexpr bool has_kernel(int id) {
   return block_scaled<Probe>() ? block::eligible(id)
          : row_major_b<Probe>() ? nn::has_kernel(id)
          : is_gated<Probe>()    ? gated::has_kernel(id)
+         : super_tile_raster<Probe>() ? supertile::has_kernel(id)
                                 : true;
 }
 template <class Probe>
-constexpr unsigned k_modes() { return block_scaled<Probe>() ? block::kModes : is_gated<Probe>() ? gated::kModes : 0xFu; }
+constexpr unsigned k_modes() {
+  return block_scaled<Probe>() ? block::kModes : is_gated<Probe>() ? gated::kModes
+         : super_tile_raster<Probe>() ? supertile::kModes : 0xFu;
+}
 
 template <class Cfg>
 using Unwrapped = Cfg;
diff --git a/cuda_l2_b200/csrc/hgemm_host.cuh b/cuda_l2_b200/csrc/hgemm_host.cuh
--- a/cuda_l2_b200/csrc/hgemm_host.cuh
+++ b/cuda_l2_b200/csrc/hgemm_host.cuh
@@ -29,6 +29,7 @@
   kNoNNLibrary = -11,
   kBadActivation = -12,
   kBadScaleLdB = -13,
+  kNoSuperTileLibrary = -14,
 };
 
 inline const char* status_string(int s) {
@@ -47,6 +48,8 @@
     case kNoNNLibrary: return "row-major B needs libb200_nn.so next to libb200_hgemm.so (missing, or it does not load)";
     case kBadActivation: return "unknown activation code (0 none, 1 relu, 2 gelu_tanh)";
     case kBadScaleLdB: return "1 x 128 scales of Bt need ld_b >= N and ld_b % 4 == 0 (16-byte aligned k-block rows)";
+    case kNoSuperTileLibrary:
+      return "this shape runs the super-tile raster of libb200_supertile.so, next to libb200_hgemm.so (missing, or it does not load)";
     default: return s > 0 ? cudaGetErrorString(static_cast<cudaError_t>(s)) : "unknown error";
   }
 }
@@ -520,6 +523,10 @@
   }
   a.M = M; a.N = N; a.K = K;
   a.group_m = group_m > 0 ? group_m : default_group_m<Cfg>();
+  if constexpr (super_tile_raster<Cfg>())
+    a.group_m = cache_hints_enabled() ? (group_m | kPanelHints) : (group_m & ~kPanelHints);
+  else if (is_super_tile(a.group_m))
+    a.group_m = default_group_m<Cfg>();
   a.c = static_cast<__half*>(C);
   a.scales = scales;
   a.ld_a = ld_a;
@@ -633,7 +640,7 @@
   const int max_workers = (max_ctas > 0 ? max_ctas : di.num_sms) / Cfg::CLUSTER_CTAS;
   a.plan = list_plan<Cfg>(tiles, K, max_workers, [&] { return max_resident_clusters<Cfg>(di); });
   a.M = rows; a.N = N; a.K = K;
-  a.group_m = group_m > 0 ? group_m : default_group_m<Cfg>();
+  a.group_m = group_m > 0 && !is_super_tile(group_m) ? group_m : default_group_m<Cfg>();
   a.c = static_cast<__half*>(C);
   a.hint_a = ptx::kL2EvictNormal; a.hint_b = ptx::kL2EvictNormal;
   a.scales = scales;
diff --git a/cuda_l2_b200/csrc/hgemm_schedule.cuh b/cuda_l2_b200/csrc/hgemm_schedule.cuh
--- a/cuda_l2_b200/csrc/hgemm_schedule.cuh
+++ b/cuda_l2_b200/csrc/hgemm_schedule.cuh
@@ -17,6 +17,55 @@
   c.n_blk = in_group / gsz;
   if (group & 1) c.n_blk = num_n_blocks - 1 - c.n_blk;
   return c;
+}
+
+constexpr int kSuperTile = 1 << 30;
+__host__ __device__ constexpr int super_tile(int sm, int sn) { return kSuperTile | (sm & 0xff) << 8 | (sn & 0xff); }
+__host__ __device__ __forceinline__ bool is_super_tile(int group_m) { return (group_m & kSuperTile) != 0; }
+constexpr int kPanelHints = 1 << 29;
+__host__ __device__ __forceinline__ bool has_panel_hints(int group_m) {
+  return (group_m & (kSuperTile | kPanelHints)) == (kSuperTile | kPanelHints);
+}
+__host__ __device__ __forceinline__ int super_tile_m(int group_m, int num_m_blocks) {
+  const int s = (group_m >> 8) & 0xff;
+  return s < 1 ? 1 : s < num_m_blocks ? s : num_m_blocks;
+}
+__host__ __device__ __forceinline__ int super_tile_n(int group_m, int num_n_blocks) {
+  const int s = group_m & 0xff;
+  return s < 1 ? 1 : s < num_n_blocks ? s : num_n_blocks;
+}
+
+struct SuperTilePos { int r, c, h, l; };
+__host__ __device__ __forceinline__ SuperTilePos super_tile_pos(int t, int num_m_blocks, int num_n_blocks, int group_m) {
+  const int sm = super_tile_m(group_m, num_m_blocks), sn = super_tile_n(group_m, num_n_blocks);
+  SuperTilePos p;
+  p.r = t / (sm * num_n_blocks);
+  const int rest = num_m_blocks - p.r * sm;
+  p.h = sm < rest ? sm : rest;
+  const int in_row = t - p.r * sm * num_n_blocks;
+  p.c = in_row / (p.h * sn);
+  p.l = in_row - p.c * p.h * sn;
+  return p;
+}
+
+__host__ __device__ __forceinline__ TileCoord super_tile_coord(int t, int num_m_blocks, int num_n_blocks, int group_m) {
+  const SuperTilePos p = super_tile_pos(t, num_m_blocks, num_n_blocks, group_m);
+  const int sm = super_tile_m(group_m, num_m_blocks), sn = super_tile_n(group_m, num_n_blocks);
+  const int col = p.l / p.h;
+  const int row = p.l - col * p.h;
+  TileCoord c;
+  c.m_blk = p.r * sm + ((col & 1) ? p.h - 1 - row : row);
+  c.n_blk = p.c * sn + col;
+  if (p.r & 1) c.n_blk = num_n_blocks - 1 - c.n_blk;
+  return c;
+}
+
+enum PanelReuse { kReuseNone = 0, kReuseA = 1, kReuseB = 2 };
+__host__ __device__ __forceinline__ int super_tile_reuse(int t, int num_m_blocks, int num_n_blocks, int group_m) {
+  const SuperTilePos p = super_tile_pos(t, num_m_blocks, num_n_blocks, group_m);
+  const int sm = super_tile_m(group_m, num_m_blocks), sn = super_tile_n(group_m, num_n_blocks);
+  if ((p.c + 1) * sn < num_n_blocks) return kReuseA;
+  return (p.r + 1) * sm < num_m_blocks ? kReuseB : kReuseNone;
 }
 
 struct WorkUnit {
diff --git a/cuda_l2_b200/csrc/hgemm_sm90.cuh b/cuda_l2_b200/csrc/hgemm_sm90.cuh
--- a/cuda_l2_b200/csrc/hgemm_sm90.cuh
+++ b/cuda_l2_b200/csrc/hgemm_sm90.cuh
@@ -58,7 +58,7 @@
   static constexpr bool STREAM_K = CLUSTER_M_ * CLUSTER_N_ == 1 && BN_ >= 64 && M_REP_ == 1;
   static constexpr bool SPLIT_K = STREAM_K && CTA_GROUP_ == 1;
   static constexpr bool BLOCK_SCALED = false, BATCHED = false, GROUPED = false, ROW_MAJOR_B = false, K_GROUPED = false,
-                        BIAS_ACT = false, BLOCK_1D1D = false, ACCUM_F32 = false;
+                        BIAS_ACT = false, BLOCK_1D1D = false, ACCUM_F32 = false, SUPER_TILE = false;
   using Cursor = NoBatches;
   using EpiArgs = Scales;
   static constexpr int EPI_BYTES = 8 * EPI_ROWS * 64 * 2;
@@ -181,6 +181,22 @@
 };
 template <class Cfg>
 __host__ __device__ constexpr bool k_grouped() { return Cfg::K_GROUPED; }
+
+template <class Base>
+struct SuperTile : Base {
+  static constexpr bool SUPER_TILE = true;
+  static_assert(!Base::E4M3 && !Base::BLOCK_SCALED && !Base::BATCHED && !Base::GROUPED && !Base::ROW_MAJOR_B &&
+                    !Base::K_GROUPED && !Base::BIAS_ACT && !Base::ACCUM_F32,
+                "super-tile raster: the 2-D 16-bit TN kernels only");
+};
+template <class Cfg>
+__host__ __device__ constexpr bool super_tile_raster() { return Cfg::SUPER_TILE; }
+
+template <class Cfg>
+__host__ __device__ __forceinline__ TileCoord raster_coord(int t, int num_m_blocks, int num_n_blocks, int group_m) {
+  if constexpr (super_tile_raster<Cfg>()) return super_tile_coord(t, num_m_blocks, num_n_blocks, group_m);
+  else return tile_coord(t, num_m_blocks, num_n_blocks, group_m);
+}
 
 template <class Cfg>
 __host__ __device__ __forceinline__ typename Cfg::Cursor make_cursor(const int* list, int count, int M, int K,
@@ -407,7 +423,8 @@
                                                      const CUtensorMap* tmap_c, int col0, int row0, int M, int N,
                                                      const RowwiseEpi* rw = nullptr, int batch = 0,
                                                      __half* __restrict__ c_raw = nullptr,
-                                                     const typename Cfg::EpiArgs* epi = nullptr) {
+                                                     const typename Cfg::EpiArgs* epi = nullptr,
+                                                     uint64_t hint_c = ptx::kL2EvictNormal) {
   using namespace ptx;
   constexpr int EN = Cfg::EPI_N;
   constexpr int PER_CHUNK = EN / 4;
@@ -465,6 +482,7 @@
   if (lane == 0) {
     if (row0 < M && col0 < N) {
       if constexpr (batched<Cfg>() || k_grouped<Cfg>()) tma_store_3d(tmap_c, epi_buf, col0, row0, batch);
+      else if constexpr (super_tile_raster<Cfg>()) tma_store_2d_hint(tmap_c, epi_buf, col0, row0, hint_c);
       else tma_store_2d(tmap_c, epi_buf, col0, row0);
     }
     tma_store_commit();
diff --git a/cuda_l2_b200/csrc/hgemm_tn_kernel_body.inc b/cuda_l2_b200/csrc/hgemm_tn_kernel_body.inc
--- a/cuda_l2_b200/csrc/hgemm_tn_kernel_body.inc
+++ b/cuda_l2_b200/csrc/hgemm_tn_kernel_body.inc
@@ -35,6 +35,8 @@
   constexpr bool kTileList = kBatched || kGrouped || kKGrouped;
   constexpr bool kRowMajorB = row_major_b<Cfg>();
   static_assert(!kTileList || KMODE == kPlain, "batched / grouped: plain schedule only");
+  constexpr bool kSuperTile = super_tile_raster<Cfg>();
+  static_assert(!kSuperTile || KMODE == kPlain, "super-tile raster: plain schedule only");
   [[maybe_unused]] const int num_batches = kTileList ? splits_arg : 1;
   [[maybe_unused]] const int* masked_m = kTileList ? reinterpret_cast<const int*>(splitk_ctr) : nullptr;
   using Cursor = typename Cfg::Cursor;
@@ -95,7 +97,15 @@
         if constexpr (kKGrouped) bt = batches.unit(u);
         else if constexpr (kTileList) bt = batches.locate(u.tile);
         const TileCoord tc =
-            kTileList ? bt.tc : tile_coord(u.tile, kGated ? gated_m_blocks() : num_m_blocks, num_n_blocks, group_m);
+            kTileList ? bt.tc : raster_coord<Cfg>(u.tile, kGated ? gated_m_blocks() : num_m_blocks, num_n_blocks, group_m);
+        [[maybe_unused]] uint64_t ha = hint_a, hb = hint_b;
+        if constexpr (kSuperTile) {
+          if (has_panel_hints(group_m)) {
+            const int reuse = super_tile_reuse(u.tile, num_m_blocks, num_n_blocks, group_m);
+            ha = reuse == kReuseA ? kL2EvictLast : kL2EvictFirst;
+            hb = reuse == kReuseB ? kL2EvictLast : kL2EvictFirst;
+          }
+        }
         const int m0 = (tc.m_blk * EM + mi) * Cfg::CTA_M + cn * Cfg::A_BOX_ROWS;
         const int n0 = (tc.n_blk * CN + cn) * BN + mi * Cfg::B_BOX_ROWS;
         [[maybe_unused]] int sa_m0 = (tc.m_blk * EM + mi) * Cfg::CTA_M;
@@ -188,8 +198,8 @@
                   tma_load_2d_hint(db + j * Cfg::B_ATOM_BYTES, &tmap_b, full, nb + 64 * j, kr, hint_b);
               }
             } else {
-            if constexpr (CN > 1) tma_load_2d_mcast_hint(dst_a, &tmap_a, full, kb * Cfg::BLOCK_K, m0, mask_a, hint_a);
-            else tma_load_2d_hint(dst_a, &tmap_a, full, kb * Cfg::BLOCK_K, m0, hint_a);
+            if constexpr (CN > 1) tma_load_2d_mcast_hint(dst_a, &tmap_a, full, kb * Cfg::BLOCK_K, m0, mask_a, ha);
+            else tma_load_2d_hint(dst_a, &tmap_a, full, kb * Cfg::BLOCK_K, m0, ha);
             if constexpr (kRowMajorB) {
               const uint32_t dst = smem_b + stage * Cfg::B_STAGE_BYTES + uint32_t(mi) * (Cfg::B_K_ROWS * kBlockKBytes);
               const int nb = (tc.n_blk * CN + cn) * BN, kr = kb * Cfg::BLOCK_K + mi * Cfg::B_K_ROWS;
@@ -201,8 +211,8 @@
                   tma_load_2d_hint(dst + j * Cfg::B_ATOM_BYTES, &tmap_b, full, nb + 64 * j, kr, hint_b);
               }
             } else {
-            if constexpr (EM > 1) tma_load_2d_mcast_hint(dst_b, &tmap_b, full, kb * Cfg::BLOCK_K, n0, mask_b, hint_b);
-            else tma_load_2d_hint(dst_b, &tmap_b, full, kb * Cfg::BLOCK_K, n0, hint_b);
+            if constexpr (EM > 1) tma_load_2d_mcast_hint(dst_b, &tmap_b, full, kb * Cfg::BLOCK_K, n0, mask_b, hb);
+            else tma_load_2d_hint(dst_b, &tmap_b, full, kb * Cfg::BLOCK_K, n0, hb);
             }
             }
           }
@@ -269,7 +279,7 @@
         }
       }
       if constexpr (kBiasAct && !kSplit) {
-        const TileCoord ptc = tile_coord(u.tile, num_m_blocks, num_n_blocks, group_m);
+        const TileCoord ptc = raster_coord<Cfg>(u.tile, num_m_blocks, num_n_blocks, group_m);
         if (wq == 0 && (KMODE != kStreamK || u.kb0 == 0))
           bias_act_prefetch<Cfg>(epi, (ptc.m_blk * EM + mi) * Cfg::CTA_M + wg * MR * 64, (ptc.n_blk * CN + cn) * BN, M,
                                  N, lane);
@@ -390,7 +400,7 @@
       [[maybe_unused]] BatchTile bt{0, M, TileCoord{0, 0}};
       if constexpr (kTileList) bt = batches.locate(tile);
       const TileCoord tc =
-          kTileList ? bt.tc : tile_coord(tile, kGated ? gated_m_blocks() : num_m_blocks, num_n_blocks, group_m);
+          kTileList ? bt.tc : raster_coord<Cfg>(tile, kGated ? gated_m_blocks() : num_m_blocks, num_n_blocks, group_m);
       const int m_cta = (tc.m_blk * EM + mi) * Cfg::CTA_M;
       const int n0 = (tc.n_blk * CN + cn) * BN;
       [[maybe_unused]] uint4* ws4 = reinterpret_cast<uint4*>(splitk_ws);
@@ -451,6 +461,9 @@
             if constexpr (kGrouped)
               epilogue_store_chunk<Cfg>(acc[r], j, epi_buf, lane, &tmap_c, n0 + j * Cfg::EPI_N, batches.start + row0,
                                         batches.end, N, nullptr, 0, c_raw);
+            else if constexpr (kSuperTile)
+              epilogue_store_chunk<Cfg>(acc[r], j, epi_buf, lane, &tmap_c, n0 + j * Cfg::EPI_N, row0, M, N, nullptr, 0,
+                                        nullptr, nullptr, has_panel_hints(group_m) ? kL2EvictFirst : kL2EvictNormal);
             else
               epilogue_store_chunk<Cfg>(acc[r], j, epi_buf, lane, &tmap_c, n0 + j * Cfg::EPI_N, row0,
                                         kBatched ? bt.rows : M, N, nullptr, bt.batch);
diff --git a/cuda_l2_b200/csrc/ptx_sm90.cuh b/cuda_l2_b200/csrc/ptx_sm90.cuh
--- a/cuda_l2_b200/csrc/ptx_sm90.cuh
+++ b/cuda_l2_b200/csrc/ptx_sm90.cuh
@@ -136,6 +136,12 @@
                ::"l"(reinterpret_cast<uint64_t>(tmap)), "r"(smem_src), "r"(c0), "r"(c1)
                : "memory");
 }
+__device__ __forceinline__ void tma_store_2d_hint(const void* tmap, uint32_t smem_src, int32_t c0, int32_t c1,
+                                                  uint64_t hint) {
+  asm volatile("cp.async.bulk.tensor.2d.global.shared::cta.bulk_group.L2::cache_hint [%0, {%2, %3}], [%1], %4;"
+               ::"l"(reinterpret_cast<uint64_t>(tmap)), "r"(smem_src), "r"(c0), "r"(c1), "l"(hint)
+               : "memory");
+}
 __device__ __forceinline__ void tma_store_3d(const void* tmap, uint32_t smem_src, int32_t c0, int32_t c1, int32_t c2) {
   asm volatile("cp.async.bulk.tensor.3d.global.shared::cta.bulk_group [%0, {%2, %3, %4}], [%1];"
                ::"l"(reinterpret_cast<uint64_t>(tmap)), "r"(smem_src), "r"(c0), "r"(c1), "r"(c2)
```

Measured after the change: 754.2, median of 6. 1.02x the previous value.
